# octavian-ganea/equidock_public

Measured on AMD Instinct MI355X. Metric: protein-pairs/sec (fwd+bwd) per IEGMN stack, higher is better.
Workload: dtype f32; 1 GPU; B: DB5.5-sized batch of 8 pairs x (200,200) residues, k=10, 8-layer IEGMN hdim 64, 50 heads, fp32; pairs_per_gpu=8, nodes_per_gpu=3200, edges_per_gpu=32000, layers=8, parallelism=dp1, weights=PyTorch default init (seed 0), ROT key/query x40 (SURVEY.md section 8c), svd_guard_pairs=0, launch_mode=hipGraph replay

## Files before the change

equidock_public_amd/_lib.py:

```python
import ctypes as C
import os

import torch

HERE = os.path.dirname(os.path.abspath(__file__))
LIB_PATH = os.path.join(HERE, 'libequidock_hip.so')
if os.environ.get('EQD_EXP_LIBRARY'):
    LIB_PATH = os.environ['EQD_EXP_LIBRARY']

EQD_MAX_SRC = 6
ABI_VERSION = 9
PARAMS_PER_LAYER = 19
GLOBAL_PARAMS = 5

c_float_p = C.POINTER(C.c_float)
c_int_p = C.POINTER(C.c_int32)


class EqdGraph(C.Structure):
    _fields_ = [('n_pairs', C.c_int32), ('n_lig', C.c_int32), ('n_rec', C.c_int32), ('n_nodes', C.c_int32),
                ('n_edges', C.c_int32), ('n_tiles', C.c_int32), ('n_att_items', C.c_int32), ('max_seg', C.c_int32),
                ('seg_off', C.c_void_p), ('src', C.c_void_p), ('dst', C.c_void_p), ('rowptr', C.c_void_p),
                ('csc_ptr', C.c_void_p), ('csc_eid', C.c_void_p), ('tile_node', C.c_void_p),
                ('att_items', C.c_void_p), ('res_id', C.c_void_p), ('mu_r_norm', C.c_void_p), ('he', C.c_void_p),
                ('x0', C.c_void_p), ('he_bf16', C.c_void_p)]


class EqdModelDesc(C.Structure):
    _fields_ = [('n_layers', C.c_int32), ('d_emb', C.c_int32), ('d_hid', C.c_int32),
                ('use_mean_node_features', C.c_int32), ('edge_feats', C.c_int32), ('n_heads', C.c_int32),
                ('cross_msgs', C.c_int32), ('use_dist_in_layers', C.c_int32), ('use_edge_features', C.c_int32),
                ('skip_weight_h', C.c_float), ('x_connection_init', C.c_float), ('lrelu_slope', C.c_float),
                ('ln_eps', C.c_float), ('svd_seed', C.c_int32), ('storage_bf16', C.c_int32)]


class EqdDropout(C.Structure):
    _fields_ = [('p', C.c_float), ('edge_z1', C.c_void_p), ('edge_ch', C.c_void_p), ('node', C.c_void_p),
                ('head', C.c_void_p)]


class EqdLinSrc(C.Structure):
    _fields_ = [('X', C.c_void_p), ('mask', C.c_void_p), ('W', C.c_void_p), ('ldx', C.c_int32), ('K', C.c_int32),
                ('w_rs', C.c_int32), ('w_cs', C.c_int32)]


class EqdLinJob(C.Structure):
    _fields_ = [('s', EqdLinSrc * EQD_MAX_SRC), ('nsrc', C.c_int32), ('M', C.c_int32), ('act', C.c_int32),
                ('rows', C.c_int32), ('bias', C.c_void_p), ('ln_g', C.c_void_p), ('ln_b', C.c_void_p),
                ('pre_ln', C.c_void_p), ('ld_pre', C.c_int32), ('R', C.c_void_p), ('ldr', C.c_int32),
                ('alpha', C.c_float), ('beta', C.c_float), ('slope', C.c_float), ('ln_eps', C.c_float),
                ('Y', C.c_void_p), ('ldy', C.c_int32), ('bf16', C.c_int32), ('mul', C.c_void_p), ('ld_mul', C.c_int32), ('pad_to', C.c_int32),
                ('Yb', C.c_void_p), ('ldyb', C.c_int32)]


class EqdAtbJob(C.Structure):
    _fields_ = [('X', C.c_void_p), ('xmask', C.c_void_p), ('ldx', C.c_int32), ('M', C.c_int32), ('Y', C.c_void_p),
                ('ldy', C.c_int32), ('N', C.c_int32), ('rows', C.c_int32), ('out', C.c_void_p), ('o_rs', C.c_int32),
                ('o_cs', C.c_int32), ('bias_out', C.c_void_p), ('slope', C.c_float), ('scale', C.c_float), ('bf16', C.c_int32),
                ('y_bf16', C.c_int32)]


class EqdEdgeParams(C.Structure):
    _fields_ = [('W1', C.c_void_p), ('ldw1', C.c_int32), ('d_in', C.c_int32), ('ln_g', C.c_void_p),
                ('ln_b', C.c_void_p), ('W2', C.c_void_p), ('b2', C.c_void_p), ('Wc1', C.c_void_p),
                ('bc1', C.c_void_p), ('wc2', C.c_void_p), ('bc2', C.c_void_p), ('slope', C.c_float),
                ('ln_eps', C.c_float), ('eta', C.c_float), ('use_dist', C.c_int32), ('use_he', C.c_int32),
                ('bf16', C.c_int32), ('drop_z1', C.c_void_p), ('drop_ch', C.c_void_p), ('drop_scale', C.c_float),
                ('aggr_bf16', C.c_void_p), ('xh_save', C.c_void_p), ('rstd_save', C.c_void_p), ('zpos_save', C.c_void_p)]


class EqdNodeUpdateParams(C.Structure):
    _fields_ = [('d_in', C.c_int32), ('d0', C.c_int32), ('d_out', C.c_int32), ('ld_cross', C.c_int32), ('Wn1', C.c_void_p),
                ('bn1', C.c_void_p), ('ln_g', C.c_void_p), ('ln_b', C.c_void_p), ('Wn2', C.c_void_p), ('bn2', C.c_void_p),
                ('skip_weight_h', C.c_float), ('slope', C.c_float), ('ln_eps', C.c_float), ('bf16', C.c_int32),
                ('drop_mul', C.c_void_p)]


class EqdNodeUpdateGrads(C.Structure):
    _fields_ = [('dWn1', C.c_void_p), ('dbn1', C.c_void_p), ('dln_g', C.c_void_p), ('dln_b', C.c_void_p),
                ('dWn2', C.c_void_p), ('dbn2', C.c_void_p)]


class EqdEdgeGrads(C.Structure):
    _fields_ = [('dW1', C.c_void_p), ('ldw1', C.c_int32), ('db1_unused', C.c_void_p), ('dln_g', C.c_void_p),
                ('dln_b', C.c_void_p), ('dW2', C.c_void_p), ('db2', C.c_void_p), ('dWc1', C.c_void_p),
                ('dbc1', C.c_void_p), ('dwc2', C.c_void_p), ('dbc2', C.c_void_p)]


_lib = None
_is_sim = False
profiling = False


class EquidockHipError(RuntimeError):
    pass


def _declare(lib):
    lib.eqd_abi_version.restype = C.c_int
    lib.eqd_last_error.restype = C.c_char_p
    lib.eqd_tile_edges.restype = C.c_int
    lib.eqd_is_simulator.restype = C.c_int
    lib.eqd_model_saved_bytes.restype = C.c_size_t
    lib.eqd_model_scratch_bytes.restype = C.c_size_t
    lib.eqd_atb_partial_bytes.restype = C.c_size_t
    lib.eqd_edge_message_bwd_workspace_bytes.restype = C.c_size_t
    lib.eqd_keypoint_pool_bwd_workspace_bytes.restype = C.c_size_t
    lib.eqd_clash_workspace_bytes.restype = C.c_size_t
    lib.eqd_node_update_bwd_workspace_bytes.restype = C.c_size_t
    lib.eqd_cross_attention_bwd_ds_workspace_bytes.restype = C.c_size_t
    lib.eqd_profile_name.restype = C.c_char_p
    lib.eqd_profile_us.restype = C.c_float
    lib.eqd_tunables_reload.restype = None
    for name in ('eqd_model_layer_state', 'eqd_model_lrelu_signs', 'eqd_model_head_backward', 'eqd_profile_begin', 'eqd_profile_end', 'eqd_profile_mark', 'eqd_ctx_create', 'eqd_ctx_destroy', 'eqd_model_check', 'eqd_model_forward', 'eqd_model_backward', 'eqd_linear', 'eqd_atb',
                 'eqd_edge_message_fwd', 'eqd_edge_message_bwd', 'eqd_edge_message_bwd_kernel_only',
                 'eqd_cross_attention_fwd', 'eqd_cross_attention_fwd_bf16', 'eqd_cross_attention_bwd_bf16',
                 'eqd_cross_attention_bwd', 'eqd_cross_attention_bwd_ds',
           'eqd_keypoint_pool_fwd', 'eqd_keypoint_pool_bwd', 'eqd_kabsch_fwd', 'eqd_kabsch_bwd',
                 'eqd_rigid_apply_fwd', 'eqd_rigid_apply_bwd', 'eqd_pair_losses_fwd', 'eqd_pair_losses_bwd', 'eqd_scalar_loss', 'eqd_pocket_ot_cost',
                 'eqd_pocket_ot_fwd', 'eqd_pocket_ot_bwd', 'eqd_rigid_augment', 'eqd_protein_graph_distances',
                 'eqd_protein_graph_select', 'eqd_protein_graph_edges', 'eqd_clash_iterations', 'eqd_dropout_pack_edges', 'eqd_dropout_draw',
                 'eqd_node_update_fwd', 'eqd_node_update_bwd', 'eqd_selftest_lane_exchanges'):
        getattr(lib, name).restype = C.c_int


EXPORTS = ('eqd_model_layer_state', 'eqd_model_lrelu_signs', 'eqd_model_head_backward', 'eqd_profile_begin', 'eqd_profile_end', 'eqd_profile_mark', 'eqd_profile_name', 'eqd_profile_us', 'eqd_ctx_create', 'eqd_ctx_destroy', 'eqd_abi_version', 'eqd_last_error', 'eqd_tile_edges', 'eqd_is_simulator', 'eqd_model_saved_bytes', 'eqd_model_saved_layout',
           'eqd_model_scratch_bytes', 'eqd_model_check', 'eqd_model_forward', 'eqd_model_backward', 'eqd_linear',
           'eqd_atb_partial_bytes', 'eqd_atb', 'eqd_edge_message_fwd', 'eqd_edge_message_bwd_workspace_bytes',
           'eqd_edge_message_bwd', 'eqd_edge_message_bwd_kernel_only', 'eqd_cross_attention_fwd',
           'eqd_cross_attention_bwd', 'eqd_cross_attention_bwd_ds', 'eqd_cross_attention_bwd_ds_workspace_bytes', 'eqd_cross_attention_fwd_bf16', 'eqd_cross_attention_bwd_bf16',
           'eqd_keypoint_pool_fwd', 'eqd_keypoint_pool_bwd',
           'eqd_keypoint_pool_bwd_workspace_bytes',
           'eqd_kabsch_fwd', 'eqd_kabsch_bwd', 'eqd_rigid_apply_fwd', 'eqd_rigid_apply_bwd', 'eqd_pair_losses_fwd',
           'eqd_pair_losses_bwd', 'eqd_scalar_loss', 'eqd_pocket_ot_cost', 'eqd_pocket_ot_fwd', 'eqd_pocket_ot_bwd',
           'eqd_rigid_augment', 'eqd_protein_graph_distances', 'eqd_protein_graph_select', 'eqd_protein_graph_edges',
           'eqd_clash_workspace_bytes', 'eqd_clash_iterations', 'eqd_dropout_pack_edges', 'eqd_dropout_draw',
           'eqd_tunables_reload', 'eqd_node_update_fwd', 'eqd_node_update_bwd_workspace_bytes', 'eqd_node_update_bwd',
           'eqd_selftest_lane_exchanges', 'eqd_chain_resident_proj_launches', 'eqd_selftest_node_chain_fwd', 'eqd_model_node_state',
           'eqd_chain_resident_wide_launches', 'eqd_chain_resident_wide_bwd_launches', 'eqd_selftest_node_chain_bwd_wide',
           'eqd_edge_fwd_half_launches', 'eqd_selftest_edge_attn_fwd')


def load_library():
    global _lib, _is_sim
    if _lib is not None:
        return _lib
    if not os.path.exists(LIB_PATH):
        raise EquidockHipError(
            f"{LIB_PATH} is missing: build it with `python -m equidock_public_amd.build` (hipcc, gfx950). "
            "There is no CPU fallback for the IEGMN hot path.")
    lib = C.CDLL(LIB_PATH)
    _declare(lib)
    if lib.eqd_abi_version() != ABI_VERSION:
        raise EquidockHipError(f"ABI version mismatch: library {lib.eqd_abi_version()} != {ABI_VERSION}")
    _lib, _is_sim = lib, bool(lib.eqd_is_simulator())
    return _lib


def load_library_for_testing(path):
    global _lib, _is_sim
    lib = C.CDLL(path)
    _declare(lib)
    _lib, _is_sim = lib, bool(lib.eqd_is_simulator())
    return _lib


def unload_for_testing():
    global _lib, _is_sim
    _lib, _is_sim = None, False


tunables_generation = 0


def reload_tunables():
    global tunables_generation
    tunables_generation += 1
    if _lib is not None:
        _lib.eqd_tunables_reload()


def is_simulator():
    return _is_sim


def check(rc):
    if rc != 0:
        raise EquidockHipError(f"libequidock_hip error {rc}: {_lib.eqd_last_error().decode()}")


def require_device(t, what='tensor'):
    if _is_sim:
        if t.is_cuda:
            raise EquidockHipError(f"{what}: the host simulator only takes CPU tensors")
    elif not t.is_cuda:
        raise EquidockHipError(
            f"{what} is on {t.device}: the IEGMN hot path runs only on an MI355X through libequidock_hip.so "
            "(no CPU fallback)")
    return t


class device_guard:

    def __init__(self, device):
        self._cm = None if (_is_sim or torch.device(device).type != 'cuda') else torch.cuda.device(device)

    def __enter__(self):
        if self._cm is not None:
            self._cm.__enter__()

    def __exit__(self, *exc):
        if self._cm is not None:
            self._cm.__exit__(*exc)
        return False


def ptr(t):
    return C.c_void_p(t.data_ptr()) if t is not None else C.c_void_p(0)


def stream_ptr(device):
    if _is_sim:
        return C.c_void_p(0)
    return C.c_void_p(torch.cuda.current_stream(device).cuda_stream)


_ctx = {}


def exec_ctx(device):
    if os.environ.get('EQD_FORK') != '1':
        return C.c_void_p(0)
    key = (id(_lib), str(device))
    if key not in _ctx:
        h = C.c_void_p(0)
        if not _is_sim:
            with torch.cuda.device(device):
                check(_lib.eqd_ctx_create(C.byref(h)))
        else:
            check(_lib.eqd_ctx_create(C.byref(h)))
        _ctx[key] = h
    return _ctx[key]


def graph_struct(p):
    g = EqdGraph()
    g.n_pairs, g.n_lig, g.n_rec, g.n_nodes = p.n_pairs, p.n_lig, p.n_rec, p.n_nodes
    g.n_edges, g.n_tiles, g.n_att_items, g.max_seg = p.n_edges, p.n_tiles, p.n_att_items, p.max_seg
    for name in ('seg_off', 'src', 'dst', 'rowptr', 'csc_ptr', 'csc_eid', 'tile_node', 'att_items', 'res_id',
                 'mu_r_norm', 'he', 'x0', 'he_bf16'):
        t = getattr(p, name)
        require_device(t, 'graph.' + name)
        setattr(g, name, t.data_ptr())
    return g
```

equidock_public_amd/csrc/eqd_common.h:

```cpp
#pragma once
#include <hip/hip_runtime.h>
#include <stdint.h>
#include <string.h>

#include "../../include/equidock_hip.h"

typedef float f32x4 __attribute__((ext_vector_type(4)));
typedef unsigned int u32x4 __attribute__((ext_vector_type(4)));

#define EQD_BLOCK 256
#define EQD_WAVES 4
#define EQD_NEG_BIG (-1.0e30f)

__device__ __forceinline__ f32x4 mfma4(float a, float b, f32x4 c) {
    return __builtin_amdgcn_mfma_f32_16x16x4f32(a, b, c, 0, 0, 0);
}
#ifdef EQD_TRACE
extern __device__ long long eqd_trace_buf[1024];
#define EQD_TR(slot)                                                                          \
    do {                                                                                      \
        const int trs_ = (slot);                                                              \
        if (blockIdx.x == 0 && blockIdx.y == 0 && threadIdx.x == 0 && trs_ < 256) {           \
            eqd_trace_buf[2 * trs_] = clock64();                                              \
            eqd_trace_buf[2 * trs_ + 1] = wall_clock64();                                     \
        }                                                                                     \
    } while (0)
#define EQD_TR_WG()                                                                           \
    do {                                                                                      \
        if (threadIdx.x == 0 && blockIdx.y == 0 && blockIdx.x < 256)                          \
            eqd_trace_buf[512 + 2 * blockIdx.x] = wall_clock64();                             \
    } while (0)
#define EQD_TR_WG_END()                                                                       \
    do {                                                                                      \
        __syncthreads();                                                                      \
        if (threadIdx.x == 0 && blockIdx.y == 0 && blockIdx.x < 256)                          \
            eqd_trace_buf[512 + 2 * blockIdx.x + 1] = wall_clock64();                         \
    } while (0)
#else
#define EQD_TR(slot) do { } while (0)
#define EQD_TR_WG() do { } while (0)
#define EQD_TR_WG_END() do { } while (0)
#endif

#ifndef EQD_GAS
#define EQD_GAS __attribute__((address_space(1)))
#endif

typedef float f4v __attribute__((ext_vector_type(4), aligned(4)));
__device__ __forceinline__ f32x4 ld4u_raw(const float* __restrict__ p, int n, const float* __restrict__ safe) {
    const int sh = (n > 0 && n < 4) ? 4 - n : 0;
    return *(const EQD_GAS f4v*)(n > 0 ? p - sh : safe);
}
__device__ __forceinline__ float4 ld4u_fix(f32x4 v, int n) {
    const int sh = (n > 0 && n < 4) ? 4 - n : 0;
    float4 r;
    r.x = n > 0 ? (sh == 0 ? v[0] : sh == 1 ? v[1] : sh == 2 ? v[2] : v[3]) : 0.f;
    r.y = n > 1 ? (sh == 0 ? v[1] : sh == 1 ? v[2] : v[3]) : 0.f;
    r.z = n > 2 ? (sh == 0 ? v[2] : v[3]) : 0.f;
    r.w = n > 3 ? v[3] : 0.f;
    return r;
}
#ifndef EQD_KERNARG_PTR
#define EQD_KERNARG_PTR(first_param) ((const void*)__builtin_amdgcn_kernarg_segment_ptr())
#endif
__device__ __forceinline__ int uni(int v) { return __builtin_amdgcn_readfirstlane(v); }
__device__ __forceinline__ float uni(float v) {
    return __builtin_bit_cast(float, __builtin_amdgcn_readfirstlane(__builtin_bit_cast(int, v)));
}
template <class T>
__device__ __forceinline__ T* uni(T* p) {
    const unsigned long long a = (unsigned long long)p;
    const unsigned lo = (unsigned)__builtin_amdgcn_readfirstlane((int)(unsigned)a);
    const unsigned hi = (unsigned)__builtin_amdgcn_readfirstlane((int)(unsigned)(a >> 32));
    return (T*)(((unsigned long long)hi << 32) | lo);
}
__device__ __forceinline__ EqdLinSrc uni(const EqdLinSrc& S) {
    EqdLinSrc U;
    U.X = uni(S.X); U.mask = uni(S.mask); U.W = uni(S.W);
    U.ldx = uni(S.ldx); U.K = uni(S.K); U.w_rs = uni(S.w_rs); U.w_cs = uni(S.w_cs);
    return U;
}
template <class T>
__device__ __forceinline__ void kernarg_to_lds(T& dst, const void* kernarg, int byte_offset) {
    const int* __restrict__ src = (const int*)((const char*)kernarg + byte_offset);
    for (int i = threadIdx.x; i < (int)(sizeof(T) / 4); i += blockDim.x) ((int*)&dst)[i] = src[i];
}

#ifdef EQD_HOSTSIM
__device__ __forceinline__ void glds16(const float* gsrc, float* lds_base) {
    __builtin_memcpy(lds_base + 4 * (threadIdx.x & 63), gsrc, 16);
}
template <int N>
__device__ __forceinline__ void vm_wait() { static_assert(N >= 0 && N <= 63, "vmcnt is a 6-bit count"); }
__device__ __forceinline__ void lds_barrier() { __syncthreads(); }
__device__ __forceinline__ void lds_reads_done() {}
template <class T>
__device__ __forceinline__ void keep_after_wait(T&) {}
#else
__device__ __forceinline__ void glds16(const float* gsrc, float* lds_base) {
    const unsigned dst = (unsigned)__builtin_amdgcn_readfirstlane((int)(unsigned)(uintptr_t)(__attribute__((address_space(3))) void*)lds_base);
    unsigned keep;
    asm volatile("s_mov_b32 %0, m0\n\ts_mov_b32 m0, %2\n\ts_nop 0\n\tglobal_load_lds_dwordx4 %1, off\n\ts_mov_b32 m0, %0"
                 : "=&s"(keep)
                 : "v"(gsrc), "s"(dst)
                 : "memory");
}
template <int N>
__device__ __forceinline__ void vm_wait() {
    static_assert(N >= 0 && N <= 63, "vmcnt is a 6-bit count");
    asm volatile("s_waitcnt vmcnt(%0)" ::"n"(N) : "memory");
}
__device__ __forceinline__ void lds_barrier() {
    asm volatile("s_waitcnt lgkmcnt(0)" ::: "memory");
    __builtin_amdgcn_s_barrier();
    asm volatile("" ::: "memory");
}
__device__ __forceinline__ void lds_reads_done() { asm volatile("s_waitcnt lgkmcnt(0)" ::: "memory"); }
template <class T>
__device__ __forceinline__ void keep_after_wait(T& v) { asm volatile("" : "+v"(v)); }
#endif

typedef short s16x4 __attribute__((ext_vector_type(4)));
__device__ __forceinline__ unsigned short f2bf(float f) {
#ifdef EQD_HOSTSIM
    unsigned u = __builtin_bit_cast(unsigned, f);
    u += 0x7fffu + ((u >> 16) & 1u);
    return (unsigned short)(u >> 16);
#else
    return __builtin_bit_cast(unsigned short, (__bf16)f);
#endif
}
__device__ __forceinline__ float bf2f(unsigned short h) { return __builtin_bit_cast(float, (unsigned)h << 16); }
#ifdef EQD_HOSTSIM
__device__ __forceinline__ s16x4 pack_bf4(float a, float b, float c, float d) {
    s16x4 r;
    r[0] = (short)f2bf(a); r[1] = (short)f2bf(b); r[2] = (short)f2bf(c); r[3] = (short)f2bf(d);
    return r;
}
#else
typedef float eqd_f32x2 __attribute__((ext_vector_type(2)));
typedef __bf16 eqd_bf16x2 __attribute__((ext_vector_type(2)));
typedef unsigned eqd_u32x2 __attribute__((ext_vector_type(2)));
__device__ __forceinline__ s16x4 pack_bf4(float a, float b, float c, float d) {
    const eqd_f32x2 lo = {a, b}, hi = {c, d};
    const eqd_bf16x2 l = __builtin_convertvector(lo, eqd_bf16x2), h = __builtin_convertvector(hi, eqd_bf16x2);
    const eqd_u32x2 r = {__builtin_bit_cast(unsigned, l), __builtin_bit_cast(unsigned, h)};
    return __builtin_bit_cast(s16x4, r);
}
#endif
__device__ __forceinline__ f32x4 mfma_bf(s16x4 a, s16x4 b, f32x4 c) {
    return __builtin_amdgcn_mfma_f32_16x16x16bf16_1k(a, b, c, 0, 0, 0);
}
typedef short s16x8 __attribute__((ext_vector_type(8)));
__device__ __forceinline__ s16x8 cat_bf(s16x4 lo, s16x4 hi) { return __builtin_shufflevector(lo, hi, 0, 1, 2, 3, 4, 5, 6, 7); }
__device__ __forceinline__ f32x4 mfma_bf32(s16x8 a, s16x8 b, f32x4 c) {
#if defined(EQD_HOSTSIM) || defined(EQD_MFMA_K16)
    const s16x4 a0 = __builtin_shufflevector(a, a, 0, 1, 2, 3), a1 = __builtin_shufflevector(a, a, 4, 5, 6, 7);
    const s16x4 b0 = __builtin_shufflevector(b, b, 0, 1, 2, 3), b1 = __builtin_shufflevector(b, b, 4, 5, 6, 7);
    return mfma_bf(a1, b1, mfma_bf(a0, b0, c));
#else
    typedef __bf16 eqd_bf16x8 __attribute__((ext_vector_type(8)));
    f32x4 d = __builtin_amdgcn_mfma_f32_16x16x32_bf16(__builtin_bit_cast(eqd_bf16x8, a), __builtin_bit_cast(eqd_bf16x8, b), c, 0, 0, 0);
    asm volatile("" ::"v"(a), "v"(d[0]));
    return d;
#endif
}

__device__ __forceinline__ s16x4 lds_tr16(const unsigned short* p) {
#ifdef EQD_HOSTSIM
    const unsigned long long a = (unsigned long long)p;
    const int lane = (int)(threadIdx.x & 63), grp = lane & ~15, i = lane & 15;
    s16x4 r;
    for (int j = 0; j < 4; ++j) {
        const int src = grp + 4 * j + (i >> 2);
        const unsigned lo = (unsigned)__shfl((int)(unsigned)a, src), hi = (unsigned)__shfl((int)(unsigned)(a >> 32), src);
        const unsigned short* q = (const unsigned short*)(((unsigned long long)hi << 32) | lo);
        r[j] = (short)q[i & 3];
    }
    return r;
#else
    return __builtin_amdgcn_ds_read_tr16_b64_v4i16((__attribute__((address_space(3))) s16x4*)p);
#endif
}

__device__ __forceinline__ f32x4 f4zero() {
    f32x4 z = {0.f, 0.f, 0.f, 0.f};
    return z;
}
__device__ __forceinline__ float lrelu(float v, float s) { return v > 0.f ? v : v * s; }
__device__ __forceinline__ float lrelu_grad(float y, float s) { return y > 0.f ? 1.f : s; }

template <int M>
__device__ __forceinline__ float lane_xor(float v) {
    static_assert(M == 1 || M == 2 || M == 4 || M == 8, "inside a row of 16 lanes");
#if defined(EQD_HOSTSIM) || defined(EQD_NO_DPP)
    return __shfl_xor(v, M);
#else
    const int i = __builtin_bit_cast(int, v);
    int r;
#ifdef EQD_DPP_ZEROED_OLD
    constexpr bool BC = false;
#else
    constexpr bool BC = true;
#endif
    if constexpr (M == 1) r = __builtin_amdgcn_update_dpp(0, i, 0xB1, 0xf, 0xf, BC);
    else if constexpr (M == 2) r = __builtin_amdgcn_update_dpp(0, i, 0x4E, 0xf, 0xf, BC);
    else if constexpr (M == 8) r = __builtin_amdgcn_update_dpp(0, i, 0x128, 0xf, 0xf, BC);
    else r = __builtin_amdgcn_update_dpp(0, __builtin_amdgcn_update_dpp(0, i, 0x141, 0xf, 0xf, BC), 0x1B, 0xf, 0xf,
                                         BC);
    return __builtin_bit_cast(float, r);
#endif
}
template <int M>
__device__ __forceinline__ float lane_swap_sum(float v, int want_max) {
#if defined(EQD_HOSTSIM) || defined(EQD_NO_PLSWAP)
    const float o = __shfl_xor(v, M);
    return want_max ? fmaxf(v, o) : v + o;
#else
    float x = v, y = v;
    if constexpr (M == 16) asm volatile("s_nop 1\n\tv_permlane16_swap_b32 %0, %1" : "+v"(x), "+v"(y));
    else asm volatile("s_nop 1\n\tv_permlane32_swap_b32 %0, %1" : "+v"(x), "+v"(y));
    return want_max ? fmaxf(x, y) : x + y;
#endif
}
__device__ __forceinline__ float exp_nooverflow(float x) {
#if defined(EQD_HOSTSIM) || defined(EQD_LIBM_EXP)
    return expf(x);
#else
    const float c = __builtin_bit_cast(float, 0x3fb8aa3bu), cl = __builtin_bit_cast(float, 0x32a5705fu);
    x = x < -1000.f ? -1000.f : x;
    const float p = x * c;
    float e = __builtin_fmaf(x, c, -p);
    e = __builtin_fmaf(x, cl, e);
    const float n = __builtin_rintf(p);
    const float f = (p - n) + e;
    return __builtin_ldexpf(__builtin_amdgcn_exp2f(f), (int)n);
#endif
}
__device__ __forceinline__ float exp2_flush(float x) {
#if defined(EQD_HOSTSIM) || defined(EQD_LIBM_EXP)
    return exp2f(x);
#else
    return __builtin_amdgcn_exp2f(x);
#endif
}
__device__ __forceinline__ float group_sum(float v) {
#if defined(EQD_HOSTSIM) || defined(EQD_NO_PLSWAP)
    v += __shfl_xor(v, 16);
    v += __shfl_xor(v, 32);
    return v;
#else
    const float s = lane_swap_sum<16>(v, 0);
    return lane_swap_sum<32>(s, 0);
#endif
}
__device__ __forceinline__ float group_max(float v) {
#if defined(EQD_HOSTSIM) || defined(EQD_NO_PLSWAP)
    v = fmaxf(v, __shfl_xor(v, 16));
    v = fmaxf(v, __shfl_xor(v, 32));
    return v;
#else
    const float s = lane_swap_sum<16>(v, 1);
    return lane_swap_sum<32>(s, 1);
#endif
}
__device__ __forceinline__ float l16_sum(float v) {
    v += lane_xor<1>(v);
    v += lane_xor<2>(v);
    v += lane_xor<4>(v);
    v += lane_xor<8>(v);
    return v;
}
__device__ __forceinline__ float wave_sum(float v) { return group_sum(l16_sum(v)); }
__device__ __forceinline__ float reduce16x16(const float (&v)[16], int l15) {
    const bool b3 = (l15 & 8) != 0, b2 = (l15 & 4) != 0, b1 = (l15 & 2) != 0, b0 = (l15 & 1) != 0;
    float w8[8], w4[4], w2[2];
#if defined(EQD_HOSTSIM) || defined(EQD_NO_DPP) || defined(EQD_NO_DPP_ASM)
#pragma unroll
    for (int i = 0; i < 8; ++i) w8[i] = (b3 ? v[i + 8] : v[i]) + lane_xor<8>(b3 ? v[i] : v[i + 8]);
#pragma unroll
    for (int i = 0; i < 4; ++i) w4[i] = (b2 ? w8[i + 4] : w8[i]) + lane_xor<4>(b2 ? w8[i] : w8[i + 4]);
#else
    asm("s_nop 1\n\t"
        "v_add_f32_dpp %0, %8, %8 row_ror:8 row_mask:0xf bank_mask:0x3\n\t"
        "v_add_f32_dpp %0, %16, %16 row_ror:8 row_mask:0xf bank_mask:0xc\n\t"
        "v_add_f32_dpp %1, %9, %9 row_ror:8 row_mask:0xf bank_mask:0x3\n\t"
        "v_add_f32_dpp %1, %17, %17 row_ror:8 row_mask:0xf bank_mask:0xc\n\t"
        "v_add_f32_dpp %2, %10, %10 row_ror:8 row_mask:0xf bank_mask:0x3\n\t"
        "v_add_f32_dpp %2, %18, %18 row_ror:8 row_mask:0xf bank_mask:0xc\n\t"
        "v_add_f32_dpp %3, %11, %11 row_ror:8 row_mask:0xf bank_mask:0x3\n\t"
        "v_add_f32_dpp %3, %19, %19 row_ror:8 row_mask:0xf bank_mask:0xc\n\t"
        "v_add_f32_dpp %4, %12, %12 row_ror:8 row_mask:0xf bank_mask:0x3\n\t"
        "v_add_f32_dpp %4, %20, %20 row_ror:8 row_mask:0xf bank_mask:0xc\n\t"
        "v_add_f32_dpp %5, %13, %13 row_ror:8 row_mask:0xf bank_mask:0x3\n\t"
        "v_add_f32_dpp %5, %21, %21 row_ror:8 row_mask:0xf bank_mask:0xc\n\t"
        "v_add_f32_dpp %6, %14, %14 row_ror:8 row_mask:0xf bank_mask:0x3\n\t"
        "v_add_f32_dpp %6, %22, %22 row_ror:8 row_mask:0xf bank_mask:0xc\n\t"
        "v_add_f32_dpp %7, %15, %15 row_ror:8 row_mask:0xf bank_mask:0x3\n\t"
        "v_add_f32_dpp %7, %23, %23 row_ror:8 row_mask:0xf bank_mask:0xc"
        : "=&v"(w8[0]), "=&v"(w8[1]), "=&v"(w8[2]), "=&v"(w8[3]), "=&v"(w8[4]), "=&v"(w8[5]), "=&v"(w8[6]), "=&v"(w8[7])
        : "v"(v[0]), "v"(v[1]), "v"(v[2]), "v"(v[3]), "v"(v[4]), "v"(v[5]), "v"(v[6]), "v"(v[7]),
          "v"(v[8]), "v"(v[9]), "v"(v[10]), "v"(v[11]), "v"(v[12]), "v"(v[13]), "v"(v[14]), "v"(v[15]));
    {
        float t[8];
        asm("s_nop 1\n\t"
            "v_mov_b32_dpp %4, %12 row_half_mirror row_mask:0xf bank_mask:0xf\n\t"
            "v_mov_b32_dpp %5, %13 row_half_mirror row_mask:0xf bank_mask:0xf\n\t"
            "v_mov_b32_dpp %6, %14 row_half_mirror row_mask:0xf bank_mask:0xf\n\t"
            "v_mov_b32_dpp %7, %15 row_half_mirror row_mask:0xf bank_mask:0xf\n\t"
            "v_mov_b32_dpp %8, %16 row_half_mirror row_mask:0xf bank_mask:0xf\n\t"
            "v_mov_b32_dpp %9, %17 row_half_mirror row_mask:0xf bank_mask:0xf\n\t"
            "v_mov_b32_dpp %10, %18 row_half_mirror row_mask:0xf bank_mask:0xf\n\t"
            "v_mov_b32_dpp %11, %19 row_half_mirror row_mask:0xf bank_mask:0xf\n\t"
            "v_add_f32_dpp %0, %4, %12 quad_perm:[3,2,1,0] row_mask:0xf bank_mask:0x5\n\t"
            "v_add_f32_dpp %0, %8, %16 quad_perm:[3,2,1,0] row_mask:0xf bank_mask:0xa\n\t"
            "v_add_f32_dpp %1, %5, %13 quad_perm:[3,2,1,0] row_mask:0xf bank_mask:0x5\n\t"
            "v_add_f32_dpp %1, %9, %17 quad_perm:[3,2,1,0] row_mask:0xf bank_mask:0xa\n\t"
            "v_add_f32_dpp %2, %6, %14 quad_perm:[3,2,1,0] row_mask:0xf bank_mask:0x5\n\t"
            "v_add_f32_dpp %2, %10, %18 quad_perm:[3,2,1,0] row_mask:0xf bank_mask:0xa\n\t"
            "v_add_f32_dpp %3, %7, %15 quad_perm:[3,2,1,0] row_mask:0xf bank_mask:0x5\n\t"
            "v_add_f32_dpp %3, %11, %19 quad_perm:[3,2,1,0] row_mask:0xf bank_mask:0xa"
            : "=&v"(w4[0]), "=&v"(w4[1]), "=&v"(w4[2]), "=&v"(w4[3]), "=&v"(t[0]), "=&v"(t[1]), "=&v"(t[2]), "=&v"(t[3]),
              "=&v"(t[4]), "=&v"(t[5]), "=&v"(t[6]), "=&v"(t[7])
            : "v"(w8[0]), "v"(w8[1]), "v"(w8[2]), "v"(w8[3]), "v"(w8[4]), "v"(w8[5]), "v"(w8[6]), "v"(w8[7]));
    }
    (void)b3;
    (void)b2;
#endif
#pragma unroll
    for (int i = 0; i < 2; ++i) w2[i] = (b1 ? w4[i + 2] : w4[i]) + lane_xor<2>(b1 ? w4[i] : w4[i + 2]);
    return (b0 ? w2[1] : w2[0]) + lane_xor<1>(b0 ? w2[0] : w2[1]);
}

__device__ __forceinline__ void wave_lds_fence() {
    __builtin_amdgcn_fence(__ATOMIC_ACQ_REL, "wavefront");
    __builtin_amdgcn_wave_barrier();
}

void eqd_set_error(const char* fmt, ...);
int eqd_check_launch(const char* what);
const char* eqd_tunable(const char* name);
bool eqd_switch_on(const char* name);
int eqd_num_cus();

static inline size_t eqd_align_up(size_t v, size_t a = 256) { return (v + a - 1) / a * a; }

struct EqdArena {
    char* base;
    size_t size, off;
    bool ok;
    EqdArena(void* p, size_t n) : base((char*)p), size(n), off(0), ok(true) {}
    template <typename T>
    T* take(size_t count) {
        size_t bytes = eqd_align_up(count * sizeof(T));
        if (base == nullptr || off + bytes > size) {
            ok = false;
            off += bytes;
            return nullptr;
        }
        T* r = (T*)(base + off);
        off += bytes;
        return r;
    }
};

#define EQD_RED_MAXSEG 64
struct EqdRedSeg {
    const float* partial;
    int nparts, pstride, n;
    float* out;
    int cols, cols_valid, ld_out;
};
struct EqdRedArg {
    EqdRedSeg s[EQD_RED_MAXSEG];
    int chain_first[EQD_RED_MAXSEG], chain_len[EQD_RED_MAXSEG];
    int chain_blk0[EQD_RED_MAXSEG];
    int nchains;
};
int eqd_launch_reduce_segments(const EqdRedSeg* segs, int nseg, hipStream_t st);
struct EqdRedList {
    EqdRedSeg seg[512];
    int n;
};

#define EQD_CHAIN_MAXJOBS 8
struct EqdChainJob {
    EqdLinJob lin;
    int src_local[EQD_MAX_SRC];
    int out_local;
    int type;
    float* aux;
    int prefetch_next;
    int next_lin;
};
struct EqdChainArg {
    EqdChainJob j[EQD_CHAIN_MAXJOBS];
    int njobs;
};
static inline void eqd_chain_job_clear(EqdChainJob& C) {
    memset(&C, 0, sizeof(C));
    for (int i = 0; i < EQD_MAX_SRC; ++i) C.src_local[i] = -1;
    C.out_local = -1;
}
int eqd_launch_rowchain(const EqdChainJob* jobs, int njobs, int rows, hipStream_t st, int* partial_rows = nullptr,
                        bool wide_ok = true);
size_t eqd_atb_batch_partial_bytes(int rows);
int eqd_atb_tail_wanted(const EqdLinJob* dh0_job, int n_atb_jobs);
int eqd_atb_with_tail(const EqdAtbJob* jobs, int njobs, void* partial, size_t partial_bytes, hipStream_t st,
                      const EqdLinJob* dh0_job, const EqdGraph* g, const float* dh0acc, const float* dh0b, int ld, int d_emb,
                      float* demb, float* emb_partial, EqdRedList* defer);
int eqd_rows_resident(int rows);
int eqd_rowres80_on();
int eqd_chain_carries_proj(int rows);
int eqd_row_tiles(int rows);
int eqd_rowchain_blocks(int rows);

int eqd_launch_vec_reduce(const float* partial, int nparts, int pstride, int n, float* out, hipStream_t st);
int eqd_launch_embed_fwd(const EqdGraph* g, const float* emb, int d_emb, int use_mu, float* h0, int ld, hipStream_t st);
struct EqdRedList;
int eqd_launch_embed_bwd(const EqdGraph* g, const float* dh0, const float* dh0b, int ld, int d_emb, float* demb,
                         float* partial, hipStream_t st, EqdRedList* defer = nullptr);
size_t eqd_embed_bwd_partial_floats(const EqdGraph* g, int d_emb);
struct EqdGatherCall {
    const float *dz, *dxrel, *d_xnew;
    float a;
    float *dP, *dQ, *dx;
    int dz_bf16;
};
struct EqdGatherArgs;
int eqd_gather_plan(const EqdGraph* g, const EqdGatherCall* c, EqdRedList* pending, EqdGatherArgs* GA, EqdRedArg* RA, int* nblk);
int eqd_gather_rest(EqdRedList* pending, hipStream_t st);
int eqd_attention_bwd_gather_fused(const EqdGraph* g, int d, const float* q, const float* k, const float* v, const float* out,
                                   const float* d_out, bool bf16);
int eqd_attention_ds_stride(const EqdGraph* g);
size_t eqd_attention_ds_bytes(const EqdGraph* g);
int eqd_attention_ds_wanted(const EqdGraph* g, int d, bool bf16);
int eqd_launch_seg_start(const EqdGraph* g, int32_t* seg_start, hipStream_t st);
int eqd_attention_fwd_bf16_impl(const EqdGraph* g, int d, const float* q, const float* k, const float* v, float* out,
                                float* lse, hipStream_t stream, bool qkv_bf16);
int eqd_launch_attention_bwd_gather(const EqdGraph* g, int d, const float* q, const float* k, const float* v, const float* out,
                                    const float* lse, const float* d_out, float* dq, float* dk, float* dv, float* delta,
                                    float qk_slope, bool bf16, const EqdGatherCall* gc, EqdRedList* pending, hipStream_t st,
                                    float* ds = nullptr, const int32_t* seg_start = nullptr, bool qkv_bf16 = false);
int eqd_launch_node_gather(const EqdGraph* g, const float* dz, const float* dxrel, const float* d_xnew, float a,
                           float* dP, float* dQ, float* dx, hipStream_t st, EqdRedList* pending = nullptr,
                           bool dz_bf16 = false);
int eqd_launch_ln_act_bwd(const float* y_act, const float* d_out, const float* gamma, int rows, int d, int ld,
                          float slope, float eps, float* dz, float* dgamma, float* dbeta, float* partial,
                          hipStream_t st, EqdRedList* defer = nullptr);
int eqd_edge_message_bwd_impl(const EqdGraph* g, const EqdEdgeParams* p, const float* P, const float* Q, const float* x,
                              const float* d_aggr_msg, const float* d_xnew, float* dP, float* dQ, float* dx,
                              const EqdEdgeGrads* grads, void* workspace, size_t ws_bytes, hipStream_t st,
                              float* part_override, EqdRedList* defer, EqdGatherCall* hold_gather = nullptr);
size_t eqd_edge_bwd_vecp_floats(const EqdGraph* g);
int eqd_edge_attn_fwd(const EqdGraph* g, const EqdEdgeParams* p, const float* P, const float* Q, const float* x,
                      float* aggr_msg, float* x_new, int d_att, const float* q, const float* k, const float* v,
                      float* att_out, float* lse, hipStream_t st);
int eqd_keypoint_pool_fwd_impl(const EqdGraph* g, int n_heads, const float* Wk, const float* Wq, const float* qmean,
                               const float* H, const float* Z, float* Y, float* Y_lig_out, float* Y_rec_out,
                               float* scores, float* lse, float* qp, float* u, hipStream_t st, float* Yc = nullptr);
int eqd_kabsch_fwd_impl(int n_pairs, int n_heads, const float* Y, const float* svd_draws, int svd_seed, float* T,
                        float* T2, float* b, float* A_out, int32_t* status, hipStream_t st, const EqdGraph* g = nullptr,
                        float* lig_out = nullptr, double* usv = nullptr);
int eqd_kabsch_bwd_impl(int n_pairs, int n_heads, const float* Y, const float* A, const float* T, const float* dT,
                        const float* db, const float* dYl_ext, const float* dYr_ext, float* dY, hipStream_t st,
                        const EqdGraph* g = nullptr, const float* d_lig = nullptr, const double* usv = nullptr);
int eqd_rigid_apply_bwd_impl(const EqdGraph* g, const float* d_lig, const float* dT_ext, const float* db_ext, float* dT,
                             float* db, hipStream_t st);
size_t eqd_ln_act_bwd_partial_floats(int rows, int d);
int eqd_launch_fill(float* p, float v, size_t n, hipStream_t st);
int eqd_launch_axpy(float* y, const float* x, float a, size_t n, hipStream_t st);
int eqd_launch_attention_bwd_act(const EqdGraph* g, int d, const float* q, const float* k, const float* v, const float* out,
                                 const float* lse, const float* d_out, float* dq, float* dk, float* dv, float* delta,
                                 float qk_slope, bool bf16, hipStream_t st);
int eqd_launch_seg_mean(const EqdGraph* g, const float* hm, float* qmean, hipStream_t st);
size_t eqd_head_u_bwd_partial_floats(int n_pairs, int K);
int eqd_launch_head_u_bwd(const EqdGraph* g, int K, const float* Wk, const float* Wq, const float* qmean,
                          const float* qp, const float* du, float* dWk, float* dWq, float* dqm_part, hipStream_t st,
                          float* part, EqdRedList* defer, int du_chunks = 1);
int eqd_launch_qmean_bwd(const EqdGraph* g, int K, const float* dqm_part, float* dhm, hipStream_t st);
int eqd_launch_keypoint_bwd(const EqdGraph* g, int K, const float* H, const float* Z, const float* scores,
                            const float* lse, const float* u, const float* dY, float* dscores, float* du,
                            float* dH, float* dZ, hipStream_t st, const float* Y = nullptr,
                            int* du_chunks = nullptr);
```

equidock_public_amd/csrc/eqd_edge_fwd_half_inl.h:

```cpp
#pragma once

#define EDGE_HALF_WAVES (2 * FWD_WAVES)
#define EDGE_HALF_FEAT1 (32 * TS - 16 * FS)
static_assert(16 * FS <= 16 * TS && EDGE_HALF_FEAT1 >= 16 * TS, "a half's feature tile lies inside its own message rows");

template <int J0, bool MOM>
__device__ __forceinline__ void edge_half_means(const float* __restrict__ tile, float* __restrict__ sxw, int rp, float invl,
                                                int nb0, int nn, int n0, int l15, int g, float* __restrict__ aggr_msg) {
    const int node = nb0 + l15;
    const int lo = __shfl(rp, node), hi = __shfl(rp, node + 1);
    const bool nv = node < nn;
    f32x4 acc[2], accx = f4zero();
    acc[0] = acc[1] = f4zero();
#pragma unroll
    for (int ks = 0; ks < 8; ++ks) {
        const int e = 4 * ks + g;
        const float am = (nv && e >= lo && e < hi) ? 1.f : 0.f;
#pragma unroll
        for (int j = 0; j < 2; ++j) acc[j] = mfma4(am, tile[e * TS + 16 * (J0 + j) + l15], acc[j]);
        if constexpr (MOM) accx = mfma4(am, tile[e * TS + 64 + (l15 & 3)], accx);
    }
#pragma unroll
    for (int r = 0; r < 4; ++r) {
        const int nd = nb0 + 4 * g + r;
        const float inv = __shfl(invl, nd);
        if (nd < nn) {
#pragma unroll
            for (int j = 0; j < 2; ++j) aggr_msg[(size_t)(n0 + nd) * 64 + 16 * (J0 + j) + l15] = acc[j][r] * inv;
            if constexpr (MOM) {
                if (l15 < 3) sxw[3 * nd + l15] = accx[r] * inv;
            }
        }
    }
}

template <bool DROP>
__device__ __forceinline__ void edge_fwd_half_body(EdgeFwdSmem<FWD_WAVES, false>& S_, const EqdGraph& G, const EqdEdgeParams& P,
                                                   int blk, const float* __restrict__ Pn, const float* __restrict__ Qn,
                                                   const float* __restrict__ x, float* __restrict__ aggr_msg,
                                                   float* __restrict__ x_new) {
    auto& sm = S_.sm;
    EQD_TR_WG();
    EQD_TR(0);
    const int lane = threadIdx.x & 63, wave = threadIdx.x >> 6;
    const int w = wave & (FWD_WAVES - 1), h = wave >> 3;
    const int l15 = lane & 15, g = lane >> 4;
    float* tile = sm.tile[w];
    float* sxw = S_.sxw[w];
    const int t = blk * FWD_WAVES + w;
    const bool live = t < G.n_tiles;
    int n0 = 0, n1 = 0, e0 = 0, ne = 0;
    if (live) {
        n0 = G.tile_node[t];
        n1 = G.tile_node[t + 1];
        e0 = G.rowptr[n0];
        ne = G.rowptr[n1] - e0;
    }
    edge_stage_weights<FWD_WAVES, 32 * TS, 64 * EDGE_HALF_WAVES>(sm, P);
    EQD_TR(1);
    const int nn = n1 - n0;
    const size_t xo = (size_t)n0 * 3;
    const int c0 = lane, c1 = lane + 64;
    int rp = 0;
    float x0a = 0.f, xa = 0.f, x0b = 0.f, xb = 0.f;
    if (live) {
        rp = G.rowptr[n0 + (lane <= nn ? lane : 0)] - e0;
        if (h == 0) {
            x0a = G.x0[xo + (c0 < 3 * nn ? c0 : 0)], xa = x[xo + (c0 < 3 * nn ? c0 : 0)];
            x0b = G.x0[xo + (c1 < 3 * nn ? c1 : 0)], xb = x[xo + (c1 < 3 * nn ? c1 : 0)];
        }
        EdgeTileState<1> S;
        S.n0 = n0;
        S.n1 = n1;
        S.ne = ne - 16 * h;
        S.ne = S.ne < 0 ? 0 : (S.ne > 16 ? 16 : S.ne);
        S.e0 = S.ne > 0 ? e0 + 16 * h : e0;
        const int row = 16 * h + l15;
        if (S.ne > 0) {
            f32x4 xh[4][1], m[4][1], ch[4][1];
            edge_tile_forward<1, DROP, false>(G, P, sm.w1, sm.w2, sm.wc1, sm.vec, tile + h * EDGE_HALF_FEAT1, Pn, Qn, x, lane, S,
                                              xh, m, ch, nullptr);
            wave_lds_fence();
#pragma unroll
            for (int mb = 0; mb < 4; ++mb)
                *(float4*)&tile[row * TS + 16 * mb + 4 * g] = make_float4(m[mb][0][0], m[mb][0][1], m[mb][0][2], m[mb][0][3]);
            if (g == 0) {
#pragma unroll
                for (int c = 0; c < 3; ++c) tile[row * TS + 64 + c] = S.xrel[0][c] * S.coef[0];
                tile[row * TS + 67] = 0.f;
            }
        } else {
#pragma unroll
            for (int mb = 0; mb < 4; ++mb) *(float4*)&tile[row * TS + 16 * mb + 4 * g] = make_float4(0.f, 0.f, 0.f, 0.f);
            if (g == 0) *(float4*)&tile[row * TS + 64] = make_float4(0.f, 0.f, 0.f, 0.f);
        }
    }
    EQD_TR(10);
    __syncthreads();
    if (live) {
    const int degl = __shfl(rp, (lane + 1) & 63) - rp;
    const float invl = (lane < nn && degl > 0) ? 1.f / (float)degl : 0.f;
    if (h == 0) {
        for (int nb0 = 0; nb0 < nn; nb0 += 16) edge_half_means<0, true>(tile, sxw, rp, invl, nb0, nn, n0, l15, g, aggr_msg);
        wave_lds_fence();
        if (c0 < 3 * nn) x_new[xo + c0] = P.eta * x0a + (1.f - P.eta) * xa + sxw[c0];
        if (c1 < 3 * nn) x_new[xo + c1] = P.eta * x0b + (1.f - P.eta) * xb + sxw[c1];
    } else {
        for (int nb0 = 0; nb0 < nn; nb0 += 16) edge_half_means<2, false>(tile, sxw, rp, invl, nb0, nn, n0, l15, g, aggr_msg);
    }
    }
    EQD_TR(11);
    EQD_TR_WG_END();
}

template <bool DROP>
__global__ __launch_bounds__(64 * EDGE_HALF_WAVES) void k_edge_attn_fwd_half(EqdGraph G, EqdEdgeParams P, int n_edge,
                                                                              const float* __restrict__ Pn,
                                                                              const float* __restrict__ Qn,
                                                                              const float* __restrict__ x,
                                                                              float* __restrict__ aggr_msg,
                                                                              float* __restrict__ x_new,
                                                                              const float* __restrict__ q,
                                                                              const float* __restrict__ k,
                                                                              const float* __restrict__ v,
                                                                              float* __restrict__ att_out,
                                                                              float* __restrict__ lse) {
    __shared__ EdgeAttnFwdSmem S;
    if ((int)blockIdx.x < n_edge) {
        edge_fwd_half_body<DROP>(S.edge, G, P, (int)blockIdx.x, Pn, Qn, x, aggr_msg, x_new);
    } else {
        if (threadIdx.x >= 512) return;
        const int half = (int)threadIdx.x >> 8;
        attn_fwd_body<4, true, 1, false, true>(S.att[half], G, (int)blockIdx.x - n_edge, half, (int)threadIdx.x & 255, 64, q, k, v,
                                  att_out, lse, true);
    }
}
```

equidock_public_amd/csrc/eqd_edge_kernels.hip:

```cpp
#include "eqd_common.h"
#include "eqd_attn_fwd_inl.h"

#include <stdlib.h>
#include <string.h>
#include <atomic>

#define WS1 45
#define WS2 68
#define TS 68
#define FS 45
#define VEC_LNG 0
#define VEC_LNB 64
#define VEC_B2 128
#define VEC_BC1 192
#define VEC_WC2 256
#define VEC_BC2 320
#define VEC_N 324
#define FWD_WAVES 8
#define BWD_WAVES 8

template <int NW, int TILE_FLOATS>
struct alignas(16) EdgeSmem {
    float w1[64 * WS1];
    float w2[64 * WS2];
    float wc1[64 * WS2];
    float vec[VEC_N];
    float tile[NW][TILE_FLOATS];
};

template <int NW, int TF, int NT = 64 * NW>
__device__ __forceinline__ void edge_stage_weights(EdgeSmem<NW, TF>& sm, const EqdEdgeParams& P) {
    static_assert(1024 % NT == 0, "W2 / Wc1 are staged as 1024 float4 in whole rounds of the workgroup");
    constexpr int N1 = (64 * 11 + NT - 1) / NT, N2 = 1024 / NT;
    const int t = threadIdx.x;
    const int koff = 2 * P.d_in;
    f32x4 v[N1];
    float4 a[N2], b[N2];
    float vec5[5];
#pragma unroll
    for (int j = 0; j < N1; ++j) {
        const int i = t + j * NT;
        const int r = i / 11, c = 4 * (i - r * 11);
        v[j] = ld4u_raw(P.W1 + (size_t)(i < 64 * 11 ? r : 0) * P.ldw1 + koff + c, i < 64 * 11 ? 42 - c : 0, P.W1);
    }
#pragma unroll
    for (int j = 0; j < N2; ++j) {
        const int i = t + j * NT;
        a[j] = ((const float4*)P.W2)[i];
        b[j] = ((const float4*)P.Wc1)[i];
    }
    {
        const int tc = t & 63;
        vec5[0] = P.ln_g[tc];
        vec5[1] = P.ln_b[tc];
        vec5[2] = P.b2[tc];
        vec5[3] = P.bc1[tc];
        vec5[4] = P.wc2[tc];
    }
    const float bc2 = P.bc2[0];
#pragma unroll
    for (int j = 0; j < N1; ++j) {
        const int i = t + j * NT;
        const int r = i / 11, c = 4 * (i - r * 11);
        if (i < 64 * 11) {
            const float4 f = ld4u_fix(v[j], 42 - c);
            float* o = &sm.w1[r * WS1 + c];
            o[0] = f.x;
            if (c + 1 < WS1) o[1] = f.y;
            if (c + 2 < WS1) o[2] = f.z;
            if (c + 3 < WS1) o[3] = f.w;
        }
    }
    if (t < 64) sm.w1[t * WS1 + 44] = 0.f;
#pragma unroll
    for (int j = 0; j < N2; ++j) {
        const int i = t + j * NT;
        const int r = i >> 4, c = (i & 15) * 4;
        *(float4*)&sm.w2[r * WS2 + c] = a[j];
        *(float4*)&sm.wc1[r * WS2 + c] = b[j];
    }
    if (t < 64) {
        sm.vec[VEC_LNG + t] = vec5[0];
        sm.vec[VEC_LNB + t] = vec5[1];
        sm.vec[VEC_B2 + t] = vec5[2];
        sm.vec[VEC_BC1 + t] = vec5[3];
        sm.vec[VEC_WC2 + t] = vec5[4];
    }
    if (t == 0) sm.vec[VEC_BC2] = bc2;
    __syncthreads();
}

__device__ __forceinline__ float rbf_sigma(int k) {
    const float t[16] = {1.f,          1.5f,         2.25f,        3.375f,        5.0625f,     7.59375f,
                         11.390625f,   17.0859375f,  25.62890625f, 38.443359375f, 57.6650390625f,
                         86.49755859375f, 129.746337890625f, 194.6195068359375f, 291.92926025390625f, 1.f};
    return t[k & 15];
}

__device__ __forceinline__ float rbf_neg_inv_sigma(int k) {
    const float t[16] = {-1.f / 1.f,          -1.f / 1.5f,         -1.f / 2.25f,        -1.f / 3.375f,        -1.f / 5.0625f,
                         -1.f / 7.59375f,     -1.f / 11.390625f,   -1.f / 17.0859375f,  -1.f / 25.62890625f,  -1.f / 38.443359375f,
                         -1.f / 57.6650390625f, -1.f / 86.49755859375f, -1.f / 129.746337890625f, -1.f / 194.6195068359375f,
                         -1.f / 291.92926025390625f, -1.f};
    return t[k & 15];
}

template <bool AFF, int NB>
__device__ __forceinline__ void chain64(f32x4 (&out)[4][NB], const f32x4 (&in)[4][NB], const float* __restrict__ W,
                                        const float* __restrict__ ga, const float* __restrict__ be, int l15, int g) {
#pragma unroll
    for (int mbi = 0; mbi < 4; ++mbi) {
        f32x4 b[NB];
#pragma unroll
        for (int nb = 0; nb < NB; ++nb) b[nb] = in[mbi][nb];
        if (AFF) {
            const float4 gg = *(const float4*)&ga[16 * mbi + 4 * g];
            const float4 bb = *(const float4*)&be[16 * mbi + 4 * g];
#pragma unroll
            for (int nb = 0; nb < NB; ++nb) {
                b[nb][0] = b[nb][0] * gg.x + bb.x;
                b[nb][1] = b[nb][1] * gg.y + bb.y;
                b[nb][2] = b[nb][2] * gg.z + bb.z;
                b[nb][3] = b[nb][3] * gg.w + bb.w;
            }
        }
        float4 w[4];
#pragma unroll
        for (int mbo = 0; mbo < 4; ++mbo) w[mbo] = *(const float4*)&W[(16 * mbo + l15) * WS2 + 16 * mbi + 4 * g];
#if !defined(EQD_HOSTSIM) && !defined(EQD_NO_LDS_BATCH) && !defined(EQD_NO_LDS_BATCH_ROWEDGE)
        __builtin_amdgcn_sched_barrier(0);
#endif
#pragma unroll
        for (int mbo = 0; mbo < 4; ++mbo) {
            const float wv[4] = {w[mbo].x, w[mbo].y, w[mbo].z, w[mbo].w};
#pragma unroll
            for (int r = 0; r < 4; ++r)
#pragma unroll
                for (int nb = 0; nb < NB; ++nb) out[mbo][nb] = mfma4(wv[r], b[nb][r], out[mbo][nb]);
        }
    }
}
template <int NB>
__device__ __forceinline__ void chain64T(f32x4 (&out)[4][NB], const f32x4 (&in)[4][NB], const float* __restrict__ W,
                                         int l15, int g) {
#pragma unroll
    for (int mbi = 0; mbi < 4; ++mbi) {
        float w[4][4];
#pragma unroll
        for (int r = 0; r < 4; ++r)
#pragma unroll
            for (int mbo = 0; mbo < 4; ++mbo) w[r][mbo] = W[(16 * mbi + 4 * g + r) * WS2 + 16 * mbo + l15];
#if !defined(EQD_HOSTSIM) && !defined(EQD_NO_LDS_BATCH) && !defined(EQD_NO_LDS_BATCH_ROWEDGE)
        __builtin_amdgcn_sched_barrier(0);
#endif
#pragma unroll
        for (int r = 0; r < 4; ++r)
#pragma unroll
            for (int mbo = 0; mbo < 4; ++mbo) {
#pragma unroll
                for (int nb = 0; nb < NB; ++nb) out[mbo][nb] = mfma4(w[r][mbo], in[mbi][nb][r], out[mbo][nb]);
            }
    }
}

template <int NB>
struct EdgeTileState {
    int e0, ne, n0, n1;
    int src[NB], dst[NB];
    bool ev[NB];
    float xrel[NB][3];
    float d2[NB];
    float rbf[NB][4];
    float mean[NB], rstd[NB];
    float coef[NB];
    unsigned zpos;
    unsigned keepz, keepc;
};

__device__ __forceinline__ unsigned drop_bits16(const uint32_t* __restrict__ words, int e, int g) {
    const uint32_t w0 = words[(size_t)e * 2], w1 = words[(size_t)e * 2 + 1];
    unsigned b = 0u;
#pragma unroll
    for (int mb = 0; mb < 4; ++mb) b |= (((mb < 2 ? w0 : w1) >> (16 * (mb & 1) + 4 * g)) & 0xfu) << (4 * mb);
    return b;
}
template <int NB>
__device__ __forceinline__ void drop_load(const EqdEdgeParams& P, EdgeTileState<NB>& S, int l15, int g) {
    S.keepz = S.keepc = 0u;
#pragma unroll
    for (int nb = 0; nb < NB; ++nb) {
        const int e = S.e0 + ((16 * nb + l15) < S.ne ? 16 * nb + l15 : 0);
        S.keepz |= drop_bits16(P.drop_z1, e, g) << (16 * nb);
        S.keepc |= drop_bits16(P.drop_ch, e, g) << (16 * nb);
    }
}

template <int NB>
__device__ __forceinline__ void edge_state_store(const EqdEdgeParams& P, const EdgeTileState<NB>& S, const f32x4 (&xh)[4][NB],
                                                 int l15, int g) {
#pragma unroll
    for (int nb = 0; nb < NB; ++nb)
        if (S.ev[nb]) {
            const size_t er = (size_t)S.e0 + 16 * nb + l15;
#pragma unroll
            for (int mb = 0; mb < 4; ++mb)
                *(float4*)&P.xh_save[er * 64 + 16 * mb + 4 * g] =
                    make_float4(xh[mb][nb][0], xh[mb][nb][1], xh[mb][nb][2], xh[mb][nb][3]);
            P.zpos_save[er * 4 + g] = (uint16_t)((S.zpos >> (16 * nb)) & 0xffffu);
            if (g == 0) P.rstd_save[er] = S.rstd[nb];
        }
}

template <int NB, bool DROP = false, bool PRE = false, bool SAVED = false>
__device__ __forceinline__ void edge_tile_forward(const EqdGraph& G, const EqdEdgeParams& P, const float* __restrict__ w1,
                                                  const float* __restrict__ w2, const float* __restrict__ wc1,
                                                  const float* __restrict__ vec, float* __restrict__ tile,
                                                  const float* __restrict__ Pn, const float* __restrict__ Qn,
                                                  const float* __restrict__ x, int lane, EdgeTileState<NB>& S,
                                                  f32x4 (&xh)[4][NB], f32x4 (&m)[4][NB], f32x4 (&ch)[4][NB],
                                                  float* __restrict__ rbf_out) {
    const int l15 = lane & 15, g = lane >> 4;
    EQD_TR(2);
    constexpr int NH = (16 * NB * 27 / 4 + 63) / 64;
    const float* __restrict__ he = G.he + (size_t)S.e0 * 27;
    const int nhe = P.use_he ? S.ne * 27 : 0;
    f32x4 hv[NH];
#pragma unroll
    for (int j = 0; j < NH; ++j) {
        const int i = 4 * (lane + 64 * j);
        hv[j] = ld4u_raw(he + (i < nhe ? i : 0), nhe - i, G.he);
    }
#pragma unroll
    for (int nb = 0; nb < NB; ++nb) {
        const int el = 16 * nb + l15;
        S.ev[nb] = el < S.ne;
        if constexpr (!PRE) {
            const int ei = S.e0 + (S.ev[nb] ? el : 0);
            S.src[nb] = G.src[ei];
            S.dst[nb] = G.dst[ei];
        }
    }
    float xs[NB][3], xd[NB][3];
    float4 pv[NB][4], qv[NB][4];
    float rsv[NB];
    unsigned zsv[NB];
#pragma unroll
    for (int nb = 0; nb < NB; ++nb) {
#pragma unroll
        for (int c = 0; c < 3; ++c) {
            xs[nb][c] = x[(size_t)S.src[nb] * 3 + c];
            xd[nb][c] = x[(size_t)S.dst[nb] * 3 + c];
        }
        if constexpr (SAVED) {
            const size_t er = (size_t)S.e0 + (S.ev[nb] ? 16 * nb + l15 : 0);
#pragma unroll
            for (int mb = 0; mb < 4; ++mb) pv[nb][mb] = *(const float4*)&P.xh_save[er * 64 + 16 * mb + 4 * g];
            rsv[nb] = P.rstd_save[er];
            zsv[nb] = P.zpos_save[er * 4 + g];
        } else {
#pragma unroll
            for (int mb = 0; mb < 4; ++mb) {
                pv[nb][mb] = *(const float4*)&Pn[(size_t)S.src[nb] * 64 + 16 * mb + 4 * g];
                qv[nb][mb] = *(const float4*)&Qn[(size_t)S.dst[nb] * 64 + 16 * mb + 4 * g];
            }
        }
    }
    for (int i = lane; i < 16 * NB * FS; i += 64) tile[i] = 0.f;
    wave_lds_fence();
    EQD_TR(3);
#pragma unroll
    for (int j = 0; j < NH; ++j) {
        const int i = 4 * (lane + 64 * j);
        const float4 hf = ld4u_fix(hv[j], nhe - i);
        const float vv[4] = {hf.x, hf.y, hf.z, hf.w};
        int e = i / 27, c = i - e * 27;
#pragma unroll
        for (int u = 0; u < 4; ++u) {
            if (i + u < nhe) tile[e * FS + c] = vv[u];
            if (++c == 27) {
                c = 0;
                ++e;
            }
        }
    }
#pragma unroll
    for (int nb = 0; nb < NB; ++nb) {
        float q = 0.f;
#pragma unroll
        for (int c = 0; c < 3; ++c) {
            const float v = S.ev[nb] ? xs[nb][c] - xd[nb][c] : 0.f;
            S.xrel[nb][c] = v;
            q += v * v;
        }
        S.d2[nb] = q;
    }
#pragma unroll
    for (int nb = 0; nb < NB; ++nb) {
        const int el = 16 * nb + l15;
#pragma unroll
        for (int j = 0; j < 4; ++j) {
            const int k = PRE ? 4 * g + j : g + 4 * j;
            if (k < 15 && S.ev[nb]) {
                const float v = P.use_dist ? exp_nooverflow(-S.d2[nb] / rbf_sigma(k)) : 0.f;
                tile[el * FS + 27 + k] = v;
                if (rbf_out) rbf_out[(size_t)(S.e0 + el) * 16 + k] = v;
            }
        }
        if (rbf_out && g == 3 && S.ev[nb]) rbf_out[(size_t)(S.e0 + el) * 16 + 15] = 0.f;
    }
    wave_lds_fence();
    EQD_TR(4);
    S.zpos = 0u;
    if constexpr (DROP) drop_load<NB>(P, S, l15, g);
    if constexpr (SAVED) {
#pragma unroll
        for (int nb = 0; nb < NB; ++nb) {
#pragma unroll
            for (int mb = 0; mb < 4; ++mb) {
                const float4 v = pv[nb][mb];
                f32x4 a;
                a[0] = S.ev[nb] ? v.x : 0.f; a[1] = S.ev[nb] ? v.y : 0.f; a[2] = S.ev[nb] ? v.z : 0.f; a[3] = S.ev[nb] ? v.w : 0.f;
                xh[mb][nb] = a;
            }
            S.zpos |= (S.ev[nb] ? zsv[nb] : 0u) << (16 * nb);
            S.mean[nb] = 0.f;
            S.rstd[nb] = rsv[nb];
        }
    } else {
#pragma unroll
    for (int nb = 0; nb < NB; ++nb)
#pragma unroll
        for (int mb = 0; mb < 4; ++mb) {
            const float4 p = pv[nb][mb], q = qv[nb][mb];
            f32x4 a;
            a[0] = S.ev[nb] ? p.x + q.x : 0.f; a[1] = S.ev[nb] ? p.y + q.y : 0.f;
            a[2] = S.ev[nb] ? p.z + q.z : 0.f; a[3] = S.ev[nb] ? p.w + q.w : 0.f;
            xh[mb][nb] = a;
        }
    EQD_TR(5);
#pragma unroll
    for (int s = 0; s < 11; ++s) {
        const int k = 4 * s + g;
        float b[NB];
#pragma unroll
        for (int nb = 0; nb < NB; ++nb) b[nb] = tile[(16 * nb + l15) * FS + k];
#pragma unroll
        for (int mb = 0; mb < 4; ++mb) {
            const float a = w1[(16 * mb + l15) * WS1 + k];
#pragma unroll
            for (int nb = 0; nb < NB; ++nb) xh[mb][nb] = mfma4(a, b[nb], xh[mb][nb]);
        }
    }
    EQD_TR(6);
#pragma unroll
    for (int nb = 0; nb < NB; ++nb) {
        float s = 0.f;
#pragma unroll
        for (int mb = 0; mb < 4; ++mb)
#pragma unroll
            for (int r = 0; r < 4; ++r) {
                const float z = xh[mb][nb][r];
                if (z > 0.f) S.zpos |= 1u << (16 * nb + 4 * mb + r);
                float v = lrelu(z, P.slope);
                if constexpr (DROP) v *= ((S.keepz >> (16 * nb + 4 * mb + r)) & 1u) ? P.drop_scale : 0.f;
                xh[mb][nb][r] = v;
                s += v;
            }
        const float mean = group_sum(s) * (1.f / 64.f);
        float q = 0.f;
#pragma unroll
        for (int mb = 0; mb < 4; ++mb)
#pragma unroll
            for (int r = 0; r < 4; ++r) {
                const float d = xh[mb][nb][r] - mean;
                q += d * d;
            }
        const float rstd = 1.f / sqrtf(group_sum(q) * (1.f / 64.f) + P.ln_eps);
#pragma unroll
        for (int mb = 0; mb < 4; ++mb)
#pragma unroll
            for (int r = 0; r < 4; ++r) xh[mb][nb][r] = (xh[mb][nb][r] - mean) * rstd;
        S.mean[nb] = mean;
        S.rstd[nb] = rstd;
    }
    }
    if constexpr (!SAVED) {
        if (P.xh_save) edge_state_store<NB>(P, S, xh, l15, g);
    }
    EQD_TR(7);
#pragma unroll
    for (int mb = 0; mb < 4; ++mb) {
        const float4 b = *(const float4*)&vec[VEC_B2 + 16 * mb + 4 * g];
        f32x4 v = {b.x, b.y, b.z, b.w};
#pragma unroll
        for (int nb = 0; nb < NB; ++nb) m[mb][nb] = v;
    }
    chain64<true, NB>(m, xh, w2, &vec[VEC_LNG], &vec[VEC_LNB], l15, g);
    EQD_TR(8);
#pragma unroll
    for (int mb = 0; mb < 4; ++mb) {
        const float4 b = *(const float4*)&vec[VEC_BC1 + 16 * mb + 4 * g];
        f32x4 v = {b.x, b.y, b.z, b.w};
#pragma unroll
        for (int nb = 0; nb < NB; ++nb) ch[mb][nb] = v;
    }
    chain64<false, NB>(ch, m, wc1, nullptr, nullptr, l15, g);
#pragma unroll
    for (int nb = 0; nb < NB; ++nb) {
        float s = 0.f;
#pragma unroll
        for (int mb = 0; mb < 4; ++mb) {
            const float4 w = *(const float4*)&vec[VEC_WC2 + 16 * mb + 4 * g];
            if constexpr (DROP) {
                const float wv[4] = {w.x, w.y, w.z, w.w};
#pragma unroll
                for (int r = 0; r < 4; ++r)
                    s += lrelu(ch[mb][nb][r], P.slope) *
                         (((S.keepc >> (16 * nb + 4 * mb + r)) & 1u) ? P.drop_scale : 0.f) * wv[r];
            } else {
                s += lrelu(ch[mb][nb][0], P.slope) * w.x + lrelu(ch[mb][nb][1], P.slope) * w.y +
                     lrelu(ch[mb][nb][2], P.slope) * w.z + lrelu(ch[mb][nb][3], P.slope) * w.w;
            }
        }
        S.coef[nb] = group_sum(s) + vec[VEC_BC2];
    }
    EQD_TR(9);
}

#define WSB 72
#define FSB 72
template <int NW, int TILE_FLOATS>
struct alignas(16) EdgeSmemBf {
    unsigned short w1[64 * WSB];
    unsigned short w2[64 * WSB];
    unsigned short wc1[64 * WSB];
    float vec[VEC_N];
    float tile[NW][TILE_FLOATS];
};
template <int NW, int TILE_FLOATS>
struct alignas(16) EdgeSmemBfBwd {
    unsigned short w1[64 * WSB];
    unsigned short w2[64 * WSB];
    unsigned short wc1[64 * WSB];
    unsigned short w2T[64 * WSB];
    unsigned short wc1T[64 * WSB];
    unsigned short w1rT[16 * WSB];
    float vec[VEC_N];
    float tile[NW][TILE_FLOATS];
};
template <int NW, bool WITH_T, class SM>
__device__ __forceinline__ void edge_stage_weights_bf(SM& sm, const EqdEdgeParams& P) {
    constexpr int NT = 64 * NW;
    constexpr int N1 = (64 * 12 + NT - 1) / NT, N2 = 1024 / NT;
    const int t = threadIdx.x;
    const int koff = 2 * P.d_in;
    if constexpr (WITH_T) {
        if (t < 64) sm.w1rT[15 * WSB + t] = 0;
    }
    {
        f32x4 v[N1];
#pragma unroll
        for (int j = 0; j < N1; ++j) {
            const int i = t + j * NT;
            const int r = i / 12, c = 4 * (i - r * 12);
            v[j] = ld4u_raw(P.W1 + (size_t)(i < 64 * 12 ? r : 0) * P.ldw1 + koff + c, i < 64 * 12 ? 42 - c : 0, P.W1);
        }
#pragma unroll
        for (int j = 0; j < N1; ++j) {
            const int i = t + j * NT;
            const int r = i / 12, c = 4 * (i - r * 12);
            if (i < 64 * 12) {
                const float4 f = ld4u_fix(v[j], 42 - c);
                const s16x4 h = pack_bf4(f.x, f.y, f.z, f.w);
                *(s16x4*)&sm.w1[r * WSB + c] = h;
                if constexpr (WITH_T) {
#pragma unroll
                    for (int u = 0; u < 4; ++u)
                        if (c + u >= 27 && c + u < 42) sm.w1rT[(c + u - 27) * WSB + r] = (unsigned short)h[u];
                }
            }
        }
    }
    {
        float4 a[N2], b[N2];
#pragma unroll
        for (int j = 0; j < N2; ++j) {
            const int i = t + j * NT;
            a[j] = ((const float4*)P.W2)[i];
            b[j] = ((const float4*)P.Wc1)[i];
        }
#pragma unroll
        for (int j = 0; j < N2; ++j) {
            const int i = t + j * NT;
            const int r = i >> 4, c = (i & 15) * 4;
            const s16x4 ha = pack_bf4(a[j].x, a[j].y, a[j].z, a[j].w), hb = pack_bf4(b[j].x, b[j].y, b[j].z, b[j].w);
            *(s16x4*)&sm.w2[r * WSB + c] = ha;
            *(s16x4*)&sm.wc1[r * WSB + c] = hb;
            if constexpr (WITH_T) {
#pragma unroll
                for (int u = 0; u < 4; ++u) {
                    sm.w2T[(c + u) * WSB + r] = (unsigned short)ha[u];
                    sm.wc1T[(c + u) * WSB + r] = (unsigned short)hb[u];
                }
            }
        }
    }
    if (t < 64) {
        sm.vec[VEC_LNG + t] = P.ln_g[t];
        sm.vec[VEC_LNB + t] = P.ln_b[t];
        sm.vec[VEC_B2 + t] = P.b2[t];
        sm.vec[VEC_BC1 + t] = P.bc1[t];
        sm.vec[VEC_WC2 + t] = P.wc2[t];
    }
    if (t == 0) sm.vec[VEC_BC2] = P.bc2[0];
    __syncthreads();
}

template <bool AFF, int NB>
__device__ __forceinline__ void chain64_bf(f32x4 (&out)[4][NB], const f32x4 (&in)[4][NB], const unsigned short* __restrict__ w,
                                           const float* __restrict__ ga, const float* __restrict__ be, int l15, int g) {
#pragma unroll
    for (int mp = 0; mp < 2; ++mp) {
        s16x8 b[NB];
        s16x4 bh[2][NB];
#pragma unroll
        for (int h = 0; h < 2; ++h) {
            const int mbi = 2 * mp + h;
            float gg[4] = {1.f, 1.f, 1.f, 1.f}, bb[4] = {0.f, 0.f, 0.f, 0.f};
            if (AFF) {
                const float4 gv = *(const float4*)&ga[16 * mbi + 4 * g];
                const float4 bv = *(const float4*)&be[16 * mbi + 4 * g];
                gg[0] = gv.x; gg[1] = gv.y; gg[2] = gv.z; gg[3] = gv.w;
                bb[0] = bv.x; bb[1] = bv.y; bb[2] = bv.z; bb[3] = bv.w;
            }
#pragma unroll
            for (int nb = 0; nb < NB; ++nb)
                bh[h][nb] = pack_bf4(in[mbi][nb][0] * gg[0] + bb[0], in[mbi][nb][1] * gg[1] + bb[1],
                                     in[mbi][nb][2] * gg[2] + bb[2], in[mbi][nb][3] * gg[3] + bb[3]);
        }
#pragma unroll
        for (int nb = 0; nb < NB; ++nb) b[nb] = cat_bf(bh[0][nb], bh[1][nb]);
        s16x8 a[4];
#pragma unroll
        for (int mb = 0; mb < 4; ++mb)
            a[mb] = cat_bf(*(const s16x4*)&w[(16 * mb + l15) * WSB + 32 * mp + 4 * g],
                           *(const s16x4*)&w[(16 * mb + l15) * WSB + 32 * mp + 16 + 4 * g]);
#if !defined(EQD_HOSTSIM) && !defined(EQD_NO_LDS_BATCH) && !defined(EQD_NO_LDS_BATCH_ROWEDGE)
        __builtin_amdgcn_sched_barrier(0);
#endif
#pragma unroll
        for (int mb = 0; mb < 4; ++mb) {
#pragma unroll
            for (int nb = 0; nb < NB; ++nb) out[mb][nb] = mfma_bf32(a[mb], b[nb], out[mb][nb]);
        }
    }
}

template <int NB, bool DROP = false, bool PRE = false, bool SAVED = false>
__device__ __forceinline__ void edge_tile_forward_bf(const EqdGraph& G, const EqdEdgeParams& P,
                                                     const unsigned short* __restrict__ w1,
                                                     const unsigned short* __restrict__ w2,
                                                     const unsigned short* __restrict__ wc1,
                                                     const float* __restrict__ vec, float* __restrict__ tile,
                                                     const float* __restrict__ Pn, const float* __restrict__ Qn,
                                                     const float* __restrict__ x, int lane, EdgeTileState<NB>& S,
                                                     f32x4 (&xh)[4][NB], f32x4 (&m)[4][NB], f32x4 (&ch)[4][NB]) {
    const int l15 = lane & 15, g = lane >> 4;
    unsigned short* __restrict__ ft = (unsigned short*)tile;
    EQD_TR(2);
    f32x4 hv[NB];
#pragma unroll
    for (int j = 0; j < NB; ++j) {
        const int i4 = lane + 64 * j, e = i4 >> 2, part = i4 & 3;
        hv[j] = *(const f32x4*)(G.he_bf16 + ((size_t)S.e0 + (e < S.ne ? e : 0)) * 32 + 8 * part);
    }
#pragma unroll
    for (int nb = 0; nb < NB; ++nb) {
        const int el = 16 * nb + l15;
        S.ev[nb] = el < S.ne;
        if constexpr (!PRE) {
            const int ei = S.e0 + (S.ev[nb] ? el : 0);
            S.src[nb] = G.src[ei];
            S.dst[nb] = G.dst[ei];
        }
    }
    float xs[NB][3], xd[NB][3];
    float4 pv[NB][4], qv[NB][4];
    float rsv[NB];
    unsigned zsv[NB];
#pragma unroll
    for (int nb = 0; nb < NB; ++nb) {
#pragma unroll
        for (int c = 0; c < 3; ++c) {
            xs[nb][c] = x[(size_t)S.src[nb] * 3 + c];
            xd[nb][c] = x[(size_t)S.dst[nb] * 3 + c];
        }
        if constexpr (SAVED) {
            const size_t er = (size_t)S.e0 + (S.ev[nb] ? 16 * nb + l15 : 0);
#pragma unroll
            for (int mb = 0; mb < 4; ++mb) pv[nb][mb] = *(const float4*)&P.xh_save[er * 64 + 16 * mb + 4 * g];
            rsv[nb] = P.rstd_save[er];
            zsv[nb] = P.zpos_save[er * 4 + g];
        } else {
#pragma unroll
            for (int mb = 0; mb < 4; ++mb) {
                pv[nb][mb] = *(const float4*)&Pn[(size_t)S.src[nb] * 64 + 16 * mb + 4 * g];
                qv[nb][mb] = *(const float4*)&Qn[(size_t)S.dst[nb] * 64 + 16 * mb + 4 * g];
            }
        }
    }
    EQD_TR(3);
    {
        const f32x4 z = f4zero();
        if (lane < 32 * NB) *(f32x4*)&ft[(lane >> 1) * FSB + 32 + 8 * (lane & 1)] = z;
#pragma unroll
        for (int j = 0; j < NB; ++j) {
            const int i4 = lane + 64 * j, e = i4 >> 2, part = i4 & 3;
            *(f32x4*)&ft[e * FSB + 8 * part] = (P.use_he && e < S.ne) ? hv[j] : z;
        }
    }
    wave_lds_fence();
#pragma unroll
    for (int nb = 0; nb < NB; ++nb) {
        float q = 0.f;
#pragma unroll
        for (int c = 0; c < 3; ++c) {
            const float v = S.ev[nb] ? xs[nb][c] - xd[nb][c] : 0.f;
            S.xrel[nb][c] = v;
            q += v * v;
        }
        S.d2[nb] = q;
        const int el = 16 * nb + l15;
#pragma unroll
        for (int j = 0; j < 4; ++j) {
            const int k = PRE ? 4 * g + j : g + 4 * j;
            float v = 0.f;
            if (k < 15 && S.ev[nb]) {
                v = P.use_dist ? exp_nooverflow(q * rbf_neg_inv_sigma(k)) : 0.f;
                ft[el * FSB + 27 + k] = f2bf(v);
            }
            if constexpr (PRE) S.rbf[nb][j] = v;
        }
    }
    wave_lds_fence();
    EQD_TR(4);
    S.zpos = 0u;
    if constexpr (DROP) drop_load<NB>(P, S, l15, g);
    if constexpr (SAVED) {
#pragma unroll
        for (int nb = 0; nb < NB; ++nb) {
#pragma unroll
            for (int mb = 0; mb < 4; ++mb) {
                const float4 v = pv[nb][mb];
                f32x4 a;
                a[0] = S.ev[nb] ? v.x : 0.f; a[1] = S.ev[nb] ? v.y : 0.f; a[2] = S.ev[nb] ? v.z : 0.f; a[3] = S.ev[nb] ? v.w : 0.f;
                xh[mb][nb] = a;
            }
            S.zpos |= (S.ev[nb] ? zsv[nb] : 0u) << (16 * nb);
            S.mean[nb] = 0.f;
            S.rstd[nb] = rsv[nb];
        }
    } else {
#pragma unroll
    for (int nb = 0; nb < NB; ++nb)
#pragma unroll
        for (int mb = 0; mb < 4; ++mb) {
            const float4 p = pv[nb][mb], q = qv[nb][mb];
            f32x4 a;
            a[0] = S.ev[nb] ? p.x + q.x : 0.f; a[1] = S.ev[nb] ? p.y + q.y : 0.f;
            a[2] = S.ev[nb] ? p.z + q.z : 0.f; a[3] = S.ev[nb] ? p.w + q.w : 0.f;
            xh[mb][nb] = a;
        }
    EQD_TR(5);
    {
        s16x8 b[NB];
#pragma unroll
        for (int nb = 0; nb < NB; ++nb)
            b[nb] = cat_bf(*(const s16x4*)&ft[(16 * nb + l15) * FSB + 4 * g], *(const s16x4*)&ft[(16 * nb + l15) * FSB + 16 + 4 * g]);
#pragma unroll
        for (int mb = 0; mb < 4; ++mb) {
            const s16x8 a = cat_bf(*(const s16x4*)&w1[(16 * mb + l15) * WSB + 4 * g], *(const s16x4*)&w1[(16 * mb + l15) * WSB + 16 + 4 * g]);
#pragma unroll
            for (int nb = 0; nb < NB; ++nb) xh[mb][nb] = mfma_bf32(a, b[nb], xh[mb][nb]);
        }
    }
    {
        s16x4 b[NB];
#pragma unroll
        for (int nb = 0; nb < NB; ++nb) b[nb] = *(const s16x4*)&ft[(16 * nb + l15) * FSB + 32 + 4 * g];
#pragma unroll
        for (int mb = 0; mb < 4; ++mb) {
            const s16x4 a = *(const s16x4*)&w1[(16 * mb + l15) * WSB + 32 + 4 * g];
#pragma unroll
            for (int nb = 0; nb < NB; ++nb) xh[mb][nb] = mfma_bf(a, b[nb], xh[mb][nb]);
        }
    }
    EQD_TR(6);
#pragma unroll
    for (int nb = 0; nb < NB; ++nb) {
        float s = 0.f;
#pragma unroll
        for (int mb = 0; mb < 4; ++mb)
#pragma unroll
            for (int r = 0; r < 4; ++r) {
                const float z = xh[mb][nb][r];
                if (z > 0.f) S.zpos |= 1u << (16 * nb + 4 * mb + r);
                float v = lrelu(z, P.slope);
                if constexpr (DROP) v *= ((S.keepz >> (16 * nb + 4 * mb + r)) & 1u) ? P.drop_scale : 0.f;
                xh[mb][nb][r] = v;
                s += v;
            }
        const float mean = group_sum(s) * (1.f / 64.f);
        float q = 0.f;
#pragma unroll
        for (int mb = 0; mb < 4; ++mb)
#pragma unroll
            for (int r = 0; r < 4; ++r) {
                const float d = xh[mb][nb][r] - mean;
                q += d * d;
            }
        const float rstd = 1.f / sqrtf(group_sum(q) * (1.f / 64.f) + P.ln_eps);
#pragma unroll
        for (int mb = 0; mb < 4; ++mb)
#pragma unroll
            for (int r = 0; r < 4; ++r) xh[mb][nb][r] = (xh[mb][nb][r] - mean) * rstd;
        S.mean[nb] = mean;
        S.rstd[nb] = rstd;
    }
    }
    if constexpr (!SAVED) {
        if (P.xh_save) edge_state_store<NB>(P, S, xh, l15, g);
    }
    EQD_TR(7);
#pragma unroll
    for (int mb = 0; mb < 4; ++mb) {
        const float4 b = *(const float4*)&vec[VEC_B2 + 16 * mb + 4 * g];
        const float4 c = *(const float4*)&vec[VEC_BC1 + 16 * mb + 4 * g];
        f32x4 v = {b.x, b.y, b.z, b.w}, u = {c.x, c.y, c.z, c.w};
#pragma unroll
        for (int nb = 0; nb < NB; ++nb) {
            m[mb][nb] = v;
            ch[mb][nb] = u;
        }
    }
    chain64_bf<true, NB>(m, xh, w2, &vec[VEC_LNG], &vec[VEC_LNB], l15, g);
    EQD_TR(8);
    chain64_bf<false, NB>(ch, m, wc1, nullptr, nullptr, l15, g);
#pragma unroll
    for (int nb = 0; nb < NB; ++nb) {
        float s = 0.f;
#pragma unroll
        for (int mb = 0; mb < 4; ++mb) {
            const float4 w = *(const float4*)&vec[VEC_WC2 + 16 * mb + 4 * g];
            if constexpr (DROP) {
                const float wv[4] = {w.x, w.y, w.z, w.w};
#pragma unroll
                for (int r = 0; r < 4; ++r)
                    s += lrelu(ch[mb][nb][r], P.slope) *
                         (((S.keepc >> (16 * nb + 4 * mb + r)) & 1u) ? P.drop_scale : 0.f) * wv[r];
            } else {
                s += lrelu(ch[mb][nb][0], P.slope) * w.x + lrelu(ch[mb][nb][1], P.slope) * w.y +
                     lrelu(ch[mb][nb][2], P.slope) * w.z + lrelu(ch[mb][nb][3], P.slope) * w.w;
            }
        }
        S.coef[nb] = group_sum(s) + vec[VEC_BC2];
    }
    EQD_TR(9);
}

template <int NB>
__device__ __forceinline__ void hbm_store(float* __restrict__ dst, const f32x4 (&v)[4][NB], const EdgeTileState<NB>& S,
                                          int l15, int g) {
#pragma unroll
    for (int nb = 0; nb < NB; ++nb)
        if (S.ev[nb]) {
            float* row = dst + (size_t)(S.e0 + 16 * nb + l15) * 64;
#pragma unroll
            for (int mb = 0; mb < 4; ++mb)
                *(float4*)&row[16 * mb + 4 * g] = make_float4(v[mb][nb][0], v[mb][nb][1], v[mb][nb][2], v[mb][nb][3]);
        }
}

template <int NW, int TF, bool BF>
struct EdgeSmemSel {
    typedef EdgeSmem<NW, TF> type;
};
template <int NW, int TF>
struct EdgeSmemSel<NW, TF, true> {
    typedef EdgeSmemBf<NW, TF> type;
};

template <int NW, bool BF>
struct EdgeFwdSmem {
    typename EdgeSmemSel<NW, 32 * TS, BF>::type sm;
    float sxw[NW][96];
};
template <int NW, bool BF, bool DROP = false>
__device__ __forceinline__ void edge_fwd_body(EdgeFwdSmem<NW, BF>& S_, const EqdGraph& G, const EqdEdgeParams& P, int blk,
                                              int nblk, const float* __restrict__ Pn, const float* __restrict__ Qn,
                                              const float* __restrict__ x, float* __restrict__ aggr_msg,
                                              float* __restrict__ x_new) {
    auto& sm = S_.sm;
    float (*sxw)[96] = S_.sxw;
    EQD_TR_WG();
    EQD_TR(0);
    const int lane = threadIdx.x & 63, wave = threadIdx.x >> 6;
    const int l15 = lane & 15, g = lane >> 4;
    float* tile = sm.tile[wave];
    constexpr bool AHEAD = BF;
    int nx_n0 = 0, nx_n1 = 0, nx_e0 = 0, nx_ne = 0, nx_src[2] = {0, 0}, nx_dst[2] = {0, 0};
    auto link_nodes = [&](int t_) {
        nx_n0 = G.tile_node[t_];
        nx_n1 = G.tile_node[t_ + 1];
    };
    auto link_range = [&]() {
        nx_e0 = G.rowptr[nx_n0];
        nx_ne = G.rowptr[nx_n1] - nx_e0;
    };
    auto link_endpoints = [&]() {
#pragma unroll
        for (int nb = 0; nb < 2; ++nb) {
            const int el = 16 * nb + l15;
            const int ei = nx_e0 + (el < nx_ne ? el : 0);
            nx_src[nb] = G.src[ei];
            nx_dst[nb] = G.dst[ei];
        }
    };
    const int t_first = blk * NW + wave, t_step = nblk * NW;
    if (t_first < G.n_tiles) {
        link_nodes(t_first);
        link_range();
        if constexpr (AHEAD) link_endpoints();
    }
    if constexpr (BF)
        edge_stage_weights_bf<NW, false>(sm, P);
    else
        edge_stage_weights(sm, P);
    EQD_TR(1);
    for (int t = t_first; t < G.n_tiles; t += t_step) {
        EdgeTileState<2> S;
        if constexpr (AHEAD) {
            S.n0 = nx_n0;
            S.n1 = nx_n1;
            S.e0 = nx_e0;
            S.ne = nx_ne;
#pragma unroll
            for (int nb = 0; nb < 2; ++nb) {
                S.src[nb] = nx_src[nb];
                S.dst[nb] = nx_dst[nb];
            }
        } else if (t == t_first) {
            S.n0 = nx_n0;
            S.n1 = nx_n1;
            S.e0 = nx_e0;
            S.ne = nx_ne;
        } else {
            S.n0 = G.tile_node[t];
            S.n1 = G.tile_node[t + 1];
            S.e0 = G.rowptr[S.n0];
            S.ne = G.rowptr[S.n1] - S.e0;
        }
        const bool more = AHEAD && t + t_step < G.n_tiles;
        if (more) link_nodes(t + t_step);
        f32x4 xh[4][2], m[4][2], ch[4][2];
        const int nn_pre = S.n1 - S.n0;
        const int rp = G.rowptr[S.n0 + (lane <= nn_pre ? lane : 0)] - S.e0;
        const size_t xo = (size_t)S.n0 * 3;
        const int c0 = lane, c1 = lane + 64;
        const float x0a = G.x0[xo + (c0 < 3 * nn_pre ? c0 : 0)], xa = x[xo + (c0 < 3 * nn_pre ? c0 : 0)];
        const float x0b = G.x0[xo + (c1 < 3 * nn_pre ? c1 : 0)], xb = x[xo + (c1 < 3 * nn_pre ? c1 : 0)];
        if constexpr (BF)
            edge_tile_forward_bf<2, DROP, true>(G, P, sm.w1, sm.w2, sm.wc1, sm.vec, tile, Pn, Qn, x, lane, S, xh, m, ch);
        else
            edge_tile_forward<2, DROP, false>(G, P, sm.w1, sm.w2, sm.wc1, sm.vec, tile, Pn, Qn, x, lane, S, xh, m, ch, nullptr);
        if (more) link_range();
        wave_lds_fence();
#pragma unroll
        for (int nb = 0; nb < 2; ++nb)
#pragma unroll
            for (int mb = 0; mb < 4; ++mb)
                *(float4*)&tile[(16 * nb + l15) * TS + 16 * mb + 4 * g] =
                    make_float4(m[mb][nb][0], m[mb][nb][1], m[mb][nb][2], m[mb][nb][3]);
        if (g == 0) {
#pragma unroll
            for (int nb = 0; nb < 2; ++nb) {
#pragma unroll
                for (int c = 0; c < 3; ++c) tile[(16 * nb + l15) * TS + 64 + c] = S.xrel[nb][c] * S.coef[nb];
                tile[(16 * nb + l15) * TS + 67] = 0.f;
            }
        }
        wave_lds_fence();
        EQD_TR(10);
        const int nn = S.n1 - S.n0;
        const int degl = __shfl(rp, (lane + 1) & 63) - rp;
        const float invl = (lane < nn && degl > 0) ? 1.f / (float)degl : 0.f;
        for (int nb0 = 0; nb0 < nn; nb0 += 16) {
            const int node = nb0 + l15;
            const int lo = __shfl(rp, node), hi = __shfl(rp, node + 1);
            const bool nv = node < nn;
            f32x4 acc[5];
#pragma unroll
            for (int j = 0; j < 5; ++j) acc[j] = f4zero();
#pragma unroll
            for (int ks = 0; ks < 8; ++ks) {
                const int e = 4 * ks + g;
                const float am = (nv && e >= lo && e < hi) ? 1.f : 0.f;
#pragma unroll
                for (int j = 0; j < 4; ++j) acc[j] = mfma4(am, tile[e * TS + 16 * j + l15], acc[j]);
                acc[4] = mfma4(am, tile[e * TS + 64 + (l15 & 3)], acc[4]);
            }
#pragma unroll
            for (int r = 0; r < 4; ++r) {
                const int nd = nb0 + 4 * g + r;
                const float inv = __shfl(invl, nd);
                if (nd < nn) {
#pragma unroll
                    for (int j = 0; j < 4; ++j) {
                        const float vv = acc[j][r] * inv;
                        aggr_msg[(size_t)(S.n0 + nd) * 64 + 16 * j + l15] = vv;
                        if constexpr (BF) {
                            if (P.aggr_bf16) P.aggr_bf16[(size_t)(S.n0 + nd) * 64 + 16 * j + l15] = f2bf(vv);
                        }
                    }
                    if (l15 < 3) sxw[wave][3 * nd + l15] = acc[4][r] * inv;
                }
            }
        }
        wave_lds_fence();
        if (more) link_endpoints();
        if (c0 < 3 * nn) x_new[xo + c0] = P.eta * x0a + (1.f - P.eta) * xa + sxw[wave][c0];
        if (c1 < 3 * nn) x_new[xo + c1] = P.eta * x0b + (1.f - P.eta) * xb + sxw[wave][c1];
        wave_lds_fence();
        EQD_TR(11);
    }
    EQD_TR_WG_END();
}
template <int NW, bool BF, bool DROP = false>
__global__ __launch_bounds__(64 * NW) void k_edge_fwd(EqdGraph G, EqdEdgeParams P, const float* __restrict__ Pn,
                                                              const float* __restrict__ Qn,
                                                              const float* __restrict__ x,
                                                              float* __restrict__ aggr_msg,
                                                              float* __restrict__ x_new) {
    __shared__ EdgeFwdSmem<NW, BF> S;
    edge_fwd_body<NW, BF, DROP>(S, G, P, (int)blockIdx.x, (int)gridDim.x, Pn, Qn, x, aggr_msg, x_new);
}
static int edge_saved_check(const EqdEdgeParams* p, const char* who) {
    const int n = (p->xh_save != nullptr) + (p->rstd_save != nullptr) + (p->zpos_save != nullptr);
    if (n != 0 && n != 3) {
        eqd_set_error("%s: xh_save, rstd_save and zpos_save must all be given or all be NULL", who);
        return EQD_ERR_NULL;
    }
    return EQD_OK;
}
static int edge_drop_mode(const EqdEdgeParams* p, const char* who) {
    if ((p->drop_z1 == nullptr) != (p->drop_ch == nullptr) || (p->drop_z1 && !(p->drop_scale > 0.f))) {
        eqd_set_error("%s: dropout needs both masks (drop_z1, drop_ch) and drop_scale > 0", who);
        return -1;
    }
    return p->drop_z1 ? 1 : 0;
}

union alignas(16) EdgeAttnFwdSmem {
    EdgeFwdSmem<FWD_WAVES, false> edge;
    AttnFwdSmem<4> att[2];
    __device__ EdgeAttnFwdSmem() {}
};
template <bool DROP>
__global__ __launch_bounds__(64 * FWD_WAVES) void k_edge_attn_fwd(EqdGraph G, EqdEdgeParams P, int n_edge,
                                                                   const float* __restrict__ Pn,
                                                                   const float* __restrict__ Qn,
                                                                   const float* __restrict__ x,
                                                                   float* __restrict__ aggr_msg,
                                                                   float* __restrict__ x_new,
                                                                   const float* __restrict__ q,
                                                                   const float* __restrict__ k,
                                                                   const float* __restrict__ v,
                                                                   float* __restrict__ att_out,
                                                                   float* __restrict__ lse) {
    __shared__ EdgeAttnFwdSmem S;
    if ((int)blockIdx.x < n_edge) {
        edge_fwd_body<FWD_WAVES, false, DROP>(S.edge, G, P, (int)blockIdx.x, n_edge, Pn, Qn, x, aggr_msg, x_new);
    } else {
        const int half = (int)threadIdx.x >> 8;
        attn_fwd_body<4, true, 1>(S.att[half], G, (int)blockIdx.x - n_edge, half, (int)threadIdx.x & 255, 64, q, k, v,
                                  att_out, lse, true);
    }
}

union alignas(16) EdgeAttnFwdSmem80 {
    EdgeFwdSmem<FWD_WAVES, false> edge;
    AttnFwdSmem<5> att;
    __device__ EdgeAttnFwdSmem80() {}
};
template <bool DROP>
__global__ __launch_bounds__(64 * FWD_WAVES) void k_edge_attn_fwd80(EqdGraph G, EqdEdgeParams P, int n_edge,
                                                                     const float* __restrict__ Pn,
                                                                     const float* __restrict__ Qn,
                                                                     const float* __restrict__ x,
                                                                     float* __restrict__ aggr_msg,
                                                                     float* __restrict__ x_new,
                                                                     const float* __restrict__ q,
                                                                     const float* __restrict__ k,
                                                                     const float* __restrict__ v,
                                                                     float* __restrict__ att_out,
                                                                     float* __restrict__ lse) {
    __shared__ EdgeAttnFwdSmem80 S;
    if ((int)blockIdx.x < n_edge) {
        edge_fwd_body<FWD_WAVES, false, DROP>(S.edge, G, P, (int)blockIdx.x, n_edge, Pn, Qn, x, aggr_msg, x_new);
    } else {
        if (threadIdx.x >= 256) return;
        attn_fwd_body<5, true, 2>(S.att, G, (int)blockIdx.x - n_edge, 0, (int)threadIdx.x, 80, q, k, v, att_out, lse, false);
    }
}

#include "eqd_edge_fwd_half_inl.h"

static int edge_grid(int n_tiles, int waves, int wg_per_cu) {
    if (n_tiles <= 0) return 1;
    const int cus = eqd_num_cus();
    const int slots = cus * waves * wg_per_cu;
    const int rounds = (n_tiles + slots - 1) / slots;
    int blocks = (n_tiles + waves * rounds - 1) / (waves * rounds);
    if (blocks > cus * wg_per_cu) blocks = cus * wg_per_cu;
    return blocks < 1 ? 1 : blocks;
}

extern "C" int eqd_edge_message_fwd(const EqdGraph* g, const EqdEdgeParams* p, const float* P, const float* Q,
                                    const float* x, float* aggr_msg, float* x_new, void* stream) {
    if (!g || !p || !P || !Q || !x || !aggr_msg || !x_new) {
        eqd_set_error("eqd_edge_message_fwd: NULL argument");
        return EQD_ERR_NULL;
    }
    if (g->n_tiles <= 0) return EQD_OK;
    const int blocks = edge_grid(g->n_tiles, FWD_WAVES, 1);
    const int drop = edge_drop_mode(p, "eqd_edge_message_fwd");
    if (drop < 0) return EQD_ERR_NULL;
    if (int rc = edge_saved_check(p, "eqd_edge_message_fwd")) return rc;
    if (p->bf16 && p->use_he && !g->he_bf16) {
        eqd_set_error("eqd_edge_message_fwd: bf16 mode needs EqdGraph.he_bf16");
        return EQD_ERR_NULL;
    }
#define EQD_EDGE_FWD_LAUNCH(BF_, DROP_)                                                                                   \
    hipLaunchKernelGGL(HIP_KERNEL_NAME(k_edge_fwd<FWD_WAVES, BF_, DROP_>), dim3(blocks), dim3(64 * FWD_WAVES), 0,         \
                       (hipStream_t)stream, *g, *p, P, Q, x, aggr_msg, x_new)
    if (p->bf16) {
        if (drop) EQD_EDGE_FWD_LAUNCH(true, true); else EQD_EDGE_FWD_LAUNCH(true, false);
    } else {
        if (drop) EQD_EDGE_FWD_LAUNCH(false, true); else EQD_EDGE_FWD_LAUNCH(false, false);
    }
#undef EQD_EDGE_FWD_LAUNCH
    return eqd_check_launch("k_edge_fwd");
}

static std::atomic<long long> g_edge_fwd_half_launches{0};
extern "C" long long eqd_edge_fwd_half_launches(void) { return g_edge_fwd_half_launches.load(); }

int eqd_edge_attn_fused(const EqdGraph* g, const EqdEdgeParams* p, int d_att, const float* q, const float* k, const float* v) {
    if (!eqd_switch_on("EQD_FUSE_FWD")) return 0;
    if (p->bf16 || (d_att != 64 && d_att != 80) || g->n_tiles <= 0 || g->n_att_items <= 0) return 0;
    if (d_att == 80 && !eqd_switch_on("EQD_FUSE_FWD80")) return 0;
    if ((((uintptr_t)q | (uintptr_t)k | (uintptr_t)v) & 15) != 0) return 0;
    const int n_edge = edge_grid(g->n_tiles, FWD_WAVES, 1);
    return n_edge + g->n_att_items <= eqd_num_cus();
}
int eqd_edge_attn_fwd(const EqdGraph* g, const EqdEdgeParams* p, const float* P, const float* Q, const float* x,
                      float* aggr_msg, float* x_new, int d_att, const float* q, const float* k, const float* v,
                      float* att_out, float* lse, hipStream_t st) {
    if (!eqd_edge_attn_fused(g, p, d_att, q, k, v)) {
        int rc = eqd_cross_attention_fwd(g, d_att, q, k, v, att_out, lse, st);
        if (rc) return rc;
        return eqd_edge_message_fwd(g, p, P, Q, x, aggr_msg, x_new, st);
    }
    const int n_edge = edge_grid(g->n_tiles, FWD_WAVES, 1);
    const int drop = edge_drop_mode(p, "eqd_edge_attn_fwd");
    if (drop < 0) return EQD_ERR_NULL;
    if (int rc = edge_saved_check(p, "eqd_edge_attn_fwd")) return rc;
    if (d_att == 80) {
        if (drop)
            hipLaunchKernelGGL(k_edge_attn_fwd80<true>, dim3(n_edge + g->n_att_items), dim3(64 * FWD_WAVES), 0, st, *g, *p, n_edge,
                               P, Q, x, aggr_msg, x_new, q, k, v, att_out, lse);
        else
            hipLaunchKernelGGL(k_edge_attn_fwd80<false>, dim3(n_edge + g->n_att_items), dim3(64 * FWD_WAVES), 0, st, *g, *p, n_edge,
                               P, Q, x, aggr_msg, x_new, q, k, v, att_out, lse);
        return eqd_check_launch("k_edge_attn_fwd");
    }
    if (eqd_switch_on("EQD_EDGE_FWD_HALF") && g->n_tiles <= FWD_WAVES * n_edge) {
        if (drop)
            hipLaunchKernelGGL(k_edge_attn_fwd_half<true>, dim3(n_edge + g->n_att_items), dim3(64 * EDGE_HALF_WAVES), 0, st, *g, *p,
                               n_edge, P, Q, x, aggr_msg, x_new, q, k, v, att_out, lse);
        else
            hipLaunchKernelGGL(k_edge_attn_fwd_half<false>, dim3(n_edge + g->n_att_items), dim3(64 * EDGE_HALF_WAVES), 0, st, *g, *p,
                               n_edge, P, Q, x, aggr_msg, x_new, q, k, v, att_out, lse);
        ++g_edge_fwd_half_launches;
        return eqd_check_launch("k_edge_attn_fwd");
    }
    if (drop)
        hipLaunchKernelGGL(k_edge_attn_fwd<true>, dim3(n_edge + g->n_att_items), dim3(64 * FWD_WAVES), 0, st, *g, *p, n_edge, P,
                           Q, x, aggr_msg, x_new, q, k, v, att_out, lse);
    else
        hipLaunchKernelGGL(k_edge_attn_fwd<false>, dim3(n_edge + g->n_att_items), dim3(64 * FWD_WAVES), 0, st, *g, *p, n_edge, P,
                           Q, x, aggr_msg, x_new, q, k, v, att_out, lse);
    return eqd_check_launch("k_edge_attn_fwd");
}

extern "C" int eqd_selftest_edge_attn_fwd(const EqdGraph* g, const EqdEdgeParams* p, const float* P, const float* Q,
                                          const float* x, float* aggr_msg, float* x_new, int d_att, const float* q,
                                          const float* k, const float* v, float* att_out, float* lse, void* stream) {
    if (!g || !p || !P || !Q || !x || !aggr_msg || !x_new || !q || !k || !v || !att_out || !lse) {
        eqd_set_error("eqd_selftest_edge_attn_fwd: NULL argument");
        return EQD_ERR_NULL;
    }
    return eqd_edge_attn_fwd(g, p, P, Q, x, aggr_msg, x_new, d_att, q, k, v, att_out, lse, (hipStream_t)stream);
}

#define VP 384
#define V_DLNG 0
#define V_DLNB 64
#define V_DWC2 128
#define V_DBC2 192
#define V_DB2 256
#define V_DBC1 320
#define VA 384
#define WP_W2 0
#define WP_WC1 4096
#define WP_W1 8192
#define WP_N 11264

struct EdgeBwdWs {
    float* dz1;
    float* dxrel;
    float* vecp;
    float* wpart;
};

#define UST 132
__device__ __forceinline__ void slab_store(float* __restrict__ slab, int wave, const f32x4 (&v)[4][1], int l15, int g) {
#pragma unroll
    for (int mb = 0; mb < 4; ++mb)
#pragma unroll
        for (int r = 0; r < 4; ++r) slab[(16 * mb + 4 * g + r) * UST + 16 * wave + l15] = v[mb][0][r];
}
template <int NJ>
__device__ __forceinline__ void slab_atb(f32x4 (&acc)[NJ], const float* __restrict__ Xt, const float* __restrict__ Yt,
                                         int mb, int nb0, int l15, int g) {
#pragma unroll 2
    for (int kc = 0; kc < 8; ++kc) {
        const f32x4 a = *(const f32x4*)&Xt[(16 * mb + l15) * UST + 16 * kc + 4 * g];
        f32x4 b[NJ];
#pragma unroll
        for (int j = 0; j < NJ; ++j) b[j] = *(const f32x4*)&Yt[(16 * (nb0 + j) + l15) * UST + 16 * kc + 4 * g];
#pragma unroll
        for (int u = 0; u < 4; ++u)
#pragma unroll
            for (int j = 0; j < NJ; ++j) acc[j] = mfma4(a[u], b[j][u], acc[j]);
    }
}

__device__ __forceinline__ void feat_atb(f32x4 (&acc)[1], const float* __restrict__ Xt, const float* __restrict__ tiles,
                                         int mb, int nb, int l15, int g) {
    const int c = 16 * nb + l15;
    const bool ok = c < FS;
    const int cc = ok ? c : 0;
#pragma unroll 2
    for (int kc = 0; kc < 8; ++kc) {
        const f32x4 a = *(const f32x4*)&Xt[(16 * mb + l15) * UST + 16 * kc + 4 * g];
        float b[4];
#pragma unroll
        for (int u = 0; u < 4; ++u) b[u] = tiles[kc * (16 * FS) + (4 * g + u) * FS + cc];
#pragma unroll
        for (int u = 0; u < 4; ++u) acc[0] = mfma4(a[u], ok ? b[u] : 0.f, acc[0]);
    }
}

#define USB 72
__device__ __forceinline__ void slab_store_bf(unsigned short* __restrict__ slab, int wave, const f32x4 (&v)[4][1], int l15,
                                              int g) {
#pragma unroll
    for (int mb = 0; mb < 4; ++mb)
        *(s16x4*)&slab[(16 * wave + l15) * USB + 16 * mb + 4 * g] = pack_bf4(v[mb][0][0], v[mb][0][1], v[mb][0][2], v[mb][0][3]);
}
template <int NJ, bool FULL>
__device__ __forceinline__ void slab_atb_bf(f32x4 (&acc)[NJ], const unsigned short* __restrict__ Xr,
                                            const unsigned short* __restrict__ Yr, int mb, int nb0, int l15, int g) {
    const int lo = (4 * g + (l15 >> 2)) * USB + 4 * (l15 & 3);
    const unsigned short* const px = Xr + lo + 16 * mb;
    auto chunk = [&](int kp) {
        const s16x8 a = cat_bf(lds_tr16(px + 32 * kp * USB), lds_tr16(px + (32 * kp + 16) * USB));
#pragma unroll
        for (int j = 0; j < NJ; ++j) {
            const unsigned short* const py = Yr + lo + 16 * (nb0 + j);
            acc[j] = mfma_bf32(a, cat_bf(lds_tr16(py + 32 * kp * USB), lds_tr16(py + (32 * kp + 16) * USB)), acc[j]);
        }
    };
    if constexpr (FULL) {
#pragma unroll
        for (int kp = 0; kp < 4; ++kp) chunk(kp);
    } else {
#pragma unroll 2
        for (int kp = 0; kp < 4; ++kp) chunk(kp);
    }
}

template <bool BF>
struct EdgeBwdSmemSel {
    typedef EdgeSmem<BWD_WAVES, 16 * FS> type;
    typedef float slab_t;
    enum { SLAB = 64 * UST };
};
template <>
struct EdgeBwdSmemSel<true> {
    typedef EdgeSmemBfBwd<BWD_WAVES, 16 * FS> type;
    typedef unsigned short slab_t;
    enum { SLAB = 128 * USB };
};

template <bool BF, bool DROP = false, bool SAVED = false>
__global__ __launch_bounds__(64 * BWD_WAVES) void k_edge_bwd(EqdGraph G, EqdEdgeParams P, const float* __restrict__ Pn,
                                                              const float* __restrict__ Qn,
                                                              const float* __restrict__ x,
                                                              const float* __restrict__ d_aggr,
                                                              const float* __restrict__ d_xnew, EdgeBwdWs W) {
    typedef EdgeBwdSmemSel<BF> Sel;
    __shared__ typename Sel::type sm;
    constexpr bool DBUF = BF;
#ifdef EQD_EXP_NO_SLABS
    constexpr bool NOSLAB = true;
#else
    constexpr bool NOSLAB = false;
#endif
    __shared__ __attribute__((aligned(16))) typename Sel::slab_t Ubuf[(DBUF ? 2 : 1) * Sel::SLAB];
    __shared__ __attribute__((aligned(16))) typename Sel::slab_t Vbuf[(DBUF ? 2 : 1) * Sel::SLAB];
    int slab_par = 0;
    EQD_TR_WG();
    EQD_TR(0);
    const int lane = threadIdx.x & 63, wave = threadIdx.x >> 6;
    const int l15 = lane & 15, g = lane >> 4;
    const int n_tiles = (G.n_edges + 15) >> 4;
    const int n_super = (n_tiles + BWD_WAVES - 1) / BWD_WAVES;
    int nx_src = 0, nx_dst = 0;
    auto endpoints = [&](int it_) {
        int e0 = 16 * (it_ * BWD_WAVES + wave), ne = G.n_edges - e0;
        ne = ne < 0 ? 0 : (ne > 16 ? 16 : ne);
        if (ne == 0) e0 = 0;
        const int ei = e0 + (l15 < ne ? l15 : 0);
        nx_src = G.src[ei];
        nx_dst = G.dst[ei];
    };
    if ((int)blockIdx.x < n_super) endpoints((int)blockIdx.x);
    if constexpr (BF)
        edge_stage_weights_bf<BWD_WAVES, true>(sm, P);
    else
        edge_stage_weights(sm, P);
    EQD_TR(1);
    float* tile = sm.tile[wave];
    float r_dlng = 0.f, r_dlnb = 0.f, r_dwc2 = 0.f, r_dbc1 = 0.f, r_db2 = 0.f, r_dbc2 = 0.f;
    const int wmb = wave >> 1, wnb = 2 * (wave & 1);
    f32x4 gW2[2] = {f4zero(), f4zero()}, gWc1[2] = {f4zero(), f4zero()}, gW1a[1] = {f4zero()}, gW1b[1] = {f4zero()};
    for (int it = blockIdx.x; it < n_super; it += gridDim.x) {
        const int t = it * BWD_WAVES + wave;
        EdgeTileState<1> S;
        S.n0 = S.n1 = 0;
        S.e0 = 16 * t;
        S.ne = G.n_edges - S.e0;
        S.ne = S.ne < 0 ? 0 : (S.ne > 16 ? 16 : S.ne);
        if (S.ne == 0) S.e0 = 0;
        S.src[0] = nx_src;
        S.dst[0] = nx_dst;
        if (it + (int)gridDim.x < n_super) endpoints(it + (int)gridDim.x);
        f32x4 xh[4][1], m[4][1], ch[4][1];
        float4 dag[4];
        float gxn[3];
        int r0, r1;
        {
            const int d = S.dst[0];
            r0 = G.rowptr[d];
            r1 = G.rowptr[d + 1];
#pragma unroll
            for (int c = 0; c < 3; ++c) gxn[c] = d_xnew[(size_t)d * 3 + c];
#pragma unroll
            for (int mb = 0; mb < 4; ++mb) dag[mb] = *(const float4*)&d_aggr[(size_t)d * 64 + 16 * mb + 4 * g];
        }
        if constexpr (BF)
            edge_tile_forward_bf<1, DROP, true, SAVED>(G, P, sm.w1, sm.w2, sm.wc1, sm.vec, tile, Pn, Qn, x, lane, S, xh, m, ch);
        else
            edge_tile_forward<1, DROP, true, SAVED>(G, P, sm.w1, sm.w2, sm.wc1, sm.vec, tile, Pn, Qn, x, lane, S, xh, m, ch, nullptr);
        float invdeg = 0.f, dcoef = 0.f, dxr[3] = {0.f, 0.f, 0.f};
        {
            invdeg = S.ev[0] ? 1.f / (float)(r1 - r0) : 0.f;
#pragma unroll
            for (int c = 0; c < 3; ++c) {
                const float gx = gxn[c] * invdeg;
                dcoef += gx * S.xrel[0][c];
                dxr[c] = gx * S.coef[0];
            }
        }
        {
            float va[16], vb[16];
#pragma unroll
            for (int mb = 0; mb < 4; ++mb) {
                const float4 w = *(const float4*)&sm.vec[VEC_WC2 + 16 * mb + 4 * g];
                const float wv[4] = {w.x, w.y, w.z, w.w};
#pragma unroll
                for (int r = 0; r < 4; ++r) {
                    const float c = ch[mb][0][r];
                    float keep = 1.f;
                    if constexpr (DROP) keep = ((S.keepc >> (4 * mb + r)) & 1u) ? P.drop_scale : 0.f;
                    const float dch = wv[r] * dcoef * (lrelu_grad(c, P.slope) * keep);
                    va[4 * mb + r] = (lrelu(c, P.slope) * keep) * dcoef;
                    vb[4 * mb + r] = dch;
                    ch[mb][0][r] = dch;
                }
            }
            r_dwc2 += reduce16x16(va, l15);
            r_dbc1 += reduce16x16(vb, l15);
            r_dbc2 += g == 0 ? dcoef : 0.f;
        }
        EQD_TR(12);
        typename Sel::slab_t* U = Ubuf + slab_par * Sel::SLAB;
        typename Sel::slab_t* V = Vbuf + slab_par * Sel::SLAB;
        if constexpr (DBUF) slab_par ^= 1;
        if constexpr (!NOSLAB) {
        if constexpr (BF) {
            slab_store_bf(U, wave, ch, l15, g);
            slab_store_bf(V, wave, m, l15, g);
        } else {
            slab_store(U, wave, ch, l15, g);
            slab_store(V, wave, m, l15, g);
        }
        __syncthreads();
        EQD_TR(13);
        if constexpr (BF)
            slab_atb_bf<2, !DROP>(gWc1, U, V, wmb, wnb, l15, g);
        else
            slab_atb<2>(gWc1, U, V, wmb, wnb, l15, g);
        }
        EQD_TR(14);
#pragma unroll
        for (int mb = 0; mb < 4; ++mb) {
            const float4 v = dag[mb];
            f32x4 a;
            a[0] = v.x * invdeg; a[1] = v.y * invdeg; a[2] = v.z * invdeg; a[3] = v.w * invdeg;
            m[mb][0] = a;
        }
        if constexpr (BF)
            chain64_bf<false, 1>(m, ch, sm.wc1T, nullptr, nullptr, l15, g);
        else
            chain64T<1>(m, ch, sm.wc1, l15, g);
        {
            float va[16];
#pragma unroll
            for (int mb = 0; mb < 4; ++mb)
#pragma unroll
                for (int r = 0; r < 4; ++r) va[4 * mb + r] = m[mb][0][r];
            r_db2 += reduce16x16(va, l15);
        }
        EQD_TR(15);
        if constexpr (!DBUF && !NOSLAB) __syncthreads();
        U = Ubuf + slab_par * Sel::SLAB;
        V = Vbuf + slab_par * Sel::SLAB;
        if constexpr (DBUF) slab_par ^= 1;
        if constexpr (!NOSLAB) {
        if constexpr (BF)
            slab_store_bf(U, wave, m, l15, g);
        else
            slab_store(U, wave, m, l15, g);
        }
        if constexpr (!NOSLAB) {
            f32x4 a1[4][1];
#pragma unroll
            for (int mb = 0; mb < 4; ++mb) {
                const float4 gg = *(const float4*)&sm.vec[VEC_LNG + 16 * mb + 4 * g];
                const float4 bb = *(const float4*)&sm.vec[VEC_LNB + 16 * mb + 4 * g];
                a1[mb][0][0] = xh[mb][0][0] * gg.x + bb.x;
                a1[mb][0][1] = xh[mb][0][1] * gg.y + bb.y;
                a1[mb][0][2] = xh[mb][0][2] * gg.z + bb.z;
                a1[mb][0][3] = xh[mb][0][3] * gg.w + bb.w;
            }
            if constexpr (BF)
                slab_store_bf(V, wave, a1, l15, g);
            else
                slab_store(V, wave, a1, l15, g);
        }
        if constexpr (!NOSLAB) {
        __syncthreads();
        EQD_TR(16);
        if constexpr (BF)
            slab_atb_bf<2, !DROP>(gW2, U, V, wmb, wnb, l15, g);
        else
            slab_atb<2>(gW2, U, V, wmb, wnb, l15, g);
        }
        EQD_TR(17);
        f32x4 dz[4][1];
#pragma unroll
        for (int mb = 0; mb < 4; ++mb) dz[mb][0] = f4zero();
        if constexpr (BF)
            chain64_bf<false, 1>(dz, m, sm.w2T, nullptr, nullptr, l15, g);
        else
            chain64T<1>(dz, m, sm.w2, l15, g);
        EQD_TR(18);
        {
            float va[16], vb[16];
#pragma unroll
            for (int mb = 0; mb < 4; ++mb)
#pragma unroll
                for (int r = 0; r < 4; ++r) {
                    va[4 * mb + r] = dz[mb][0][r] * xh[mb][0][r];
                    vb[4 * mb + r] = dz[mb][0][r];
                }
            r_dlng += reduce16x16(va, l15);
            r_dlnb += reduce16x16(vb, l15);
        }
        {
            float s1 = 0.f, s2 = 0.f;
#pragma unroll
            for (int mb = 0; mb < 4; ++mb) {
                const float4 gg = *(const float4*)&sm.vec[VEC_LNG + 16 * mb + 4 * g];
                const float gv[4] = {gg.x, gg.y, gg.z, gg.w};
#pragma unroll
                for (int r = 0; r < 4; ++r) {
                    const float dxh = dz[mb][0][r] * gv[r];
                    dz[mb][0][r] = dxh;
                    s1 += dxh;
                    s2 += dxh * xh[mb][0][r];
                }
            }
            s1 = group_sum(s1) * (1.f / 64.f);
            s2 = group_sum(s2) * (1.f / 64.f);
#pragma unroll
            for (int mb = 0; mb < 4; ++mb)
#pragma unroll
                for (int r = 0; r < 4; ++r) {
                    const float xhv = xh[mb][0][r];
                    float lg = ((S.zpos >> (4 * mb + r)) & 1u) ? 1.f : P.slope;
                    if constexpr (DROP) lg *= ((S.keepz >> (4 * mb + r)) & 1u) ? P.drop_scale : 0.f;
                    const float v = S.ev[0] ? S.rstd[0] * (dz[mb][0][r] - s1 - xhv * s2) * lg : 0.f;
                    dz[mb][0][r] = v;
                }
        }
        EQD_TR(19);
        if constexpr (BF) {
            if (S.ev[0]) {
                unsigned short* row = (unsigned short*)W.dz1 + (size_t)(S.e0 + l15) * 64;
#pragma unroll
                for (int mb = 0; mb < 4; ++mb)
                    *(s16x4*)&row[16 * mb + 4 * g] = pack_bf4(dz[mb][0][0], dz[mb][0][1], dz[mb][0][2], dz[mb][0][3]);
            }
        } else {
            hbm_store<1>(W.dz1, dz, S, l15, g);
        }
        if constexpr (!DBUF && !NOSLAB) __syncthreads();
        U = Ubuf + slab_par * Sel::SLAB;
        V = Vbuf + slab_par * Sel::SLAB;
        if constexpr (DBUF) slab_par ^= 1;
        if constexpr (NOSLAB) {
        } else if constexpr (BF) {
            slab_store_bf(U, wave, dz, l15, g);
            const unsigned short* __restrict__ ft = (const unsigned short*)tile;
#pragma unroll
            for (int i = 0; i < 3; ++i)
                *(s16x4*)&V[(16 * wave + l15) * USB + 12 * g + 4 * i] = *(const s16x4*)&ft[l15 * FSB + 12 * g + 4 * i];
            __syncthreads();
            slab_atb_bf<1, !DROP>(gW1a, U, V, wmb, wave & 1, l15, g);
            if (wave < 4) slab_atb_bf<1, !DROP>(gW1b, U, V, wave, 2, l15, g);
        } else {
            slab_store(U, wave, dz, l15, g);
            __syncthreads();
            feat_atb(gW1a, U, &sm.tile[0][0], wmb, wave & 1, l15, g);
            if (wave < 4) feat_atb(gW1b, U, &sm.tile[0][0], wave, 2, l15, g);
        }
        EQD_TR(20);
        if (P.use_dist) {
            f32x4 dr = f4zero();
            if constexpr (BF) {
#pragma unroll
                for (int mp = 0; mp < 2; ++mp)
                    dr = mfma_bf32(cat_bf(*(const s16x4*)&sm.w1rT[l15 * WSB + 32 * mp + 4 * g],
                                          *(const s16x4*)&sm.w1rT[l15 * WSB + 32 * mp + 16 + 4 * g]),
                                   cat_bf(pack_bf4(dz[2 * mp][0][0], dz[2 * mp][0][1], dz[2 * mp][0][2], dz[2 * mp][0][3]),
                                          pack_bf4(dz[2 * mp + 1][0][0], dz[2 * mp + 1][0][1], dz[2 * mp + 1][0][2],
                                                   dz[2 * mp + 1][0][3])), dr);
            } else {
#pragma unroll
                for (int mbi = 0; mbi < 4; ++mbi)
#pragma unroll
                    for (int r = 0; r < 4; ++r) {
                        const float w = (l15 < 15) ? sm.w1[(16 * mbi + 4 * g + r) * WS1 + 27 + l15] : 0.f;
                        dr = mfma4(w, dz[mbi][0][r], dr);
                    }
            }
            float s = 0.f;
#pragma unroll
            for (int r = 0; r < 4; ++r) {
                const int k = 4 * g + r;
                if (k < 15) {
                    float e;
                    if constexpr (BF) e = S.rbf[0][r];
                    else e = S.ev[0] ? tile[l15 * FS + 27 + k] : 1.f;
                    s += dr[r] * e * rbf_neg_inv_sigma(k);
                }
            }
            const float dd2 = group_sum(s);
#pragma unroll
            for (int c = 0; c < 3; ++c) dxr[c] += 2.f * S.xrel[0][c] * dd2;
        }
        if (g == 0 && S.ev[0]) {
            float* o = W.dxrel + (size_t)(S.e0 + l15) * 4;
            o[0] = dxr[0]; o[1] = dxr[1]; o[2] = dxr[2]; o[3] = 0.f;
        }
        if constexpr (!DBUF && !NOSLAB) __syncthreads();
        EQD_TR(21);
    }
    {
        if constexpr (DBUF) __syncthreads();
        float* const U = (float*)Ubuf;
        float* vs = U + wave * VP;
        const int fo = 16 * (l15 >> 2) + 4 * g + (l15 & 3);
        vs[V_DLNG + fo] = r_dlng;
        vs[V_DLNB + fo] = r_dlnb;
        vs[V_DWC2 + fo] = r_dwc2;
        vs[V_DB2 + fo] = r_db2;
        vs[V_DBC1 + fo] = r_dbc1;
        const float t = wave_sum(r_dbc2);
        if (lane == 0) vs[V_DBC2] = t;
        __syncthreads();
        float* vp = W.vecp + (size_t)blockIdx.x * VP;
        for (int i = threadIdx.x; i < VP; i += 64 * BWD_WAVES) {
            float a = 0.f;
#pragma unroll
            for (int w = 0; w < BWD_WAVES; ++w) a += ((const float*)U)[w * VP + i];
            vp[i] = a;
        }
    }
    if (!W.wpart) return;
    float* wp = W.wpart + (size_t)blockIdx.x * WP_N;
#pragma unroll
    for (int j = 0; j < 2; ++j)
#pragma unroll
        for (int r = 0; r < 4; ++r) {
            const int row = 16 * wmb + 4 * g + r, col = 16 * (wnb + j) + l15;
            wp[WP_W2 + row * 64 + col] = gW2[j][r];
            wp[WP_WC1 + row * 64 + col] = gWc1[j][r];
        }
#pragma unroll
    for (int r = 0; r < 4; ++r) {
        wp[WP_W1 + (16 * wmb + 4 * g + r) * 48 + 16 * (wave & 1) + l15] = gW1a[0][r];
        if (wave < 4) wp[WP_W1 + (16 * wave + 4 * g + r) * 48 + 32 + l15] = gW1b[0][r];
    }
    EQD_TR(22);
    EQD_TR_WG_END();
}

template <bool BF, bool DROP>
__global__ __launch_bounds__(64 * BWD_WAVES) void k_edge_signs(EqdGraph G, EqdEdgeParams P, const float* __restrict__ Pn,
                                                                const float* __restrict__ Qn,
                                                                const float* __restrict__ x,
                                                                unsigned char* __restrict__ z1_pos,
                                                                unsigned char* __restrict__ ch_pos) {
    __shared__ typename EdgeSmemSel<BWD_WAVES, 16 * FS, BF>::type sm;
    if constexpr (BF)
        edge_stage_weights_bf<BWD_WAVES, false>(sm, P);
    else
        edge_stage_weights(sm, P);
    const int lane = threadIdx.x & 63, wave = threadIdx.x >> 6;
    const int l15 = lane & 15, g = lane >> 4;
    float* tile = sm.tile[wave];
    const int n_tiles = (G.n_edges + 15) >> 4;
    for (int t = blockIdx.x * BWD_WAVES + wave; t < n_tiles; t += gridDim.x * BWD_WAVES) {
        EdgeTileState<1> S;
        S.n0 = S.n1 = 0;
        S.e0 = 16 * t;
        S.ne = G.n_edges - S.e0;
        S.ne = S.ne > 16 ? 16 : S.ne;
        f32x4 xh[4][1], m[4][1], ch[4][1];
        if constexpr (BF)
            edge_tile_forward_bf<1, DROP>(G, P, sm.w1, sm.w2, sm.wc1, sm.vec, tile, Pn, Qn, x, lane, S, xh, m, ch);
        else
            edge_tile_forward<1, DROP>(G, P, sm.w1, sm.w2, sm.wc1, sm.vec, tile, Pn, Qn, x, lane, S, xh, m, ch, nullptr);
        if (S.ev[0]) {
            const size_t row = (size_t)(S.e0 + l15) * 64;
#pragma unroll
            for (int mb = 0; mb < 4; ++mb)
#pragma unroll
                for (int r = 0; r < 4; ++r) {
                    z1_pos[row + 16 * mb + 4 * g + r] = (unsigned char)((S.zpos >> (4 * mb + r)) & 1u);
                    ch_pos[row + 16 * mb + 4 * g + r] = ch[mb][0][r] > 0.f ? 1 : 0;
                }
        }
        wave_lds_fence();
    }
}

int eqd_launch_edge_signs(const EqdGraph* g, const EqdEdgeParams* p, const float* P, const float* Q, const float* x,
                          unsigned char* z1_pos, unsigned char* ch_pos, hipStream_t st) {
    if (g->n_edges <= 0) return EQD_OK;
    const int n_tiles = (g->n_edges + 15) / 16;
    int blocks = (n_tiles + BWD_WAVES - 1) / BWD_WAVES;
    if (blocks > eqd_num_cus()) blocks = eqd_num_cus();
#define EQD_EDGE_SIGNS_LAUNCH(BF_, DROP_)                                                                                 \
    hipLaunchKernelGGL(HIP_KERNEL_NAME(k_edge_signs<BF_, DROP_>), dim3(blocks), dim3(64 * BWD_WAVES), 0, st, *g, *p, P, Q, x, \
                       z1_pos, ch_pos)
    if (p->bf16) {
        if (p->drop_z1) EQD_EDGE_SIGNS_LAUNCH(true, true); else EQD_EDGE_SIGNS_LAUNCH(true, false);
    } else {
        if (p->drop_z1) EQD_EDGE_SIGNS_LAUNCH(false, true); else EQD_EDGE_SIGNS_LAUNCH(false, false);
    }
#undef EQD_EDGE_SIGNS_LAUNCH
    return eqd_check_launch("k_edge_signs");
}

static int edge_bwd_blocks(const EqdGraph* g) {
    const int n_tiles = (g->n_edges + 15) / 16;
    int n_super = (n_tiles + BWD_WAVES - 1) / BWD_WAVES;
    if (n_super < 1) n_super = 1;
    const int cus = eqd_num_cus();
    return n_super < cus ? n_super : cus;
}
size_t eqd_edge_bwd_vecp_floats(const EqdGraph* g) {
    return (size_t)edge_bwd_blocks(g) * (BWD_WAVES * VP + WP_N);
}

static size_t edge_bwd_carve(const EqdGraph* g, EqdArena& A, EdgeBwdWs* W) {
    const size_t E = (size_t)g->n_edges;
    EdgeBwdWs w;
    w.dz1 = A.take<float>(E * 64);
    w.dxrel = A.take<float>(E * 4);
    w.vecp = A.take<float>(eqd_edge_bwd_vecp_floats(g));
    w.wpart = w.vecp ? w.vecp + (size_t)edge_bwd_blocks(g) * BWD_WAVES * VP : nullptr;
    if (W) *W = w;
    return A.off;
}

extern "C" size_t eqd_edge_message_bwd_workspace_bytes(const EqdGraph* g) {
    EqdArena A(nullptr, 0);
    return edge_bwd_carve(g, A, nullptr) + 256;
}

extern "C" int eqd_edge_message_bwd_kernel_only(const EqdGraph* g, const EqdEdgeParams* p, const float* P,
                                                const float* Q, const float* x, const float* d_aggr_msg,
                                                const float* d_xnew, float* dQ, float* dx, void* workspace,
                                                size_t ws_bytes, void* stream) {
    (void)dQ;
    (void)dx;
    if (!g || !p || !P || !Q || !x || !d_aggr_msg || !d_xnew) {
        eqd_set_error("eqd_edge_message_bwd_kernel_only: NULL argument");
        return EQD_ERR_NULL;
    }
    EqdArena A(workspace, ws_bytes);
    EdgeBwdWs W;
    edge_bwd_carve(g, A, &W);
    if (!A.ok) {
        eqd_set_error("eqd_edge_message_bwd_kernel_only: workspace too small");
        return EQD_ERR_WORKSPACE;
    }
    if (g->n_edges <= 0) return EQD_OK;
    if (const char* ko = eqd_tunable("EQD_EXP_EDGE_NO_PARTIALS"))
        if (ko[0] == '1' && ko[1] == 0) W.wpart = nullptr;
    if (int rc = edge_saved_check(p, "eqd_edge_message_bwd_kernel_only")) return rc;
    const bool sv = p->xh_save != nullptr;
#define EQD_EDGE_BWD_KO(BF_, SV_)                                                                                       \
    hipLaunchKernelGGL(HIP_KERNEL_NAME(k_edge_bwd<BF_, false, SV_>), dim3(edge_bwd_blocks(g)), dim3(64 * BWD_WAVES), 0, \
                       (hipStream_t)stream, *g, *p, P, Q, x, d_aggr_msg, d_xnew, W)
    if (p->bf16) {
        if (sv) EQD_EDGE_BWD_KO(true, true); else EQD_EDGE_BWD_KO(true, false);
    } else {
        if (sv) EQD_EDGE_BWD_KO(false, true); else EQD_EDGE_BWD_KO(false, false);
    }
#undef EQD_EDGE_BWD_KO
    return eqd_check_launch("k_edge_bwd");
}

extern "C" int eqd_edge_message_bwd(const EqdGraph* g, const EqdEdgeParams* p, const float* P, const float* Q,
                                    const float* x, const float* d_aggr_msg, const float* d_xnew, float* dP,
                                    float* dQ, float* dx, const EqdEdgeGrads* grads, void* workspace,
                                    size_t ws_bytes, void* stream) {
    return eqd_edge_message_bwd_impl(g, p, P, Q, x, d_aggr_msg, d_xnew, dP, dQ, dx, grads, workspace, ws_bytes,
                                     (hipStream_t)stream, nullptr, nullptr, nullptr);
}

int eqd_edge_message_bwd_impl(const EqdGraph* g, const EqdEdgeParams* p, const float* P, const float* Q, const float* x,
                              const float* d_aggr_msg, const float* d_xnew, float* dP, float* dQ, float* dx,
                              const EqdEdgeGrads* grads, void* workspace, size_t ws_bytes, hipStream_t st,
                              float* part_override, EqdRedList* defer, EqdGatherCall* hold_gather) {
    if (!g || !p || !P || !Q || !x || !d_aggr_msg || !d_xnew || !dP || !dQ || !dx || !grads) {
        eqd_set_error("eqd_edge_message_bwd: NULL argument");
        return EQD_ERR_NULL;
    }
    EqdArena A(workspace, ws_bytes);
    EdgeBwdWs W;
    edge_bwd_carve(g, A, &W);
    if (!A.ok) {
        eqd_set_error("eqd_edge_message_bwd: workspace too small (%zu needed, %zu given)", A.off, ws_bytes);
        return EQD_ERR_WORKSPACE;
    }
    const int blocks = edge_bwd_blocks(g);
    if (part_override) {
        W.vecp = part_override;
        W.wpart = part_override + (size_t)blocks * BWD_WAVES * VP;
    }
    if (g->n_edges > 0) {
        const int drop = edge_drop_mode(p, "eqd_edge_message_bwd");
        if (drop < 0) return EQD_ERR_NULL;
        if (p->bf16 && p->use_he && !g->he_bf16) {
            eqd_set_error("eqd_edge_message_bwd: bf16 mode needs EqdGraph.he_bf16");
            return EQD_ERR_NULL;
        }
        if (int rcs = edge_saved_check(p, "eqd_edge_message_bwd")) return rcs;
        const bool sv = p->xh_save != nullptr;
#define EQD_EDGE_BWD_LAUNCH(BF_, DROP_, SV_)                                                                               \
    hipLaunchKernelGGL(HIP_KERNEL_NAME(k_edge_bwd<BF_, DROP_, SV_>), dim3(blocks), dim3(64 * BWD_WAVES), 0, st, *g, *p, P, Q, \
                       x, d_aggr_msg, d_xnew, W)
#define EQD_EDGE_BWD_LAUNCH2(BF_, DROP_) do { if (sv) EQD_EDGE_BWD_LAUNCH(BF_, DROP_, true); else EQD_EDGE_BWD_LAUNCH(BF_, DROP_, false); } while (0)
        if (p->bf16) {
            if (drop) EQD_EDGE_BWD_LAUNCH2(true, true); else EQD_EDGE_BWD_LAUNCH2(true, false);
        } else {
            if (drop) EQD_EDGE_BWD_LAUNCH2(false, true); else EQD_EDGE_BWD_LAUNCH2(false, false);
        }
#undef EQD_EDGE_BWD_LAUNCH2
#undef EQD_EDGE_BWD_LAUNCH
        int rc = eqd_check_launch("k_edge_bwd");
        if (rc) return rc;
        const int nw = blocks;
        const int koff = 2 * p->d_in;
        EqdRedSeg segs[9] = {
            {W.vecp + V_DLNG, nw, VP, 64, grads->dln_g, 0, 0, 0}, {W.vecp + V_DLNB, nw, VP, 64, grads->dln_b, 0, 0, 0},
            {W.vecp + V_DWC2, nw, VP, 64, grads->dwc2, 0, 0, 0},  {W.vecp + V_DBC2, nw, VP, 1, grads->dbc2, 0, 0, 0},
            {W.vecp + V_DB2, nw, VP, 64, grads->db2, 0, 0, 0},    {W.vecp + V_DBC1, nw, VP, 64, grads->dbc1, 0, 0, 0},
            {W.wpart + WP_W2, blocks, WP_N, 4096, grads->dW2, 0, 0, 0},
            {W.wpart + WP_WC1, blocks, WP_N, 4096, grads->dWc1, 0, 0, 0},
            {W.wpart + WP_W1, blocks, WP_N, 64 * 48, grads->dW1 + koff, 48, 42, grads->ldw1}};
        if (defer && defer->n + 9 <= 512) {
            for (int i = 0; i < 9; ++i) defer->seg[defer->n++] = segs[i];
        } else if ((rc = eqd_launch_reduce_segments(segs, 9, st))) {
            return rc;
        }
    }
    if (hold_gather) {
        *hold_gather = EqdGatherCall{W.dz1, W.dxrel, d_xnew, 1.f - p->eta, dP, dQ, dx, p->bf16 != 0 ? 1 : 0};
        return EQD_OK;
    }
    return eqd_launch_node_gather(g, W.dz1, W.dxrel, d_xnew, 1.f - p->eta, dP, dQ, dx, st, defer, p->bf16 != 0);
}
```

include/equidock_hip.h:

```cpp
#ifndef EQUIDOCK_HIP_H
#define EQUIDOCK_HIP_H

#include <stddef.h>
#include <stdint.h>

#ifdef __cplusplus
extern "C" {
#endif

#define EQD_ABI_VERSION 9
#define EQD_TILE_EDGES 32
#define EQD_ATT_BLOCK 32
#define EQD_MAX_SRC 6
#define EQD_PARAMS_PER_LAYER 19
#define EQD_GLOBAL_PARAMS 5

enum {
    EQD_OK = 0,
    EQD_ERR_NULL = 1,
    EQD_ERR_SHAPE = 2,
    EQD_ERR_UNSUPPORTED = 3,
    EQD_ERR_WORKSPACE = 4,
    EQD_ERR_LAUNCH = 5
};

int eqd_abi_version(void);
const char* eqd_last_error(void);
int eqd_tile_edges(void);
int eqd_is_simulator(void);
void eqd_tunables_reload(void);
long long eqd_chain_resident_launches(void);
long long eqd_chain_resident_bwd_launches(void);
typedef struct EqdNodeChainBwdTest {
    int32_t rows, with_dh, d0;
    float skip_weight_h, slope, ln_eps;
    const float* dh_X[6];
    const float* dh_W[6];
    int32_t dh_wcs[6];
    const float* dH_above;
    float* dH;
    const float* Wn2;
    const float* Wn1;
    const float* y_act;
    const float* ln_g;
    const float* drop_mul;
    float* dz;
    float* ln_part;
    float* d_aggr_msg;
    float* d_aggr_cross;
    float* dh0acc;
} EqdNodeChainBwdTest;
int eqd_selftest_node_chain_bwd(const EqdNodeChainBwdTest* t, int* partial_rows , void* stream);
long long eqd_chain_resident_proj_launches(void);
long long eqd_chain_resident_wide_launches(void);
long long eqd_chain_resident_wide_bwd_launches(void);
typedef struct EqdNodeChainBwdWideTest {
    int32_t rows;
    float skip_weight_h, slope, ln_eps;
    const float* dh_X[6];
    const float* dh_W[6];
    int32_t dh_wcs[6];
    const float* dH_above;
    float* dH;
    const float* Wn2;
    const float* Wn1;
    const float* y_act;
    const float* ln_g;
    const float* drop_mul;
    float* dz;
    float* ln_part;
    float* d_aggr_msg;
    float* d_aggr_cross;
    float* dh0acc;
} EqdNodeChainBwdWideTest;
int eqd_selftest_node_chain_bwd_wide(const EqdNodeChainBwdWideTest* t, int* partial_rows , void* stream);
typedef struct EqdNodeChainFwdTest {
    int32_t rows, d0, form;
    float skip_weight_h, slope, ln_eps;
    const float* h; const float* aggr_msg; const float* aggr_cross; const float* h0;
    const float* Wn1; const float* Bn1; const float* ln_g; const float* ln_b; const float* Wn2; const float* Bn2;
    const float* drop_mul;
    float* a1n; float* y_act; float* h_out;
    const float* W1; const float* B1; const float* WQ; const float* WK; const float* WV;
    float* P; float* Q; float* qa; float* ka; float* va;
    const float* WM; const float* BM; const float* head_mul ; float* hm;
} EqdNodeChainFwdTest;
int eqd_selftest_node_chain_fwd(const EqdNodeChainFwdTest* t, void* stream);
int eqd_selftest_lane_exchanges(const float* in256, int* mismatch, float* out256, void* stream);

int eqd_profile_begin(void* stream, int max_launches);
int eqd_profile_end(void);
int eqd_profile_mark(const char* label);
const char* eqd_profile_name(int i);
float eqd_profile_us(int i);

typedef struct EqdGraph {
    int32_t n_pairs, n_lig, n_rec, n_nodes, n_edges, n_tiles, n_att_items, max_seg;
    const int32_t* seg_off;
    const int32_t* src;
    const int32_t* dst;
    const int32_t* rowptr;
    const int32_t* csc_ptr;
    const int32_t* csc_eid;
    const int32_t* tile_node;
    const int32_t* att_items;
    const int32_t* res_id;
    const float* mu_r_norm;
    const float* he;
    const float* x0;
    const uint16_t* he_bf16;
} EqdGraph;

typedef struct EqdModelDesc {
    int32_t n_layers;
    int32_t d_emb;
    int32_t d_hid;
    int32_t use_mean_node_features;
    int32_t edge_feats;
    int32_t n_heads;
    int32_t cross_msgs, use_dist_in_layers, use_edge_features;
    float skip_weight_h, x_connection_init, lrelu_slope, ln_eps;
    int32_t svd_seed;
    int32_t storage_bf16;
} EqdModelDesc;

typedef struct EqdDropout {
    float p;
    const uint32_t* edge_z1;
    const uint32_t* edge_ch;
    const float* node;
    const float* head;
} EqdDropout;

int eqd_dropout_draw(const EqdModelDesc* m, const EqdGraph* g, float p, const uint64_t* seed, uint32_t* edge_z1,
                     uint32_t* edge_ch, float* node, float* head, void* stream);

int eqd_dropout_pack_edges(int n_edges, int e_ll, const float* factors_ll, const float* factors_rr,
                           const int64_t* perm, uint32_t* words, void* stream);


int eqd_ctx_create(void** ctx);
int eqd_ctx_destroy(void* ctx);

size_t eqd_model_saved_bytes(const EqdModelDesc* m, const EqdGraph* g);
size_t eqd_model_scratch_bytes(const EqdModelDesc* m, const EqdGraph* g);
int eqd_model_saved_layout(const EqdModelDesc* m, const EqdGraph* g);
int eqd_model_check(const EqdModelDesc* m, const EqdGraph* g);

int eqd_model_layer_state(const EqdModelDesc* m, const EqdGraph* g, const void* saved, size_t saved_bytes, int layer,
                          const float** h, int* h_width, const float** x);

int eqd_model_node_state(const EqdModelDesc* m, const EqdGraph* g, const void* saved, size_t saved_bytes, int layer,
                         const float** out , int* d_in, int* d_att);

int eqd_model_lrelu_signs(const EqdModelDesc* m, const EqdGraph* g, const float* const* params, const EqdDropout* drop,
                          const void* saved, size_t saved_bytes, int layer, unsigned char* edge_z1, unsigned char* edge_ch,
                          unsigned char* node, unsigned char* q, unsigned char* k, void* stream);

int eqd_model_forward(const EqdModelDesc* m, const EqdGraph* g, const float* const* params, const EqdDropout* drop,
                      const float* svd_draws,
                      float* lig_out, float* Y_lig, float* Y_rec, float* T, float* b, int32_t* svd_status,
                      void* saved, size_t saved_bytes, void* scratch, size_t scratch_bytes, void* stream, void* ctx);

int eqd_model_backward(const EqdModelDesc* m, const EqdGraph* g, const float* const* params, const EqdDropout* drop,
                       const float* d_lig, const float* d_Ylig, const float* d_Yrec, const float* d_T,
                       const float* d_b, const float* d_h_last, const float* d_x_last,
                       float* grad_flat, const int64_t* grad_offsets,
                       const void* saved, size_t saved_bytes, void* scratch, size_t scratch_bytes, void* stream,
                       void* ctx);

int eqd_model_head_backward(const EqdModelDesc* m, const EqdGraph* g, const float* const* params, const EqdDropout* drop,
                            const float* d_lig, const float* d_Ylig, const float* d_Yrec, const float* d_T,
                            const float* d_b, float* grad_flat, const int64_t* grad_offsets,
                            const void* saved, size_t saved_bytes, void* scratch, size_t scratch_bytes,
                            float* d_h_L, float* d_x_L, void* stream);


typedef struct EqdLinSrc {
    const float* X;
    const float* mask;
    const float* W;
    int32_t ldx, K, w_rs, w_cs;
} EqdLinSrc;
typedef struct EqdLinJob {
    EqdLinSrc s[EQD_MAX_SRC];
    int32_t nsrc, M, act, rows;
    const float* bias;
    const float* ln_g; const float* ln_b; float* pre_ln; int32_t ld_pre;
    const float* R; int32_t ldr;
    float alpha, beta, slope, ln_eps;
    float* Y; int32_t ldy;
    int32_t bf16;
    const float* mul; int32_t ld_mul;
    int32_t pad_to;
    uint16_t* Yb; int32_t ldyb;
} EqdLinJob;
int eqd_linear(const EqdLinJob* jobs , int njobs, void* stream);

typedef struct EqdAtbJob {
    const float* X; const float* xmask; int32_t ldx, M;
    const float* Y; int32_t ldy, N;
    int32_t rows;
    float* out; int32_t o_rs, o_cs;
    float* bias_out;
    float slope;
    float scale;
    int32_t bf16;
    int32_t y_bf16;
} EqdAtbJob;
size_t eqd_atb_partial_bytes(const EqdAtbJob* jobs , int njobs);
int eqd_atb(const EqdAtbJob* jobs , int njobs, void* partial, size_t partial_bytes, void* stream);

typedef struct EqdEdgeParams {
    const float* W1; int32_t ldw1;
    int32_t d_in;
    const float* ln_g; const float* ln_b;
    const float* W2; const float* b2;
    const float* Wc1; const float* bc1; const float* wc2; const float* bc2;
    float slope, ln_eps, eta;
    int32_t use_dist, use_he;
    int32_t bf16;
    const uint32_t* drop_z1; const uint32_t* drop_ch; float drop_scale;
    uint16_t* aggr_bf16;
    float* xh_save; float* rstd_save; uint16_t* zpos_save;
} EqdEdgeParams;
int eqd_edge_message_fwd(const EqdGraph* g, const EqdEdgeParams* p, const float* P, const float* Q,
                         const float* x, float* aggr_msg, float* x_new, void* stream);
long long eqd_edge_fwd_half_launches(void);
int eqd_selftest_edge_attn_fwd(const EqdGraph* g, const EqdEdgeParams* p, const float* P, const float* Q, const float* x,
                               float* aggr_msg, float* x_new, int d_att, const float* q, const float* k, const float* v,
                               float* att_out, float* lse, void* stream);
typedef struct EqdEdgeGrads {
    float* dW1; int32_t ldw1;
    float* db1_unused;
    float* dln_g; float* dln_b; float* dW2; float* db2; float* dWc1; float* dbc1; float* dwc2; float* dbc2;
} EqdEdgeGrads;
size_t eqd_edge_message_bwd_workspace_bytes(const EqdGraph* g);
int eqd_edge_message_bwd(const EqdGraph* g, const EqdEdgeParams* p, const float* P, const float* Q,
                         const float* x, const float* d_aggr_msg, const float* d_xnew,
                         float* dP, float* dQ, float* dx, const EqdEdgeGrads* grads,
                         void* workspace, size_t ws_bytes, void* stream);

int eqd_edge_message_bwd_kernel_only(const EqdGraph* g, const EqdEdgeParams* p, const float* P, const float* Q,
                                     const float* x, const float* d_aggr_msg, const float* d_xnew,
                                     float* dQ, float* dx, void* workspace, size_t ws_bytes, void* stream);

int eqd_cross_attention_fwd(const EqdGraph* g, int d, const float* q, const float* k, const float* v,
                            float* out, float* lse, void* stream);
int eqd_cross_attention_bwd(const EqdGraph* g, int d, const float* q, const float* k, const float* v,
                            const float* out, const float* lse, const float* d_out,
                            float* dq, float* dk, float* dv, float* delta , void* stream);
size_t eqd_cross_attention_bwd_ds_workspace_bytes(const EqdGraph* g);
int eqd_cross_attention_bwd_ds(const EqdGraph* g, int d, const float* q, const float* k, const float* v,
                               const float* out, const float* lse, const float* d_out,
                               float* dq, float* dk, float* dv, void* ws, size_t ws_bytes, void* stream);

int eqd_cross_attention_fwd_bf16(const EqdGraph* g, int d, const float* q, const float* k, const float* v,
                                 float* out, float* lse, void* stream);
int eqd_cross_attention_bwd_bf16(const EqdGraph* g, int d, const float* q, const float* k, const float* v,
                                 const float* out, const float* lse, const float* d_out,
                                 float* dq, float* dk, float* dv, float* delta, void* stream);

typedef struct EqdNodeUpdateParams {
    int32_t d_in;
    int32_t d0;
    int32_t d_out;
    int32_t ld_cross;
    const float* Wn1;
    const float* bn1;
    const float* ln_g; const float* ln_b;
    const float* Wn2;
    const float* bn2;
    float skip_weight_h, slope, ln_eps;
    int32_t bf16;
    const float* drop_mul;
} EqdNodeUpdateParams;
typedef struct EqdNodeUpdateGrads {
    float* dWn1; float* dbn1; float* dln_g; float* dln_b; float* dWn2; float* dbn2;
} EqdNodeUpdateGrads;
int eqd_node_update_fwd(int rows, const EqdNodeUpdateParams* p, const float* h, const float* aggr_msg,
                        const float* aggr_cross, const float* h0, float* h_out, float* y_act, float* a1n, void* stream);
size_t eqd_node_update_bwd_workspace_bytes(int rows, const EqdNodeUpdateParams* p);
int eqd_node_update_bwd(int rows, const EqdNodeUpdateParams* p, const float* h, const float* aggr_msg,
                        const float* aggr_cross, const float* h0, const float* y_act, const float* a1n,
                        const float* d_h_out, float* d_h, float* d_aggr_msg, float* d_aggr_cross, float* d_h0,
                        const EqdNodeUpdateGrads* grads, void* workspace, size_t ws_bytes, void* stream);

int eqd_keypoint_pool_fwd(const EqdGraph* g, int n_heads, const float* Wk, const float* Wq, const float* qmean,
                          const float* H, const float* Z, float* Y, float* scores, float* lse,
                          float* qp, float* u, void* stream);

size_t eqd_keypoint_pool_bwd_workspace_bytes(const EqdGraph* g, int n_heads);
int eqd_keypoint_pool_bwd(const EqdGraph* g, int n_heads, const float* Wk, const float* Wq, const float* qmean,
                          const float* qp, const float* u, const float* H, const float* Z, const float* scores,
                          const float* lse, const float* dY, float* dH, float* dZ, float* dWk, float* dWq, float* d_hm,
                          void* workspace, size_t ws_bytes, void* stream);

int eqd_kabsch_fwd(int n_pairs, int n_heads, const float* Y, const float* svd_draws, int svd_seed,
                   float* T, float* b, float* A_out, int32_t* status, void* stream);
int eqd_kabsch_bwd(int n_pairs, int n_heads, const float* Y, const float* A, const float* T,
                   const float* dT, const float* db, float* dY, void* stream);

int eqd_rigid_apply_fwd(const EqdGraph* g, const float* T, const float* b, float* lig_out, void* stream);
int eqd_rigid_apply_bwd(const EqdGraph* g, const float* d_lig, float* dT, float* db, void* stream);

int eqd_pair_losses_fwd(const EqdGraph* g, const float* lig_pred, const float* lig_target, const float* rec,
                        float sigma, float surface_ct, float* mse, float* inter, float* s_lig, float* s_rec,
                        void* stream);
int eqd_pair_losses_bwd(const EqdGraph* g, const float* lig_pred, const float* lig_target, const float* rec,
                        float sigma, float surface_ct, const float* s_lig, const float* s_rec, const float* d_mse,
                        const float* d_inter, float* d_lig_pred, void* stream);

int eqd_rigid_augment(const EqdGraph* g, const float* x_lig, const float* R, const float* t, float* new_x,
                      const int32_t* pocket_off, const float* pocket_in, float* pocket_out, void* stream);

int eqd_protein_graph_distances(int n, const float* atoms, const int32_t* atom_off, double* D, void* stream);
int eqd_protein_graph_select(int n, int max_neighbor, double cutoff, const double* D, const double* x, int32_t* nbr,
                             double* nbr_dist, int32_t* deg, float* mu_r_norm, void* stream);
int eqd_protein_graph_edges(int n, int max_neighbor, const int32_t* edge_off, const int32_t* nbr, const double* nbr_dist,
                            const double* x, const double* n_i, const double* u_i, const double* v_i, int32_t* src,
                            int32_t* dst, float* he, void* stream);

typedef struct EqdClashState {
    float euler[3];
    float trans[3];
    float loss;
    int32_t it;
    int32_t done;
    int32_t reserved;
} EqdClashState;
size_t eqd_clash_workspace_bytes(int n_lig, int n_rec);
int eqd_clash_iterations(int n_iter, int n_lig, int n_rec, const float* lig0, const float* rec, float sigma, float surface_ct,
                         float loss_stop, int max_it, EqdClashState* state, void* workspace, size_t ws_bytes, void* stream);

int eqd_pocket_ot_cost(int n_pairs, int n_heads, const int32_t* pocket_off, const float* pocket_lig,
                       const float* pocket_rec, const float* Y_lig, const float* Y_rec, float* cost, void* stream);
int eqd_pocket_ot_fwd(int n_pairs, int n_heads, const int32_t* pocket_off, const float* plan, const float* cost,
                      float* ot, void* stream);
int eqd_pocket_ot_bwd(int n_pairs, int n_heads, const int32_t* pocket_off, const float* pocket_lig,
                      const float* pocket_rec, const float* Y_lig, const float* Y_rec, const float* plan,
                      const float* d_ot, float* dY_lig, float* dY_rec, void* stream);

int eqd_scalar_loss(const EqdGraph* g, int n_heads, const float* lig, const float* Y_lig, const float* Y_rec,
                    float* d_lig, float* d_Ylig, float* d_Yrec, float* pair_loss, float* loss, int32_t* counter,
                    void* stream);

#ifdef __cplusplus
}
#endif
#endif
```

Baseline: 8801 pairs/s.

## Stage edge weights via direct global-to-LDS DMA overlapped with first tile loads

Adds a DMA path for the edge-message kernels (forward half-tile and backward). Weights are staged into LDS with global_load_lds_dword instead of register round-trips. Each tile's gathers (he, endpoint coords, P/Q rows, dropout words) are split into a load phase issued before the weight staging barrier and a compute phase after it. In the backward kernel the next tile's loads are also prefetched at the end of each iteration. This is meant to hide weight-staging and gather latency, at the cost of more live registers, which could lower occupancy. The path is gated by edge_dma_on().

```diff
diff --git a/equidock_public_amd/_lib.py b/equidock_public_amd/_lib.py
--- a/equidock_public_amd/_lib.py
+++ b/equidock_public_amd/_lib.py
@@ -138,7 +138,7 @@
            'eqd_tunables_reload', 'eqd_node_update_fwd', 'eqd_node_update_bwd_workspace_bytes', 'eqd_node_update_bwd',
            'eqd_selftest_lane_exchanges', 'eqd_chain_resident_proj_launches', 'eqd_selftest_node_chain_fwd', 'eqd_model_node_state',
            'eqd_chain_resident_wide_launches', 'eqd_chain_resident_wide_bwd_launches', 'eqd_selftest_node_chain_bwd_wide',
-           'eqd_edge_fwd_half_launches', 'eqd_selftest_edge_attn_fwd')
+           'eqd_edge_fwd_half_launches', 'eqd_selftest_edge_attn_fwd', 'eqd_edge_dma_launches')
 
 
 def load_library():
diff --git a/equidock_public_amd/csrc/eqd_common.h b/equidock_public_amd/csrc/eqd_common.h
--- a/equidock_public_amd/csrc/eqd_common.h
+++ b/equidock_public_amd/csrc/eqd_common.h
@@ -90,6 +90,13 @@
 __device__ __forceinline__ void glds16(const float* gsrc, float* lds_base) {
     __builtin_memcpy(lds_base + 4 * (threadIdx.x & 63), gsrc, 16);
 }
+__device__ __forceinline__ void glds4(const float* gsrc, float* lds_base, const float* lo, const float* hi) {
+    if (gsrc < lo || gsrc + 1 > hi) {
+        fprintf(stderr, "glds4: source %p outside [%p, %p)\n", (const void*)gsrc, (const void*)lo, (const void*)hi);
+        abort();
+    }
+    __builtin_memcpy(lds_base + (threadIdx.x & 63), gsrc, 4);
+}
 template <int N>
 __device__ __forceinline__ void vm_wait() { static_assert(N >= 0 && N <= 63, "vmcnt is a 6-bit count"); }
 __device__ __forceinline__ void lds_barrier() { __syncthreads(); }
@@ -101,6 +108,14 @@
     const unsigned dst = (unsigned)__builtin_amdgcn_readfirstlane((int)(unsigned)(uintptr_t)(__attribute__((address_space(3))) void*)lds_base);
     unsigned keep;
     asm volatile("s_mov_b32 %0, m0\n\ts_mov_b32 m0, %2\n\ts_nop 0\n\tglobal_load_lds_dwordx4 %1, off\n\ts_mov_b32 m0, %0"
+                 : "=&s"(keep)
+                 : "v"(gsrc), "s"(dst)
+                 : "memory");
+}
+__device__ __forceinline__ void glds4(const float* gsrc, float* lds_base, const float*, const float*) {
+    const unsigned dst = (unsigned)__builtin_amdgcn_readfirstlane((int)(unsigned)(uintptr_t)(__attribute__((address_space(3))) void*)lds_base);
+    unsigned keep;
+    asm volatile("s_mov_b32 %0, m0\n\ts_mov_b32 m0, %2\n\ts_nop 0\n\tglobal_load_lds_dword %1, off\n\ts_mov_b32 m0, %0"
                  : "=&s"(keep)
                  : "v"(gsrc), "s"(dst)
                  : "memory");
diff --git a/equidock_public_amd/csrc/eqd_edge_fwd_half_inl.h b/equidock_public_amd/csrc/eqd_edge_fwd_half_inl.h
--- a/equidock_public_amd/csrc/eqd_edge_fwd_half_inl.h
+++ b/equidock_public_amd/csrc/eqd_edge_fwd_half_inl.h
@@ -34,7 +34,7 @@
     }
 }
 
-template <bool DROP>
+template <bool DROP, bool DMA>
 __device__ __forceinline__ void edge_fwd_half_body(EdgeFwdSmem<FWD_WAVES, false>& S_, const EqdGraph& G, const EqdEdgeParams& P,
                                                    int blk, const float* __restrict__ Pn, const float* __restrict__ Qn,
                                                    const float* __restrict__ x, float* __restrict__ aggr_msg,
@@ -56,30 +56,48 @@
         e0 = G.rowptr[n0];
         ne = G.rowptr[n1] - e0;
     }
-    edge_stage_weights<FWD_WAVES, 32 * TS, 64 * EDGE_HALF_WAVES>(sm, P);
+    if constexpr (!DMA) edge_stage_weights<FWD_WAVES, 32 * TS, 64 * EDGE_HALF_WAVES>(sm, P);
     EQD_TR(1);
     const int nn = n1 - n0;
     const size_t xo = (size_t)n0 * 3;
     const int c0 = lane, c1 = lane + 64;
     int rp = 0;
     float x0a = 0.f, xa = 0.f, x0b = 0.f, xb = 0.f;
+    EdgeTileState<1> S;
+    EdgeTileLoads<1> LD;
+    S.ne = 0;
     if (live) {
-        rp = G.rowptr[n0 + (lane <= nn ? lane : 0)] - e0;
+        rp = G.rowptr[n0 + (lane <= nn ? lane : 0)];
         if (h == 0) {
             x0a = G.x0[xo + (c0 < 3 * nn ? c0 : 0)], xa = x[xo + (c0 < 3 * nn ? c0 : 0)];
             x0b = G.x0[xo + (c1 < 3 * nn ? c1 : 0)], xb = x[xo + (c1 < 3 * nn ? c1 : 0)];
         }
-        EdgeTileState<1> S;
         S.n0 = n0;
         S.n1 = n1;
         S.ne = ne - 16 * h;
         S.ne = S.ne < 0 ? 0 : (S.ne > 16 ? 16 : S.ne);
         S.e0 = S.ne > 0 ? e0 + 16 * h : e0;
+        EQD_TR(2);
+        if (S.ne > 0) edge_tile_load<1, false, false, DROP && DMA>(G, P, Pn, Qn, x, lane, S, LD);
+    }
+    if constexpr (DMA) {
+        edge_stage_request<EDGE_HALF_WAVES>(sm, P);
+        edge_stage_publish();
+    }
+    if (live) {
+        if constexpr (DMA) {
+            keep_after_wait(rp);
+            if (h == 0) {
+                keep_after_wait(x0a); keep_after_wait(xa); keep_after_wait(x0b); keep_after_wait(xb);
+            }
+        }
+        rp -= e0;
         const int row = 16 * h + l15;
         if (S.ne > 0) {
             f32x4 xh[4][1], m[4][1], ch[4][1];
-            edge_tile_forward<1, DROP, false>(G, P, sm.w1, sm.w2, sm.wc1, sm.vec, tile + h * EDGE_HALF_FEAT1, Pn, Qn, x, lane, S,
-                                              xh, m, ch, nullptr);
+            if constexpr (DMA) edge_tile_loads_keep<1, false, DROP && DMA>(LD);
+            edge_tile_compute<1, DROP, false, false, DROP && DMA>(G, P, sm.w1, sm.w2, sm.wc1, sm.vec, tile + h * EDGE_HALF_FEAT1, lane, S,
+                                                           LD, xh, m, ch, nullptr);
             wave_lds_fence();
 #pragma unroll
             for (int mb = 0; mb < 4; ++mb)
@@ -113,7 +131,7 @@
     EQD_TR_WG_END();
 }
 
-template <bool DROP>
+template <bool DROP, bool DMA>
 __global__ __launch_bounds__(64 * EDGE_HALF_WAVES) void k_edge_attn_fwd_half(EqdGraph G, EqdEdgeParams P, int n_edge,
                                                                               const float* __restrict__ Pn,
                                                                               const float* __restrict__ Qn,
@@ -127,7 +145,7 @@
                                                                               float* __restrict__ lse) {
     __shared__ EdgeAttnFwdSmem S;
     if ((int)blockIdx.x < n_edge) {
-        edge_fwd_half_body<DROP>(S.edge, G, P, (int)blockIdx.x, Pn, Qn, x, aggr_msg, x_new);
+        edge_fwd_half_body<DROP, DMA>(S.edge, G, P, (int)blockIdx.x, Pn, Qn, x, aggr_msg, x_new);
     } else {
         if (threadIdx.x >= 512) return;
         const int half = (int)threadIdx.x >> 8;
diff --git a/equidock_public_amd/csrc/eqd_edge_kernels.hip b/equidock_public_amd/csrc/eqd_edge_kernels.hip
--- a/equidock_public_amd/csrc/eqd_edge_kernels.hip
+++ b/equidock_public_amd/csrc/eqd_edge_kernels.hip
@@ -90,6 +90,36 @@
     __syncthreads();
 }
 
+template <int NWAVES, int NW, int TF>
+__device__ __forceinline__ void edge_stage_request(EdgeSmem<NW, TF>& sm, const EqdEdgeParams& P) {
+    static_assert(64 % NWAVES == 0 && NWAVES >= 6, "rows are dealt in whole rounds; waves 0 .. 5 take the vectors");
+    const int lane = threadIdx.x & 63, wave = threadIdx.x >> 6;
+    const float* const w1 = P.W1 + 2 * P.d_in;
+    const float* const w1_end = w1 + (size_t)63 * P.ldw1 + 42;
+#pragma unroll
+    for (int j = 0; j < 64 / NWAVES; ++j) {
+        const int r = wave + NWAVES * j;
+        if (lane < 42) glds4(w1 + (size_t)r * P.ldw1 + lane, &sm.w1[r * WS1], P.W1, w1_end);
+        glds4(P.W2 + r * 64 + lane, &sm.w2[r * WS2], P.W2, P.W2 + 4096);
+        glds4(P.Wc1 + r * 64 + lane, &sm.wc1[r * WS2], P.Wc1, P.Wc1 + 4096);
+    }
+    if (wave < 5) {
+        const float* const v = wave == 0 ? P.ln_g : wave == 1 ? P.ln_b : wave == 2 ? P.b2 : wave == 3 ? P.bc1 : P.wc2;
+        glds4(v + lane, &sm.vec[64 * wave], v, v + 64);
+    } else if (wave == 5) {
+        if (lane == 0) glds4(P.bc2, &sm.vec[VEC_BC2], P.bc2, P.bc2 + 1);
+    }
+    if (threadIdx.x < 64) {
+        float* o = &sm.w1[threadIdx.x * WS1 + 42];
+        o[0] = 0.f; o[1] = 0.f; o[2] = 0.f;
+    }
+}
+__device__ __forceinline__ void edge_stage_publish() {
+    vm_wait<0>();
+    lds_barrier();
+}
+static_assert(VEC_LNG == 0 && VEC_LNB == 64 && VEC_B2 == 128 && VEC_BC1 == 192 && VEC_WC2 == 256, "edge_stage_request");
+
 __device__ __forceinline__ float rbf_sigma(int k) {
     const float t[16] = {1.f,          1.5f,         2.25f,        3.375f,        5.0625f,     7.59375f,
                          11.390625f,   17.0859375f,  25.62890625f, 38.443359375f, 57.6650390625f,
@@ -177,12 +207,14 @@
     unsigned keepz, keepc;
 };
 
-__device__ __forceinline__ unsigned drop_bits16(const uint32_t* __restrict__ words, int e, int g) {
-    const uint32_t w0 = words[(size_t)e * 2], w1 = words[(size_t)e * 2 + 1];
+__device__ __forceinline__ unsigned drop_bits16w(uint32_t w0, uint32_t w1, int g) {
     unsigned b = 0u;
 #pragma unroll
     for (int mb = 0; mb < 4; ++mb) b |= (((mb < 2 ? w0 : w1) >> (16 * (mb & 1) + 4 * g)) & 0xfu) << (4 * mb);
     return b;
+}
+__device__ __forceinline__ unsigned drop_bits16(const uint32_t* __restrict__ words, int e, int g) {
+    return drop_bits16w(words[(size_t)e * 2], words[(size_t)e * 2 + 1], g);
 }
 template <int NB>
 __device__ __forceinline__ void drop_load(const EqdEdgeParams& P, EdgeTileState<NB>& S, int l15, int g) {
@@ -211,6 +243,286 @@
         }
 }
 
+template <int NB>
+struct EdgeTileLoads {
+    static constexpr int NH = (16 * NB * 27 / 4 + 63) / 64;
+    f32x4 hv[NH];
+    float xs[NB][3], xd[NB][3];
+    float4 pv[NB][4], qv[NB][4];
+    float rsv[NB];
+    unsigned zsv[NB];
+    uint32_t dz[NB][2], dc[NB][2];
+};
+template <int NB, bool PRE = false, bool SAVED = false, bool DROPPRE = false>
+__device__ __forceinline__ void edge_tile_load(const EqdGraph& G, const EqdEdgeParams& P, const float* __restrict__ Pn,
+                                               const float* __restrict__ Qn, const float* __restrict__ x, int lane,
+                                               EdgeTileState<NB>& S, EdgeTileLoads<NB>& L) {
+    const int l15 = lane & 15, g = lane >> 4;
+    constexpr int NH = EdgeTileLoads<NB>::NH;
+    const float* __restrict__ he = G.he + (size_t)S.e0 * 27;
+    const int nhe = P.use_he ? S.ne * 27 : 0;
+#pragma unroll
+    for (int j = 0; j < NH; ++j) {
+        const int i = 4 * (lane + 64 * j);
+        L.hv[j] = ld4u_raw(he + (i < nhe ? i : 0), nhe - i, G.he);
+    }
+#pragma unroll
+    for (int nb = 0; nb < NB; ++nb) {
+        const int el = 16 * nb + l15;
+        S.ev[nb] = el < S.ne;
+        if constexpr (!PRE) {
+            const int ei = S.e0 + (S.ev[nb] ? el : 0);
+            S.src[nb] = G.src[ei];
+            S.dst[nb] = G.dst[ei];
+        }
+    }
+#pragma unroll
+    for (int nb = 0; nb < NB; ++nb) {
+#pragma unroll
+        for (int c = 0; c < 3; ++c) {
+            L.xs[nb][c] = x[(size_t)S.src[nb] * 3 + c];
+            L.xd[nb][c] = x[(size_t)S.dst[nb] * 3 + c];
+        }
+        if constexpr (SAVED) {
+            const size_t er = (size_t)S.e0 + (S.ev[nb] ? 16 * nb + l15 : 0);
+#pragma unroll
+            for (int mb = 0; mb < 4; ++mb) L.pv[nb][mb] = *(const float4*)&P.xh_save[er * 64 + 16 * mb + 4 * g];
+            L.rsv[nb] = P.rstd_save[er];
+            L.zsv[nb] = P.zpos_save[er * 4 + g];
+        } else {
+#pragma unroll
+            for (int mb = 0; mb < 4; ++mb) {
+                L.pv[nb][mb] = *(const float4*)&Pn[(size_t)S.src[nb] * 64 + 16 * mb + 4 * g];
+                L.qv[nb][mb] = *(const float4*)&Qn[(size_t)S.dst[nb] * 64 + 16 * mb + 4 * g];
+            }
+        }
+        if constexpr (DROPPRE) {
+            const size_t e = (size_t)(S.e0 + ((16 * nb + l15) < S.ne ? 16 * nb + l15 : 0));
+#pragma unroll
+            for (int u = 0; u < 2; ++u) {
+                L.dz[nb][u] = P.drop_z1[e * 2 + u];
+                L.dc[nb][u] = P.drop_ch[e * 2 + u];
+            }
+        }
+    }
+}
+template <int NB, bool SAVED, bool DROPPRE>
+__device__ __forceinline__ void edge_tile_loads_keep(EdgeTileLoads<NB>& L) {
+    auto k4 = [](float4& v) { keep_after_wait(v.x); keep_after_wait(v.y); keep_after_wait(v.z); keep_after_wait(v.w); };
+#pragma unroll
+    for (int j = 0; j < EdgeTileLoads<NB>::NH; ++j) keep_after_wait(L.hv[j]);
+#pragma unroll
+    for (int nb = 0; nb < NB; ++nb) {
+#pragma unroll
+        for (int c = 0; c < 3; ++c) {
+            keep_after_wait(L.xs[nb][c]);
+            keep_after_wait(L.xd[nb][c]);
+        }
+#pragma unroll
+        for (int mb = 0; mb < 4; ++mb) {
+            k4(L.pv[nb][mb]);
+            if constexpr (!SAVED) k4(L.qv[nb][mb]);
+        }
+        if constexpr (SAVED) {
+            keep_after_wait(L.rsv[nb]);
+            keep_after_wait(L.zsv[nb]);
+        }
+        if constexpr (DROPPRE) {
+#pragma unroll
+            for (int u = 0; u < 2; ++u) {
+                keep_after_wait(L.dz[nb][u]);
+                keep_after_wait(L.dc[nb][u]);
+            }
+        }
+    }
+}
+template <int NB, bool DROP = false, bool PRE = false, bool SAVED = false, bool DROPPRE = false>
+__device__ __forceinline__ void edge_tile_compute(const EqdGraph& G, const EqdEdgeParams& P, const float* __restrict__ w1,
+                                                  const float* __restrict__ w2, const float* __restrict__ wc1,
+                                                  const float* __restrict__ vec, float* __restrict__ tile, int lane,
+                                                  EdgeTileState<NB>& S, const EdgeTileLoads<NB>& L, f32x4 (&xh)[4][NB],
+                                                  f32x4 (&m)[4][NB], f32x4 (&ch)[4][NB], float* __restrict__ rbf_out) {
+    static_assert(DROP || !DROPPRE, "dropout words without dropout");
+    const int l15 = lane & 15, g = lane >> 4;
+    constexpr int NH = EdgeTileLoads<NB>::NH;
+    const int nhe = P.use_he ? S.ne * 27 : 0;
+    const f32x4 (&hv)[NH] = L.hv;
+    const float (&xs)[NB][3] = L.xs, (&xd)[NB][3] = L.xd;
+    const float4 (&pv)[NB][4] = L.pv, (&qv)[NB][4] = L.qv;
+    const float (&rsv)[NB] = L.rsv;
+    const unsigned (&zsv)[NB] = L.zsv;
+#pragma unroll
+    for (int nb = 0; nb < NB; ++nb) S.ev[nb] = 16 * nb + l15 < S.ne;
+    for (int i = lane; i < 16 * NB * FS; i += 64) tile[i] = 0.f;
+    wave_lds_fence();
+    EQD_TR(3);
+#pragma unroll
+    for (int j = 0; j < NH; ++j) {
+        const int i = 4 * (lane + 64 * j);
+        const float4 hf = ld4u_fix(hv[j], nhe - i);
+        const float vv[4] = {hf.x, hf.y, hf.z, hf.w};
+        int e = i / 27, c = i - e * 27;
+#pragma unroll
+        for (int u = 0; u < 4; ++u) {
+            if (i + u < nhe) tile[e * FS + c] = vv[u];
+            if (++c == 27) {
+                c = 0;
+                ++e;
+            }
+        }
+    }
+#pragma unroll
+    for (int nb = 0; nb < NB; ++nb) {
+        float q = 0.f;
+#pragma unroll
+        for (int c = 0; c < 3; ++c) {
+            const float v = S.ev[nb] ? xs[nb][c] - xd[nb][c] : 0.f;
+            S.xrel[nb][c] = v;
+            q += v * v;
+        }
+        S.d2[nb] = q;
+    }
+#pragma unroll
+    for (int nb = 0; nb < NB; ++nb) {
+        const int el = 16 * nb + l15;
+#pragma unroll
+        for (int j = 0; j < 4; ++j) {
+            const int k = PRE ? 4 * g + j : g + 4 * j;
+            if (k < 15 && S.ev[nb]) {
+                const float v = P.use_dist ? exp_nooverflow(-S.d2[nb] / rbf_sigma(k)) : 0.f;
+                tile[el * FS + 27 + k] = v;
+                if (rbf_out) rbf_out[(size_t)(S.e0 + el) * 16 + k] = v;
+            }
+        }
+        if (rbf_out && g == 3 && S.ev[nb]) rbf_out[(size_t)(S.e0 + el) * 16 + 15] = 0.f;
+    }
+    wave_lds_fence();
+    EQD_TR(4);
+    S.zpos = 0u;
+    if constexpr (DROPPRE) {
+        S.keepz = S.keepc = 0u;
+#pragma unroll
+        for (int nb = 0; nb < NB; ++nb) {
+            S.keepz |= drop_bits16w(L.dz[nb][0], L.dz[nb][1], g) << (16 * nb);
+            S.keepc |= drop_bits16w(L.dc[nb][0], L.dc[nb][1], g) << (16 * nb);
+        }
+    } else if constexpr (DROP) {
+        drop_load<NB>(P, S, l15, g);
+    }
+    if constexpr (SAVED) {
+#pragma unroll
+        for (int nb = 0; nb < NB; ++nb) {
+#pragma unroll
+            for (int mb = 0; mb < 4; ++mb) {
+                const float4 v = pv[nb][mb];
+                f32x4 a;
+                a[0] = S.ev[nb] ? v.x : 0.f; a[1] = S.ev[nb] ? v.y : 0.f; a[2] = S.ev[nb] ? v.z : 0.f; a[3] = S.ev[nb] ? v.w : 0.f;
+                xh[mb][nb] = a;
+            }
+            S.zpos |= (S.ev[nb] ? zsv[nb] : 0u) << (16 * nb);
+            S.mean[nb] = 0.f;
+            S.rstd[nb] = rsv[nb];
+        }
+    } else {
+#pragma unroll
+    for (int nb = 0; nb < NB; ++nb)
+#pragma unroll
+        for (int mb = 0; mb < 4; ++mb) {
+            const float4 p = pv[nb][mb], q = qv[nb][mb];
+            f32x4 a;
+            a[0] = S.ev[nb] ? p.x + q.x : 0.f; a[1] = S.ev[nb] ? p.y + q.y : 0.f;
+            a[2] = S.ev[nb] ? p.z + q.z : 0.f; a[3] = S.ev[nb] ? p.w + q.w : 0.f;
+            xh[mb][nb] = a;
+        }
+    EQD_TR(5);
+#pragma unroll
+    for (int s = 0; s < 11; ++s) {
+        const int k = 4 * s + g;
+        float b[NB];
+#pragma unroll
+        for (int nb = 0; nb < NB; ++nb) b[nb] = tile[(16 * nb + l15) * FS + k];
+#pragma unroll
+        for (int mb = 0; mb < 4; ++mb) {
+            const float a = w1[(16 * mb + l15) * WS1 + k];
+#pragma unroll
+            for (int nb = 0; nb < NB; ++nb) xh[mb][nb] = mfma4(a, b[nb], xh[mb][nb]);
+        }
+    }
+    EQD_TR(6);
+#pragma unroll
+    for (int nb = 0; nb < NB; ++nb) {
+        float s = 0.f;
+#pragma unroll
+        for (int mb = 0; mb < 4; ++mb)
+#pragma unroll
+            for (int r = 0; r < 4; ++r) {
+                const float z = xh[mb][nb][r];
+                if (z > 0.f) S.zpos |= 1u << (16 * nb + 4 * mb + r);
+                float v = lrelu(z, P.slope);
+                if constexpr (DROP) v *= ((S.keepz >> (16 * nb + 4 * mb + r)) & 1u) ? P.drop_scale : 0.f;
+                xh[mb][nb][r] = v;
+                s += v;
+            }
+        const float mean = group_sum(s) * (1.f / 64.f);
+        float q = 0.f;
+#pragma unroll
+        for (int mb = 0; mb < 4; ++mb)
+#pragma unroll
+            for (int r = 0; r < 4; ++r) {
+                const float d = xh[mb][nb][r] - mean;
+                q += d * d;
+            }
+        const float rstd = 1.f / sqrtf(group_sum(q) * (1.f / 64.f) + P.ln_eps);
+#pragma unroll
+        for (int mb = 0; mb < 4; ++mb)
+#pragma unroll
+            for (int r = 0; r < 4; ++r) xh[mb][nb][r] = (xh[mb][nb][r] - mean) * rstd;
+        S.mean[nb] = mean;
+        S.rstd[nb] = rstd;
+    }
+    }
+    if constexpr (!SAVED) {
+        if (P.xh_save) edge_state_store<NB>(P, S, xh, l15, g);
+    }
+    EQD_TR(7);
+#pragma unroll
+    for (int mb = 0; mb < 4; ++mb) {
+        const float4 b = *(const float4*)&vec[VEC_B2 + 16 * mb + 4 * g];
+        f32x4 v = {b.x, b.y, b.z, b.w};
+#pragma unroll
+        for (int nb = 0; nb < NB; ++nb) m[mb][nb] = v;
+    }
+    chain64<true, NB>(m, xh, w2, &vec[VEC_LNG], &vec[VEC_LNB], l15, g);
+    EQD_TR(8);
+#pragma unroll
+    for (int mb = 0; mb < 4; ++mb) {
+        const float4 b = *(const float4*)&vec[VEC_BC1 + 16 * mb + 4 * g];
+        f32x4 v = {b.x, b.y, b.z, b.w};
+#pragma unroll
+        for (int nb = 0; nb < NB; ++nb) ch[mb][nb] = v;
+    }
+    chain64<false, NB>(ch, m, wc1, nullptr, nullptr, l15, g);
+#pragma unroll
+    for (int nb = 0; nb < NB; ++nb) {
+        float s = 0.f;
+#pragma unroll
+        for (int mb = 0; mb < 4; ++mb) {
+            const float4 w = *(const float4*)&vec[VEC_WC2 + 16 * mb + 4 * g];
+            if constexpr (DROP) {
+                const float wv[4] = {w.x, w.y, w.z, w.w};
+#pragma unroll
+                for (int r = 0; r < 4; ++r)
+                    s += lrelu(ch[mb][nb][r], P.slope) *
+                         (((S.keepc >> (16 * nb + 4 * mb + r)) & 1u) ? P.drop_scale : 0.f) * wv[r];
+            } else {
+                s += lrelu(ch[mb][nb][0], P.slope) * w.x + lrelu(ch[mb][nb][1], P.slope) * w.y +
+                     lrelu(ch[mb][nb][2], P.slope) * w.z + lrelu(ch[mb][nb][3], P.slope) * w.w;
+            }
+        }
+        S.coef[nb] = group_sum(s) + vec[VEC_BC2];
+    }
+    EQD_TR(9);
+}
 template <int NB, bool DROP = false, bool PRE = false, bool SAVED = false>
 __device__ __forceinline__ void edge_tile_forward(const EqdGraph& G, const EqdEdgeParams& P, const float* __restrict__ w1,
                                                   const float* __restrict__ w2, const float* __restrict__ wc1,
@@ -219,212 +531,10 @@
                                                   const float* __restrict__ x, int lane, EdgeTileState<NB>& S,
                                                   f32x4 (&xh)[4][NB], f32x4 (&m)[4][NB], f32x4 (&ch)[4][NB],
                                                   float* __restrict__ rbf_out) {
-    const int l15 = lane & 15, g = lane >> 4;
     EQD_TR(2);
-    constexpr int NH = (16 * NB * 27 / 4 + 63) / 64;
-    const float* __restrict__ he = G.he + (size_t)S.e0 * 27;
-    const int nhe = P.use_he ? S.ne * 27 : 0;
-    f32x4 hv[NH];
-#pragma unroll
-    for (int j = 0; j < NH; ++j) {
-        const int i = 4 * (lane + 64 * j);
-        hv[j] = ld4u_raw(he + (i < nhe ? i : 0), nhe - i, G.he);
-    }
-#pragma unroll
-    for (int nb = 0; nb < NB; ++nb) {
-        const int el = 16 * nb + l15;
-        S.ev[nb] = el < S.ne;
-        if constexpr (!PRE) {
-            const int ei = S.e0 + (S.ev[nb] ? el : 0);
-            S.src[nb] = G.src[ei];
-            S.dst[nb] = G.dst[ei];
-        }
-    }
-    float xs[NB][3], xd[NB][3];
-    float4 pv[NB][4], qv[NB][4];
-    float rsv[NB];
-    unsigned zsv[NB];
-#pragma unroll
-    for (int nb = 0; nb < NB; ++nb) {
-#pragma unroll
-        for (int c = 0; c < 3; ++c) {
-            xs[nb][c] = x[(size_t)S.src[nb] * 3 + c];
-            xd[nb][c] = x[(size_t)S.dst[nb] * 3 + c];
-        }
-        if constexpr (SAVED) {
-            const size_t er = (size_t)S.e0 + (S.ev[nb] ? 16 * nb + l15 : 0);
-#pragma unroll
-            for (int mb = 0; mb < 4; ++mb) pv[nb][mb] = *(const float4*)&P.xh_save[er * 64 + 16 * mb + 4 * g];
-            rsv[nb] = P.rstd_save[er];
-            zsv[nb] = P.zpos_save[er * 4 + g];
-        } else {
-#pragma unroll
-            for (int mb = 0; mb < 4; ++mb) {
-                pv[nb][mb] = *(const float4*)&Pn[(size_t)S.src[nb] * 64 + 16 * mb + 4 * g];
-                qv[nb][mb] = *(const float4*)&Qn[(size_t)S.dst[nb] * 64 + 16 * mb + 4 * g];
-            }
-        }
-    }
-    for (int i = lane; i < 16 * NB * FS; i += 64) tile[i] = 0.f;
-    wave_lds_fence();
-    EQD_TR(3);
-#pragma unroll
-    for (int j = 0; j < NH; ++j) {
-        const int i = 4 * (lane + 64 * j);
-        const float4 hf = ld4u_fix(hv[j], nhe - i);
-        const float vv[4] = {hf.x, hf.y, hf.z, hf.w};
-        int e = i / 27, c = i - e * 27;
-#pragma unroll
-        for (int u = 0; u < 4; ++u) {
-            if (i + u < nhe) tile[e * FS + c] = vv[u];
-            if (++c == 27) {
-                c = 0;
-                ++e;
-            }
-        }
-    }
-#pragma unroll
-    for (int nb = 0; nb < NB; ++nb) {
-        float q = 0.f;
-#pragma unroll
-        for (int c = 0; c < 3; ++c) {
-            const float v = S.ev[nb] ? xs[nb][c] - xd[nb][c] : 0.f;
-            S.xrel[nb][c] = v;
-            q += v * v;
-        }
-        S.d2[nb] = q;
-    }
-#pragma unroll
-    for (int nb = 0; nb < NB; ++nb) {
-        const int el = 16 * nb + l15;
-#pragma unroll
-        for (int j = 0; j < 4; ++j) {
-            const int k = PRE ? 4 * g + j : g + 4 * j;
-            if (k < 15 && S.ev[nb]) {
-                const float v = P.use_dist ? exp_nooverflow(-S.d2[nb] / rbf_sigma(k)) : 0.f;
-                tile[el * FS + 27 + k] = v;
-                if (rbf_out) rbf_out[(size_t)(S.e0 + el) * 16 + k] = v;
-            }
-        }
-        if (rbf_out && g == 3 && S.ev[nb]) rbf_out[(size_t)(S.e0 + el) * 16 + 15] = 0.f;
-    }
-    wave_lds_fence();
-    EQD_TR(4);
-    S.zpos = 0u;
-    if constexpr (DROP) drop_load<NB>(P, S, l15, g);
-    if constexpr (SAVED) {
-#pragma unroll
-        for (int nb = 0; nb < NB; ++nb) {
-#pragma unroll
-            for (int mb = 0; mb < 4; ++mb) {
-                const float4 v = pv[nb][mb];
-                f32x4 a;
-                a[0] = S.ev[nb] ? v.x : 0.f; a[1] = S.ev[nb] ? v.y : 0.f; a[2] = S.ev[nb] ? v.z : 0.f; a[3] = S.ev[nb] ? v.w : 0.f;
-                xh[mb][nb] = a;
-            }
-            S.zpos |= (S.ev[nb] ? zsv[nb] : 0u) << (16 * nb);
-            S.mean[nb] = 0.f;
-            S.rstd[nb] = rsv[nb];
-        }
-    } else {
-#pragma unroll
-    for (int nb = 0; nb < NB; ++nb)
-#pragma unroll
-        for (int mb = 0; mb < 4; ++mb) {
-            const float4 p = pv[nb][mb], q = qv[nb][mb];
-            f32x4 a;
-            a[0] = S.ev[nb] ? p.x + q.x : 0.f; a[1] = S.ev[nb] ? p.y + q.y : 0.f;
-            a[2] = S.ev[nb] ? p.z + q.z : 0.f; a[3] = S.ev[nb] ? p.w + q.w : 0.f;
-            xh[mb][nb] = a;
-        }
-    EQD_TR(5);
-#pragma unroll
-    for (int s = 0; s < 11; ++s) {
-        const int k = 4 * s + g;
-        float b[NB];
-#pragma unroll
-        for (int nb = 0; nb < NB; ++nb) b[nb] = tile[(16 * nb + l15) * FS + k];
-#pragma unroll
-        for (int mb = 0; mb < 4; ++mb) {
-            const float a = w1[(16 * mb + l15) * WS1 + k];
-#pragma unroll
-            for (int nb = 0; nb < NB; ++nb) xh[mb][nb] = mfma4(a, b[nb], xh[mb][nb]);
-        }
-    }
-    EQD_TR(6);
-#pragma unroll
-    for (int nb = 0; nb < NB; ++nb) {
-        float s = 0.f;
-#pragma unroll
-        for (int mb = 0; mb < 4; ++mb)
-#pragma unroll
-            for (int r = 0; r < 4; ++r) {
-                const float z = xh[mb][nb][r];
-                if (z > 0.f) S.zpos |= 1u << (16 * nb + 4 * mb + r);
-                float v = lrelu(z, P.slope);
-                if constexpr (DROP) v *= ((S.keepz >> (16 * nb + 4 * mb + r)) & 1u) ? P.drop_scale : 0.f;
-                xh[mb][nb][r] = v;
-                s += v;
-            }
-        const float mean = group_sum(s) * (1.f / 64.f);
-        float q = 0.f;
-#pragma unroll
-        for (int mb = 0; mb < 4; ++mb)
-#pragma unroll
-            for (int r = 0; r < 4; ++r) {
-                const float d = xh[mb][nb][r] - mean;
-                q += d * d;
-            }
-        const float rstd = 1.f / sqrtf(group_sum(q) * (1.f / 64.f) + P.ln_eps);
-#pragma unroll
-        for (int mb = 0; mb < 4; ++mb)
-#pragma unroll
-            for (int r = 0; r < 4; ++r) xh[mb][nb][r] = (xh[mb][nb][r] - mean) * rstd;
-        S.mean[nb] = mean;
-        S.rstd[nb] = rstd;
-    }
-    }
-    if constexpr (!SAVED) {
-        if (P.xh_save) edge_state_store<NB>(P, S, xh, l15, g);
-    }
-    EQD_TR(7);
-#pragma unroll
-    for (int mb = 0; mb < 4; ++mb) {
-        const float4 b = *(const float4*)&vec[VEC_B2 + 16 * mb + 4 * g];
-        f32x4 v = {b.x, b.y, b.z, b.w};
-#pragma unroll
-        for (int nb = 0; nb < NB; ++nb) m[mb][nb] = v;
-    }
-    chain64<true, NB>(m, xh, w2, &vec[VEC_LNG], &vec[VEC_LNB], l15, g);
-    EQD_TR(8);
-#pragma unroll
-    for (int mb = 0; mb < 4; ++mb) {
-        const float4 b = *(const float4*)&vec[VEC_BC1 + 16 * mb + 4 * g];
-        f32x4 v = {b.x, b.y, b.z, b.w};
-#pragma unroll
-        for (int nb = 0; nb < NB; ++nb) ch[mb][nb] = v;
-    }
-    chain64<false, NB>(ch, m, wc1, nullptr, nullptr, l15, g);
-#pragma unroll
-    for (int nb = 0; nb < NB; ++nb) {
-        float s = 0.f;
-#pragma unroll
-        for (int mb = 0; mb < 4; ++mb) {
-            const float4 w = *(const float4*)&vec[VEC_WC2 + 16 * mb + 4 * g];
-            if constexpr (DROP) {
-                const float wv[4] = {w.x, w.y, w.z, w.w};
-#pragma unroll
-                for (int r = 0; r < 4; ++r)
-                    s += lrelu(ch[mb][nb][r], P.slope) *
-                         (((S.keepc >> (16 * nb + 4 * mb + r)) & 1u) ? P.drop_scale : 0.f) * wv[r];
-            } else {
-                s += lrelu(ch[mb][nb][0], P.slope) * w.x + lrelu(ch[mb][nb][1], P.slope) * w.y +
-                     lrelu(ch[mb][nb][2], P.slope) * w.z + lrelu(ch[mb][nb][3], P.slope) * w.w;
-            }
-        }
-        S.coef[nb] = group_sum(s) + vec[VEC_BC2];
-    }
-    EQD_TR(9);
+    EdgeTileLoads<NB> L;
+    edge_tile_load<NB, PRE, SAVED, false>(G, P, Pn, Qn, x, lane, S, L);
+    edge_tile_compute<NB, DROP, PRE, SAVED, false>(G, P, w1, w2, wc1, vec, tile, lane, S, L, xh, m, ch, rbf_out);
 }
 
 #define WSB 72
@@ -795,7 +905,7 @@
     typename EdgeSmemSel<NW, 32 * TS, BF>::type sm;
     float sxw[NW][96];
 };
-template <int NW, bool BF, bool DROP = false>
+template <int NW, bool BF, bool DROP = false, bool DMA = false>
 __device__ __forceinline__ void edge_fwd_body(EdgeFwdSmem<NW, BF>& S_, const EqdGraph& G, const EqdEdgeParams& P, int blk,
                                               int nblk, const float* __restrict__ Pn, const float* __restrict__ Qn,
                                               const float* __restrict__ x, float* __restrict__ aggr_msg,
@@ -832,13 +942,21 @@
         link_range();
         if constexpr (AHEAD) link_endpoints();
     }
-    if constexpr (BF)
-        edge_stage_weights_bf<NW, false>(sm, P);
-    else
-        edge_stage_weights(sm, P);
-    EQD_TR(1);
-    for (int t = t_first; t < G.n_tiles; t += t_step) {
-        EdgeTileState<2> S;
+    static_assert(!(BF && DMA), "bf16 converts while it stages");
+    EdgeTileState<2> S;
+    EdgeTileLoads<2> LD;
+    int rp_raw = 0;
+    float x0a = 0.f, xa = 0.f, x0b = 0.f, xb = 0.f;
+    const int c0 = lane, c1 = lane + 64;
+    auto node_loads = [&]() {
+        const int nn_pre = S.n1 - S.n0;
+        const size_t xo = (size_t)S.n0 * 3;
+        rp_raw = G.rowptr[S.n0 + (lane <= nn_pre ? lane : 0)];
+        x0a = G.x0[xo + (c0 < 3 * nn_pre ? c0 : 0)], xa = x[xo + (c0 < 3 * nn_pre ? c0 : 0)];
+        x0b = G.x0[xo + (c1 < 3 * nn_pre ? c1 : 0)], xb = x[xo + (c1 < 3 * nn_pre ? c1 : 0)];
+    };
+    bool more = false;
+    auto tile_head = [&](int t) {
         if constexpr (AHEAD) {
             S.n0 = nx_n0;
             S.n1 = nx_n1;
@@ -860,19 +978,30 @@
             S.e0 = G.rowptr[S.n0];
             S.ne = G.rowptr[S.n1] - S.e0;
         }
-        const bool more = AHEAD && t + t_step < G.n_tiles;
+        more = AHEAD && t + t_step < G.n_tiles;
         if (more) link_nodes(t + t_step);
+        node_loads();
+        if constexpr (DMA) {
+            EQD_TR(2);
+            edge_tile_load<2, false, false, DROP>(G, P, Pn, Qn, x, lane, S, LD);
+        }
+    };
+    auto tile_rest = [&](int t, bool first) {
         f32x4 xh[4][2], m[4][2], ch[4][2];
-        const int nn_pre = S.n1 - S.n0;
-        const int rp = G.rowptr[S.n0 + (lane <= nn_pre ? lane : 0)] - S.e0;
         const size_t xo = (size_t)S.n0 * 3;
-        const int c0 = lane, c1 = lane + 64;
-        const float x0a = G.x0[xo + (c0 < 3 * nn_pre ? c0 : 0)], xa = x[xo + (c0 < 3 * nn_pre ? c0 : 0)];
-        const float x0b = G.x0[xo + (c1 < 3 * nn_pre ? c1 : 0)], xb = x[xo + (c1 < 3 * nn_pre ? c1 : 0)];
-        if constexpr (BF)
+        if constexpr (BF) {
             edge_tile_forward_bf<2, DROP, true>(G, P, sm.w1, sm.w2, sm.wc1, sm.vec, tile, Pn, Qn, x, lane, S, xh, m, ch);
-        else
+        } else if constexpr (DMA) {
+            if (first) {
+                keep_after_wait(rp_raw);
+                keep_after_wait(x0a); keep_after_wait(xa); keep_after_wait(x0b); keep_after_wait(xb);
+                edge_tile_loads_keep<2, false, DROP>(LD);
+            }
+            edge_tile_compute<2, DROP, false, false, DROP>(G, P, sm.w1, sm.w2, sm.wc1, sm.vec, tile, lane, S, LD, xh, m, ch, nullptr);
+        } else {
             edge_tile_forward<2, DROP, false>(G, P, sm.w1, sm.w2, sm.wc1, sm.vec, tile, Pn, Qn, x, lane, S, xh, m, ch, nullptr);
+        }
+        const int rp = rp_raw - S.e0;
         if (more) link_range();
         wave_lds_fence();
 #pragma unroll
@@ -932,17 +1061,45 @@
         if (c1 < 3 * nn) x_new[xo + c1] = P.eta * x0b + (1.f - P.eta) * xb + sxw[wave][c1];
         wave_lds_fence();
         EQD_TR(11);
+    };
+    if constexpr (DMA) {
+        int t = t_first;
+        const bool any = t < G.n_tiles;
+        if (any) tile_head(t);
+        edge_stage_request<NW>(sm, P);
+        edge_stage_publish();
+        EQD_TR(1);
+        if (any) {
+            bool first = true;
+            for (;;) {
+                tile_rest(t, first);
+                first = false;
+                t += t_step;
+                if (t >= G.n_tiles) break;
+                tile_head(t);
+            }
+        }
+    } else {
+        if constexpr (BF)
+            edge_stage_weights_bf<NW, false>(sm, P);
+        else
+            edge_stage_weights(sm, P);
+        EQD_TR(1);
+        for (int t = t_first; t < G.n_tiles; t += t_step) {
+            tile_head(t);
+            tile_rest(t, false);
+        }
     }
     EQD_TR_WG_END();
 }
-template <int NW, bool BF, bool DROP = false>
+template <int NW, bool BF, bool DROP = false, bool DMA = false>
 __global__ __launch_bounds__(64 * NW) void k_edge_fwd(EqdGraph G, EqdEdgeParams P, const float* __restrict__ Pn,
                                                               const float* __restrict__ Qn,
                                                               const float* __restrict__ x,
                                                               float* __restrict__ aggr_msg,
                                                               float* __restrict__ x_new) {
     __shared__ EdgeFwdSmem<NW, BF> S;
-    edge_fwd_body<NW, BF, DROP>(S, G, P, (int)blockIdx.x, (int)gridDim.x, Pn, Qn, x, aggr_msg, x_new);
+    edge_fwd_body<NW, BF, DROP, DMA>(S, G, P, (int)blockIdx.x, (int)gridDim.x, Pn, Qn, x, aggr_msg, x_new);
 }
 static int edge_saved_check(const EqdEdgeParams* p, const char* who) {
     const int n = (p->xh_save != nullptr) + (p->rstd_save != nullptr) + (p->zpos_save != nullptr);
@@ -965,7 +1122,7 @@
     AttnFwdSmem<4> att[2];
     __device__ EdgeAttnFwdSmem() {}
 };
-template <bool DROP>
+template <bool DROP, bool DMA>
 __global__ __launch_bounds__(64 * FWD_WAVES) void k_edge_attn_fwd(EqdGraph G, EqdEdgeParams P, int n_edge,
                                                                    const float* __restrict__ Pn,
                                                                    const float* __restrict__ Qn,
@@ -979,7 +1136,7 @@
                                                                    float* __restrict__ lse) {
     __shared__ EdgeAttnFwdSmem S;
     if ((int)blockIdx.x < n_edge) {
-        edge_fwd_body<FWD_WAVES, false, DROP>(S.edge, G, P, (int)blockIdx.x, n_edge, Pn, Qn, x, aggr_msg, x_new);
+        edge_fwd_body<FWD_WAVES, false, DROP, DMA>(S.edge, G, P, (int)blockIdx.x, n_edge, Pn, Qn, x, aggr_msg, x_new);
     } else {
         const int half = (int)threadIdx.x >> 8;
         attn_fwd_body<4, true, 1>(S.att[half], G, (int)blockIdx.x - n_edge, half, (int)threadIdx.x & 255, 64, q, k, v,
@@ -992,7 +1149,7 @@
     AttnFwdSmem<5> att;
     __device__ EdgeAttnFwdSmem80() {}
 };
-template <bool DROP>
+template <bool DROP, bool DMA>
 __global__ __launch_bounds__(64 * FWD_WAVES) void k_edge_attn_fwd80(EqdGraph G, EqdEdgeParams P, int n_edge,
                                                                      const float* __restrict__ Pn,
                                                                      const float* __restrict__ Qn,
@@ -1006,7 +1163,7 @@
                                                                      float* __restrict__ lse) {
     __shared__ EdgeAttnFwdSmem80 S;
     if ((int)blockIdx.x < n_edge) {
-        edge_fwd_body<FWD_WAVES, false, DROP>(S.edge, G, P, (int)blockIdx.x, n_edge, Pn, Qn, x, aggr_msg, x_new);
+        edge_fwd_body<FWD_WAVES, false, DROP, DMA>(S.edge, G, P, (int)blockIdx.x, n_edge, Pn, Qn, x, aggr_msg, x_new);
     } else {
         if (threadIdx.x >= 256) return;
         attn_fwd_body<5, true, 2>(S.att, G, (int)blockIdx.x - n_edge, 0, (int)threadIdx.x, 80, q, k, v, att_out, lse, false);
@@ -1014,6 +1171,13 @@
 }
 
 #include "eqd_edge_fwd_half_inl.h"
+
+static std::atomic<long long> g_edge_dma_launches{0};
+extern "C" long long eqd_edge_dma_launches(void) { return g_edge_dma_launches.load(); }
+static bool edge_dma_on() {
+    const char* f = eqd_tunable("EQD_EDGE_DMA_STAGE");
+    return f && f[0] == '1' && f[1] == 0;
+}
 
 static int edge_grid(int n_tiles, int waves, int wg_per_cu) {
     if (n_tiles <= 0) return 1;
@@ -1040,13 +1204,16 @@
         eqd_set_error("eqd_edge_message_fwd: bf16 mode needs EqdGraph.he_bf16");
         return EQD_ERR_NULL;
     }
-#define EQD_EDGE_FWD_LAUNCH(BF_, DROP_)                                                                                   \
-    hipLaunchKernelGGL(HIP_KERNEL_NAME(k_edge_fwd<FWD_WAVES, BF_, DROP_>), dim3(blocks), dim3(64 * FWD_WAVES), 0,         \
+#define EQD_EDGE_FWD_LAUNCH(BF_, DROP_, DMA_)                                                                             \
+    hipLaunchKernelGGL(HIP_KERNEL_NAME(k_edge_fwd<FWD_WAVES, BF_, DROP_, DMA_>), dim3(blocks), dim3(64 * FWD_WAVES), 0,   \
                        (hipStream_t)stream, *g, *p, P, Q, x, aggr_msg, x_new)
     if (p->bf16) {
-        if (drop) EQD_EDGE_FWD_LAUNCH(true, true); else EQD_EDGE_FWD_LAUNCH(true, false);
+        if (drop) EQD_EDGE_FWD_LAUNCH(true, true, false); else EQD_EDGE_FWD_LAUNCH(true, false, false);
+    } else if (edge_dma_on()) {
+        if (drop) EQD_EDGE_FWD_LAUNCH(false, true, true); else EQD_EDGE_FWD_LAUNCH(false, false, true);
+        ++g_edge_dma_launches;
     } else {
-        if (drop) EQD_EDGE_FWD_LAUNCH(false, true); else EQD_EDGE_FWD_LAUNCH(false, false);
+        if (drop) EQD_EDGE_FWD_LAUNCH(false, true, false); else EQD_EDGE_FWD_LAUNCH(false, false, false);
     }
 #undef EQD_EDGE_FWD_LAUNCH
     return eqd_check_launch("k_edge_fwd");
@@ -1075,31 +1242,30 @@
     const int drop = edge_drop_mode(p, "eqd_edge_attn_fwd");
     if (drop < 0) return EQD_ERR_NULL;
     if (int rc = edge_saved_check(p, "eqd_edge_attn_fwd")) return rc;
+    const bool dma = edge_dma_on();
+    if (dma) ++g_edge_dma_launches;
+#define EQD_EDGE_ATTN_LAUNCH(KERNEL_, WAVES_)                                                                             \
+    do {                                                                                                                  \
+        if (drop && dma) EQD_EDGE_ATTN_LAUNCH1(KERNEL_, WAVES_, true, true);                                              \
+        else if (drop) EQD_EDGE_ATTN_LAUNCH1(KERNEL_, WAVES_, true, false);                                               \
+        else if (dma) EQD_EDGE_ATTN_LAUNCH1(KERNEL_, WAVES_, false, true);                                                \
+        else EQD_EDGE_ATTN_LAUNCH1(KERNEL_, WAVES_, false, false);                                                        \
+    } while (0)
+#define EQD_EDGE_ATTN_LAUNCH1(KERNEL_, WAVES_, DROP_, DMA_)                                                               \
+    hipLaunchKernelGGL(HIP_KERNEL_NAME(KERNEL_<DROP_, DMA_>), dim3(n_edge + g->n_att_items), dim3(64 * (WAVES_)), 0, st, *g, \
+                       *p, n_edge, P, Q, x, aggr_msg, x_new, q, k, v, att_out, lse)
     if (d_att == 80) {
-        if (drop)
-            hipLaunchKernelGGL(k_edge_attn_fwd80<true>, dim3(n_edge + g->n_att_items), dim3(64 * FWD_WAVES), 0, st, *g, *p, n_edge,
-                               P, Q, x, aggr_msg, x_new, q, k, v, att_out, lse);
-        else
-            hipLaunchKernelGGL(k_edge_attn_fwd80<false>, dim3(n_edge + g->n_att_items), dim3(64 * FWD_WAVES), 0, st, *g, *p, n_edge,
-                               P, Q, x, aggr_msg, x_new, q, k, v, att_out, lse);
+        EQD_EDGE_ATTN_LAUNCH(k_edge_attn_fwd80, FWD_WAVES);
         return eqd_check_launch("k_edge_attn_fwd");
     }
     if (eqd_switch_on("EQD_EDGE_FWD_HALF") && g->n_tiles <= FWD_WAVES * n_edge) {
-        if (drop)
-            hipLaunchKernelGGL(k_edge_attn_fwd_half<true>, dim3(n_edge + g->n_att_items), dim3(64 * EDGE_HALF_WAVES), 0, st, *g, *p,
-                               n_edge, P, Q, x, aggr_msg, x_new, q, k, v, att_out, lse);
-        else
-            hipLaunchKernelGGL(k_edge_attn_fwd_half<false>, dim3(n_edge + g->n_att_items), dim3(64 * EDGE_HALF_WAVES), 0, st, *g, *p,
-                               n_edge, P, Q, x, aggr_msg, x_new, q, k, v, att_out, lse);
+        EQD_EDGE_ATTN_LAUNCH(k_edge_attn_fwd_half, EDGE_HALF_WAVES);
         ++g_edge_fwd_half_launches;
         return eqd_check_launch("k_edge_attn_fwd");
     }
-    if (drop)
-        hipLaunchKernelGGL(k_edge_attn_fwd<true>, dim3(n_edge + g->n_att_items), dim3(64 * FWD_WAVES), 0, st, *g, *p, n_edge, P,
-                           Q, x, aggr_msg, x_new, q, k, v, att_out, lse);
-    else
-        hipLaunchKernelGGL(k_edge_attn_fwd<false>, dim3(n_edge + g->n_att_items), dim3(64 * FWD_WAVES), 0, st, *g, *p, n_edge, P,
-                           Q, x, aggr_msg, x_new, q, k, v, att_out, lse);
+    EQD_EDGE_ATTN_LAUNCH(k_edge_attn_fwd, FWD_WAVES);
+#undef EQD_EDGE_ATTN_LAUNCH
+#undef EQD_EDGE_ATTN_LAUNCH1
     return eqd_check_launch("k_edge_attn_fwd");
 }
 
@@ -1214,7 +1380,7 @@
     enum { SLAB = 128 * USB };
 };
 
-template <bool BF, bool DROP = false, bool SAVED = false>
+template <bool BF, bool DROP = false, bool SAVED = false, bool DMA = false>
 __global__ __launch_bounds__(64 * BWD_WAVES) void k_edge_bwd(EqdGraph G, EqdEdgeParams P, const float* __restrict__ Pn,
                                                               const float* __restrict__ Qn,
                                                               const float* __restrict__ x,
@@ -1247,43 +1413,74 @@
         nx_dst = G.dst[ei];
     };
     if ((int)blockIdx.x < n_super) endpoints((int)blockIdx.x);
-    if constexpr (BF)
+    static_assert(!(BF && DMA), "bf16 converts while it stages");
+    EdgeTileState<1> S;
+    EdgeTileLoads<1> LD;
+    float4 dag[4];
+    float gxn[3];
+    int r0 = 0, r1 = 0;
+    auto tile_of = [&](int it_) {
+        S.n0 = S.n1 = 0;
+        S.e0 = 16 * (it_ * BWD_WAVES + wave);
+        S.ne = G.n_edges - S.e0;
+        S.ne = S.ne < 0 ? 0 : (S.ne > 16 ? 16 : S.ne);
+        if (S.ne == 0) S.e0 = 0;
+        S.src[0] = nx_src;
+        S.dst[0] = nx_dst;
+    };
+    auto dst_loads = [&]() {
+        const int d = S.dst[0];
+        r0 = G.rowptr[d];
+        r1 = G.rowptr[d + 1];
+#pragma unroll
+        for (int c = 0; c < 3; ++c) gxn[c] = d_xnew[(size_t)d * 3 + c];
+#pragma unroll
+        for (int mb = 0; mb < 4; ++mb) dag[mb] = *(const float4*)&d_aggr[(size_t)d * 64 + 16 * mb + 4 * g];
+    };
+    auto tile_head = [&](int it_) {
+        tile_of(it_);
+        if (it_ + (int)gridDim.x < n_super) endpoints(it_ + (int)gridDim.x);
+        dst_loads();
+        if constexpr (DMA) {
+            EQD_TR(2);
+            edge_tile_load<1, true, SAVED, DROP>(G, P, Pn, Qn, x, lane, S, LD);
+        }
+    };
+    if constexpr (BF) {
         edge_stage_weights_bf<BWD_WAVES, true>(sm, P);
-    else
+    } else if constexpr (DMA) {
+        if ((int)blockIdx.x < n_super) tile_head((int)blockIdx.x);
+        edge_stage_request<BWD_WAVES>(sm, P);
+        edge_stage_publish();
+    } else {
         edge_stage_weights(sm, P);
+    }
+    bool first = true;
     EQD_TR(1);
     float* tile = sm.tile[wave];
     float r_dlng = 0.f, r_dlnb = 0.f, r_dwc2 = 0.f, r_dbc1 = 0.f, r_db2 = 0.f, r_dbc2 = 0.f;
     const int wmb = wave >> 1, wnb = 2 * (wave & 1);
     f32x4 gW2[2] = {f4zero(), f4zero()}, gWc1[2] = {f4zero(), f4zero()}, gW1a[1] = {f4zero()}, gW1b[1] = {f4zero()};
     for (int it = blockIdx.x; it < n_super; it += gridDim.x) {
-        const int t = it * BWD_WAVES + wave;
-        EdgeTileState<1> S;
-        S.n0 = S.n1 = 0;
-        S.e0 = 16 * t;
-        S.ne = G.n_edges - S.e0;
-        S.ne = S.ne < 0 ? 0 : (S.ne > 16 ? 16 : S.ne);
-        if (S.ne == 0) S.e0 = 0;
-        S.src[0] = nx_src;
-        S.dst[0] = nx_dst;
-        if (it + (int)gridDim.x < n_super) endpoints(it + (int)gridDim.x);
+        if constexpr (!DMA) tile_head(it);
         f32x4 xh[4][1], m[4][1], ch[4][1];
-        float4 dag[4];
-        float gxn[3];
-        int r0, r1;
-        {
-            const int d = S.dst[0];
-            r0 = G.rowptr[d];
-            r1 = G.rowptr[d + 1];
-#pragma unroll
-            for (int c = 0; c < 3; ++c) gxn[c] = d_xnew[(size_t)d * 3 + c];
-#pragma unroll
-            for (int mb = 0; mb < 4; ++mb) dag[mb] = *(const float4*)&d_aggr[(size_t)d * 64 + 16 * mb + 4 * g];
-        }
-        if constexpr (BF)
+        if constexpr (BF) {
             edge_tile_forward_bf<1, DROP, true, SAVED>(G, P, sm.w1, sm.w2, sm.wc1, sm.vec, tile, Pn, Qn, x, lane, S, xh, m, ch);
-        else
+        } else if constexpr (DMA) {
+            if (first) {
+                keep_after_wait(r0); keep_after_wait(r1);
+#pragma unroll
+                for (int c = 0; c < 3; ++c) keep_after_wait(gxn[c]);
+#pragma unroll
+                for (int mb = 0; mb < 4; ++mb) {
+                    keep_after_wait(dag[mb].x); keep_after_wait(dag[mb].y); keep_after_wait(dag[mb].z); keep_after_wait(dag[mb].w);
+                }
+                edge_tile_loads_keep<1, SAVED, DROP>(LD);
+            }
+            edge_tile_compute<1, DROP, true, SAVED, DROP>(G, P, sm.w1, sm.w2, sm.wc1, sm.vec, tile, lane, S, LD, xh, m, ch, nullptr);
+        } else {
             edge_tile_forward<1, DROP, true, SAVED>(G, P, sm.w1, sm.w2, sm.wc1, sm.vec, tile, Pn, Qn, x, lane, S, xh, m, ch, nullptr);
+        }
         float invdeg = 0.f, dcoef = 0.f, dxr[3] = {0.f, 0.f, 0.f};
         {
             invdeg = S.ev[0] ? 1.f / (float)(r1 - r0) : 0.f;
@@ -1509,6 +1706,10 @@
         }
         if constexpr (!DBUF && !NOSLAB) __syncthreads();
         EQD_TR(21);
+        if constexpr (DMA) {
+            first = false;
+            if (it + (int)gridDim.x < n_super) tile_head(it + (int)gridDim.x);
+        }
     }
     {
         if constexpr (DBUF) __syncthreads();
@@ -1657,13 +1858,16 @@
         if (ko[0] == '1' && ko[1] == 0) W.wpart = nullptr;
     if (int rc = edge_saved_check(p, "eqd_edge_message_bwd_kernel_only")) return rc;
     const bool sv = p->xh_save != nullptr;
-#define EQD_EDGE_BWD_KO(BF_, SV_)                                                                                       \
-    hipLaunchKernelGGL(HIP_KERNEL_NAME(k_edge_bwd<BF_, false, SV_>), dim3(edge_bwd_blocks(g)), dim3(64 * BWD_WAVES), 0, \
+#define EQD_EDGE_BWD_KO(BF_, SV_, DMA_)                                                                                 \
+    hipLaunchKernelGGL(HIP_KERNEL_NAME(k_edge_bwd<BF_, false, SV_, DMA_>), dim3(edge_bwd_blocks(g)), dim3(64 * BWD_WAVES), 0, \
                        (hipStream_t)stream, *g, *p, P, Q, x, d_aggr_msg, d_xnew, W)
     if (p->bf16) {
-        if (sv) EQD_EDGE_BWD_KO(true, true); else EQD_EDGE_BWD_KO(true, false);
+        if (sv) EQD_EDGE_BWD_KO(true, true, false); else EQD_EDGE_BWD_KO(true, false, false);
+    } else if (edge_dma_on()) {
+        if (sv) EQD_EDGE_BWD_KO(false, true, true); else EQD_EDGE_BWD_KO(false, false, true);
+        ++g_edge_dma_launches;
     } else {
-        if (sv) EQD_EDGE_BWD_KO(false, true); else EQD_EDGE_BWD_KO(false, false);
+        if (sv) EQD_EDGE_BWD_KO(false, true, false); else EQD_EDGE_BWD_KO(false, false, false);
     }
 #undef EQD_EDGE_BWD_KO
     return eqd_check_launch("k_edge_bwd");
@@ -1706,14 +1910,17 @@
         }
         if (int rcs = edge_saved_check(p, "eqd_edge_message_bwd")) return rcs;
         const bool sv = p->xh_save != nullptr;
-#define EQD_EDGE_BWD_LAUNCH(BF_, DROP_, SV_)                                                                               \
-    hipLaunchKernelGGL(HIP_KERNEL_NAME(k_edge_bwd<BF_, DROP_, SV_>), dim3(blocks), dim3(64 * BWD_WAVES), 0, st, *g, *p, P, Q, \
-                       x, d_aggr_msg, d_xnew, W)
-#define EQD_EDGE_BWD_LAUNCH2(BF_, DROP_) do { if (sv) EQD_EDGE_BWD_LAUNCH(BF_, DROP_, true); else EQD_EDGE_BWD_LAUNCH(BF_, DROP_, false); } while (0)
+#define EQD_EDGE_BWD_LAUNCH(BF_, DROP_, SV_, DMA_)                                                                         \
+    hipLaunchKernelGGL(HIP_KERNEL_NAME(k_edge_bwd<BF_, DROP_, SV_, DMA_>), dim3(blocks), dim3(64 * BWD_WAVES), 0, st, *g, *p, \
+                       P, Q, x, d_aggr_msg, d_xnew, W)
+#define EQD_EDGE_BWD_LAUNCH2(BF_, DROP_, DMA_) do { if (sv) EQD_EDGE_BWD_LAUNCH(BF_, DROP_, true, DMA_); else EQD_EDGE_BWD_LAUNCH(BF_, DROP_, false, DMA_); } while (0)
         if (p->bf16) {
-            if (drop) EQD_EDGE_BWD_LAUNCH2(true, true); else EQD_EDGE_BWD_LAUNCH2(true, false);
+            if (drop) EQD_EDGE_BWD_LAUNCH2(true, true, false); else EQD_EDGE_BWD_LAUNCH2(true, false, false);
+        } else if (edge_dma_on() && (sv || !drop)) {
+            if (drop) EQD_EDGE_BWD_LAUNCH(false, true, true, true); else EQD_EDGE_BWD_LAUNCH2(false, false, true);
+            ++g_edge_dma_launches;
         } else {
-            if (drop) EQD_EDGE_BWD_LAUNCH2(false, true); else EQD_EDGE_BWD_LAUNCH2(false, false);
+            if (drop) EQD_EDGE_BWD_LAUNCH2(false, true, false); else EQD_EDGE_BWD_LAUNCH2(false, false, false);
         }
 #undef EQD_EDGE_BWD_LAUNCH2
 #undef EQD_EDGE_BWD_LAUNCH
diff --git a/include/equidock_hip.h b/include/equidock_hip.h
--- a/include/equidock_hip.h
+++ b/include/equidock_hip.h
@@ -227,6 +227,7 @@
 int eqd_edge_message_fwd(const EqdGraph* g, const EqdEdgeParams* p, const float* P, const float* Q,
                          const float* x, float* aggr_msg, float* x_new, void* stream);
 long long eqd_edge_fwd_half_launches(void);
+long long eqd_edge_dma_launches(void);
 int eqd_selftest_edge_attn_fwd(const EqdGraph* g, const EqdEdgeParams* p, const float* P, const float* Q, const float* x,
                                float* aggr_msg, float* x_new, int d_att, const float* q, const float* k, const float* v,
                                float* att_out, float* lse, void* stream);
```

Result: slower. 8647 pairs/s (-1.8%).
